# kenahm/se3-icp

Measured on AMD Instinct MI355X. Metric: ICP iterations/sec + pairs/sec, ~120k-pt KITTI clouds, 1/2/4/8 GPU, higher is better.
Workload: dtype f32 sweep + f64 certify/solve

## Files before the change

include/se3icp.h:

```cpp
#ifndef SE3ICP_H
#define SE3ICP_H

#include <stdint.h>

#ifdef __cplusplus
extern "C" {
#endif

#define SE3ICP_ABI_VERSION 4

typedef enum se3icp_status {
    SE3ICP_OK = 0,
    SE3ICP_ERR_INVALID_ARG = -1,
    SE3ICP_ERR_INVALID_METHOD = -2,
    SE3ICP_ERR_EMPTY_CLOUD = -3,
    SE3ICP_ERR_K_TOO_LARGE = -4,
    SE3ICP_ERR_NO_DEVICE = -5,
    SE3ICP_ERR_HIP = -6,
    SE3ICP_ERR_NONFINITE = -7,
    SE3ICP_ERR_OUT_OF_MEMORY = -8,
    SE3ICP_ERR_INTERNAL = -9
} se3icp_status;

typedef enum se3icp_method {
    SE3ICP_PT2PT = 0,
    SE3ICP_PT2PL = 1,
    SE3ICP_GICP = 2,
    SE3ICP_SE3_PT2PT = 3,
    SE3ICP_SE3_PT2PL = 4,
    SE3ICP_SE3_GICP = 5,
    SE3ICP_SE3_GICP_WITH_CF = 6,
    SE3ICP_SE3_PURE_PT2PT = 7,
    SE3ICP_SE3_PURE_PT2PL = 8,
    SE3ICP_SE3_PURE_GICP = 9,
    SE3ICP_NUM_METHODS = 10
} se3icp_method;

typedef struct se3icp_params {
    int32_t max_num_iterations;
    int32_t max_num_se3_iterations;
    int32_t number_of_nn_for_LRF;
    int32_t _reserved;
    double mse;
    double mse_switch_error;
    double estimated_overlap;
    double alpha_rot;
    double beta_transl;
    double scale_preprocessing;
} se3icp_params;

typedef struct se3icp_result {
    double T[16];
    int32_t num_iterations;
    int32_t num_pure_se3_iterations;
    int32_t status;
    int32_t num_rechecked;
    double scaling_factor;
    double time_setup_ms;
    double time_loop_ms;
    double time_se3_correspondence_search_ms;
    double time_before_pure_icp_ms;
} se3icp_result;

int se3icp_abi_version(void);
const char* se3icp_status_string(int status);
int se3icp_method_from_name(const char* name);
const char* se3icp_method_name(int method);
void se3icp_default_params(se3icp_params* p);
int se3icp_device_count(void);

typedef struct se3icp_registration se3icp_registration;

se3icp_registration* se3icp_registration_new(void);
void se3icp_registration_free(se3icp_registration* r);
int se3icp_set_source_cloud(se3icp_registration* r, const double* xyz, int64_t n);
int se3icp_set_target_cloud(se3icp_registration* r, const double* xyz, int64_t n);
se3icp_params* se3icp_params_of(se3icp_registration* r);
int se3icp_run_icp(se3icp_registration* r, const char* variant);
int se3icp_run_se3_icp(se3icp_registration* r, const char* variant);
int se3icp_run_se3_icp_with_cf(se3icp_registration* r);
int se3icp_run_se3_pure(se3icp_registration* r, const char* variant);
int se3icp_get_result(const se3icp_registration* r, se3icp_result* out);

int se3icp_register_batch(int device, int32_t n_pairs, const double* const* src_xyz, const int64_t* n_src,
                          const double* const* tgt_xyz, const int64_t* n_tgt, int method,
                          const se3icp_params* params, se3icp_result* results);

int se3icp_register_batch_device(int device, int32_t n_pairs, const double* d_src_xyz, const int64_t* src_off,
                                 const double* d_tgt_xyz, const int64_t* tgt_off, int method,
                                 const se3icp_params* params, se3icp_result* results, void* hip_stream);

int se3icp_register_sweep(int device, int32_t n_pairs, const double* const* src_xyz, const int64_t* n_src,
                          const double* const* tgt_xyz, const int64_t* n_tgt, int method, int32_t n_variants,
                          const se3icp_params* variants, int32_t max_group, se3icp_result* results);
int se3icp_register_sweep_device(int device, int32_t n_pairs, const double* d_src_xyz, const int64_t* src_off,
                                 const double* d_tgt_xyz, const int64_t* tgt_off, int method, int32_t n_variants,
                                 const se3icp_params* variants, int32_t max_group, se3icp_result* results,
                                 void* hip_stream);

int se3icp_register_graph(int device, int32_t n_clouds, const double* const* xyz, const int64_t* n_pts,
                          int32_t n_pairs, const int32_t* src_cloud, const int32_t* tgt_cloud, int method,
                          const se3icp_params* params, int32_t sharing, se3icp_result* results);
int se3icp_register_graph_device(int device, int32_t n_clouds, const double* d_xyz, const int64_t* off,
                                 int32_t n_pairs, const int32_t* src_cloud, const int32_t* tgt_cloud, int method,
                                 const se3icp_params* params, int32_t sharing, se3icp_result* results,
                                 void* hip_stream);
struct se3icp_report_options;
struct se3icp_report;
int se3icp_register_graph_report(int device, int32_t n_clouds, const double* const* xyz, const int64_t* n_pts,
                                 int32_t n_pairs, const int32_t* src_cloud, const int32_t* tgt_cloud, int method,
                                 const se3icp_params* params, int32_t sharing, se3icp_result* results,
                                 const struct se3icp_report_options* opts, struct se3icp_report* reports);
int se3icp_register_graph_report_device(int device, int32_t n_clouds, const double* d_xyz, const int64_t* off,
                                        int32_t n_pairs, const int32_t* src_cloud, const int32_t* tgt_cloud,
                                        int method, const se3icp_params* params, int32_t sharing,
                                        se3icp_result* results, void* hip_stream,
                                        const struct se3icp_report_options* opts, struct se3icp_report* reports);
#define SE3ICP_GRAPH_STATS_N 9
int se3icp_last_graph_stats(int device, int64_t* out, int n);

int se3icp_set_batch_sharing(int device, int level);

typedef enum se3icp_stop_reason {
    SE3ICP_STOP_CONVERGED = 0,
    SE3ICP_STOP_MAX_ITERATIONS = 1,
    SE3ICP_STOP_MAX_SE3_ITERATIONS = 2,
    SE3ICP_STOP_RUNAWAY = 3
} se3icp_stop_reason;

typedef struct se3icp_report_options {
    double max_correspondence_distance;
    int32_t* corr_idx;
    double* corr_dist;
    int32_t outputs_on_device;
    int32_t _reserved;
} se3icp_report_options;

typedef struct se3icp_report {
    double fitness;
    double inlier_rmse;
    double information[36];
    double final_mse;
    double final_mse_change;
    int64_t n_inliers;
    int32_t switched;
    int32_t stop_reason;
} se3icp_report;

int se3icp_report_version(void);

int se3icp_register_batch_report(int device, int32_t n_pairs, const double* const* src_xyz, const int64_t* n_src,
                                 const double* const* tgt_xyz, const int64_t* n_tgt, int method,
                                 const se3icp_params* params, se3icp_result* results,
                                 const se3icp_report_options* opts, se3icp_report* reports);
int se3icp_register_batch_report_device(int device, int32_t n_pairs, const double* d_src_xyz, const int64_t* src_off,
                                        const double* d_tgt_xyz, const int64_t* tgt_off, int method,
                                        const se3icp_params* params, se3icp_result* results, void* hip_stream,
                                        const se3icp_report_options* opts, se3icp_report* reports);
int se3icp_register_sweep_report(int device, int32_t n_pairs, const double* const* src_xyz, const int64_t* n_src,
                                 const double* const* tgt_xyz, const int64_t* n_tgt, int method, int32_t n_variants,
                                 const se3icp_params* variants, int32_t max_group, se3icp_result* results,
                                 const se3icp_report_options* opts, se3icp_report* reports);
int se3icp_register_sweep_report_device(int device, int32_t n_pairs, const double* d_src_xyz, const int64_t* src_off,
                                        const double* d_tgt_xyz, const int64_t* tgt_off, int method,
                                        int32_t n_variants, const se3icp_params* variants, int32_t max_group,
                                        se3icp_result* results, void* hip_stream,
                                        const se3icp_report_options* opts, se3icp_report* reports);
int se3icp_request_report(se3icp_registration* r, const se3icp_report_options* opts);
int se3icp_get_report(const se3icp_registration* r, se3icp_report* out);

int se3icp_register(int device, const double* src_xyz, int64_t n_src, const double* tgt_xyz, int64_t n_tgt,
                    int method, const se3icp_params* params, se3icp_result* result);


int se3icp_toldi_frames(int device, const double* xyz, int64_t n, int k, double* frames);
int se3icp_knn_self(int device, const double* xyz, int64_t n, int k, int32_t* idx);
int se3icp_estimate_normals(int device, const double* xyz, int64_t n, int k, double* normals);
int se3icp_nn(int device, const double* query, int64_t nq, const double* data, int64_t nd, int dim,
              int32_t* idx, double* d2, int32_t* num_rechecked);

int64_t se3icp_synthetic_pairs(int device, const double* base, int64_t n, int32_t n_cases, const double* T,
                               double ratio, double noise_var, uint64_t seed, double* src_out, double* tgt_out,
                               int outputs_on_device);

#define SE3ICP_GEN_ARGS_LTR 1
int64_t se3icp_synthetic_reference(const double* cloud, int64_t n, int32_t n_cases, double ratio, double noise_var,
                                   double t_range, double r_range, int32_t flags, double* src_out, double* tgt_out,
                                   double* T_out);
int64_t se3icp_synthetic_reference_device(int device, const double* cloud, int64_t n, int32_t n_cases, double ratio,
                                          double noise_var, double t_range, double r_range, int32_t flags,
                                          double* src_out, double* tgt_out, double* T_out, int outputs_on_device);
int64_t se3icp_random_downsample(const double* xyz, int64_t n, double ratio, uint32_t seed, double* out);

int se3icp_set_profiling(int device, int on);
int se3icp_last_kernel_times(int device, double* out);
#define SE3ICP_KERNEL_TIMES_N 26
int se3icp_last_kernel_times_n(int device, double* out, int n);

typedef struct se3icp_trace {
    int32_t pair;
    int32_t max_iters;
    int32_t* corr_idx;
    float* corr_dist;
    uint64_t* trim_key;
    double* T;
    double* mse;
    int32_t* phase;
    int32_t iters_recorded;
    int32_t _reserved;
} se3icp_trace;
int se3icp_set_trace(int device, se3icp_trace* trace);

int se3icp_set_lrf_exact(int device, int exact_only);

int se3icp_set_nn_events(int device, int on);

#ifdef __cplusplus
}
#endif
#endif
```

se3-icp_amd/csrc/capi.cpp:

```cpp
#include <hip/hip_runtime.h>

#include <cmath>
#include <cstdio>
#include <cstring>
#include <iostream>
#include <mutex>
#include <string>
#include <vector>

#include "engine.hpp"
#include "graph.hpp"
#include "se3icp.h"

using se3icp::Engine;
using se3icp::engine_for;
using se3icp::graph_check;
using se3icp::GS_COUNT;

namespace {

const char* kMethodNames[SE3ICP_NUM_METHODS] = {"pt2pt",     "pt2pl",     "gicp",
                                                "se3_pt2pt", "se3_pt2pl", "se3_gicp",
                                                "se3_gicp_with_cf", "se3_pure_pt2pt", "se3_pure_pt2pl",
                                                "se3_pure_gicp"};
// ... 27 lines not shown
    se3icp_result res;
    bool want_report = false, have_report = false;
    se3icp_report_options ropts{};
    se3icp_report rep{};
};

extern "C" {

int se3icp_abi_version(void) { return SE3ICP_ABI_VERSION; }

const char* se3icp_status_string(int status) {
    switch (status) {
        case SE3ICP_OK: return "ok";
        case SE3ICP_ERR_INVALID_ARG: return "invalid argument";
        case SE3ICP_ERR_INVALID_METHOD: return "invalid method name";
        case SE3ICP_ERR_EMPTY_CLOUD: return "empty point cloud";
        case SE3ICP_ERR_K_TOO_LARGE: return "number_of_nn_for_LRF too large (unused since ABI 3: any k is taken)";
        case SE3ICP_ERR_NO_DEVICE: return "no usable HIP device (the engine has no CPU fallback)";
        case SE3ICP_ERR_HIP: return "HIP runtime error";
        case SE3ICP_ERR_NONFINITE: return "non-finite pose";
        case SE3ICP_ERR_OUT_OF_MEMORY: return "out of device memory";
        case SE3ICP_ERR_INTERNAL: return "internal error: a result left unset or out of range";
        default: return "unknown status";
    }
}

int se3icp_method_from_name(const char* name) {
    if (!name) return SE3ICP_ERR_INVALID_METHOD;
    for (int m = 0; m < SE3ICP_NUM_METHODS; ++m)
        if (!std::strcmp(name, kMethodNames[m])) return m;
    return SE3ICP_ERR_INVALID_METHOD;
}

const char* se3icp_method_name(int method) {
    return (method >= 0 && method < SE3ICP_NUM_METHODS) ? kMethodNames[method] : nullptr;
}

void se3icp_default_params(se3icp_params* p) {
    if (!p) return;
    std::memset(p, 0, sizeof(*p));
    p->max_num_iterations = 150;
    p->max_num_se3_iterations = 20;
    p->number_of_nn_for_LRF = 30;
    p->mse = 0.00001;
    p->mse_switch_error = 0.001;
    p->estimated_overlap = 1.0;
    p->alpha_rot = 3.0;
    p->beta_transl = 1.0;
    p->scale_preprocessing = 3.0;
}

int se3icp_device_count(void) {
    int n = 0;
    if (hipGetDeviceCount(&n) != hipSuccess) return 0;
    return n;
}

static se3icp_params params_or_defaults(const se3icp_params* params) {
    se3icp_params p;
    if (params) p = *params; else se3icp_default_params(&p);
    return p;
}

struct PairRanges {
    std::vector<const double*> s, t;
    std::vector<int64_t> ns, nt;
};
static int pair_ranges(int32_t n_pairs, const double* d_src_xyz, const int64_t* src_off, const double* d_tgt_xyz,
                       const int64_t* tgt_off, PairRanges* r) {
    if (n_pairs <= 0 || !d_src_xyz || !d_tgt_xyz || !src_off || !tgt_off) return SE3ICP_ERR_INVALID_ARG;
    r->s.resize(n_pairs); r->t.resize(n_pairs); r->ns.resize(n_pairs); r->nt.resize(n_pairs);
    for (int i = 0; i < n_pairs; ++i) {
        r->s[i] = d_src_xyz + 3 * src_off[i];
        r->t[i] = d_tgt_xyz + 3 * tgt_off[i];
        r->ns[i] = src_off[i + 1] - src_off[i];
        r->nt[i] = tgt_off[i + 1] - tgt_off[i];
    }
    return SE3ICP_OK;
}

static int report_check(const se3icp_report_options* opts, const se3icp_report* reports, bool per_point_allowed) {
    if (!opts || !reports) return SE3ICP_ERR_INVALID_ARG;
    if (std::isnan(opts->max_correspondence_distance)) return SE3ICP_ERR_INVALID_ARG;
    if (!per_point_allowed && (opts->corr_idx || opts->corr_dist)) return SE3ICP_ERR_INVALID_ARG;
    return SE3ICP_OK;
}

static int pairs_check(int32_t n_pairs, const double* const* src, const int64_t* n_src, const double* const* tgt,
                       const int64_t* n_tgt, int method, const se3icp_params* prm, const se3icp_result* results) {
    if (n_pairs <= 0 || !n_src || !n_tgt || !results) return SE3ICP_ERR_INVALID_ARG;
    if (method < 0 || method >= SE3ICP_NUM_METHODS) return SE3ICP_ERR_INVALID_METHOD;
    for (int32_t p = 0; p < n_pairs; ++p)
        if (n_src[p] <= 0 || n_tgt[p] <= 0) return SE3ICP_ERR_EMPTY_CLOUD;
    if (method >= SE3ICP_SE3_PT2PT && prm && prm->number_of_nn_for_LRF <= 0) return SE3ICP_ERR_INVALID_ARG;
    for (int32_t p = 0; p < n_pairs; ++p)
        if (!src[p] || !tgt[p]) return SE3ICP_ERR_INVALID_ARG;
    return SE3ICP_OK;
}

static int batch_run(int device, int args, int32_t n_pairs, const double* const* src, const int64_t* n_src,
                     const double* const* tgt, const int64_t* n_tgt, bool on_device, int method,
                     const se3icp_params* params, se3icp_result* results, void* hip_stream,
                     const se3icp_report_options* opts, se3icp_report* reports, bool with_report) {
    if (with_report) {
        int rc = args ? args : report_check(opts, reports, true);
        if (!rc) rc = pairs_check(n_pairs, src, n_src, tgt, n_tgt, method, params, results);
        if (rc) return rc;
    }
    Engine* e = usable_engine(device);
    if (!e) return SE3ICP_ERR_NO_DEVICE;
    if (args) return args;
    const se3icp_params p = params_or_defaults(params);
    std::lock_guard<std::mutex> lk(e->mutex());
    return e->register_batch(n_pairs, src, n_src, tgt, n_tgt, on_device, method, p, results, (hipStream_t)hip_stream,
                             with_report ? opts : nullptr, with_report ? reports : nullptr);
}

static int sweep_run(int device, int args, int32_t n_pairs, const double* const* src, const int64_t* n_src,
                     const double* const* tgt, const int64_t* n_tgt, bool on_device, int method, int32_t n_variants,
                     const se3icp_params* variants, int32_t max_group, se3icp_result* results, void* hip_stream,
                     const se3icp_report_options* opts, se3icp_report* reports, bool with_report) {
    int rc = args;
    if (!rc && with_report) rc = report_check(opts, reports, false);
    if (!rc && (n_variants <= 0 || !variants || max_group < 0)) rc = SE3ICP_ERR_INVALID_ARG;
    if (!rc) rc = pairs_check(n_pairs, src, n_src, tgt, n_tgt, method, variants, results);
    for (int32_t v = 1; !rc && v < n_variants; ++v)
        if (variants[v].number_of_nn_for_LRF != variants[0].number_of_nn_for_LRF ||
            variants[v].scale_preprocessing != variants[0].scale_preprocessing)
            rc = SE3ICP_ERR_INVALID_ARG;
    if (rc) return rc;
    Engine* e = usable_engine(device);
    if (!e) return SE3ICP_ERR_NO_DEVICE;
    std::lock_guard<std::mutex> lk(e->mutex());
    return e->register_sweep(n_pairs, src, n_src, tgt, n_tgt, on_device, method, n_variants, variants, max_group,
                             results, (hipStream_t)hip_stream, with_report ? opts : nullptr,
                             with_report ? reports : nullptr);
}

int se3icp_register_batch(int device, int32_t n_pairs, const double* const* src_xyz, const int64_t* n_src,
                          const double* const* tgt_xyz, const int64_t* n_tgt, int method,
                          const se3icp_params* params, se3icp_result* results) {
    return batch_run(device, SE3ICP_OK, n_pairs, src_xyz, n_src, tgt_xyz, n_tgt, false, method, params, results,
                     nullptr, nullptr, nullptr, false);
}

int se3icp_register_batch_device(int device, int32_t n_pairs, const double* d_src_xyz, const int64_t* src_off,
                                 const double* d_tgt_xyz, const int64_t* tgt_off, int method,
                                 const se3icp_params* params, se3icp_result* results, void* hip_stream) {
    PairRanges r;
    const int args = pair_ranges(n_pairs, d_src_xyz, src_off, d_tgt_xyz, tgt_off, &r);
    return batch_run(device, args, n_pairs, r.s.data(), r.ns.data(), r.t.data(), r.nt.data(), true, method, params,
                     results, hip_stream, nullptr, nullptr, false);
}

int se3icp_register_batch_report(int device, int32_t n_pairs, const double* const* src_xyz, const int64_t* n_src,
                                 const double* const* tgt_xyz, const int64_t* n_tgt, int method,
                                 const se3icp_params* params, se3icp_result* results,
                                 const se3icp_report_options* opts, se3icp_report* reports) {
    const int args = (!src_xyz || !tgt_xyz) ? SE3ICP_ERR_INVALID_ARG : SE3ICP_OK;
    return batch_run(device, args, n_pairs, src_xyz, n_src, tgt_xyz, n_tgt, false, method, params, results, nullptr,
                     opts, reports, true);
}

int se3icp_register_batch_report_device(int device, int32_t n_pairs, const double* d_src_xyz, const int64_t* src_off,
                                        const double* d_tgt_xyz, const int64_t* tgt_off, int method,
                                        const se3icp_params* params, se3icp_result* results, void* hip_stream,
                                        const se3icp_report_options* opts, se3icp_report* reports) {
    PairRanges r;
    const int args = pair_ranges(n_pairs, d_src_xyz, src_off, d_tgt_xyz, tgt_off, &r);
    return batch_run(device, args, n_pairs, r.s.data(), r.ns.data(), r.t.data(), r.nt.data(), true, method, params,
                     results, hip_stream, opts, reports, true);
}

int se3icp_register_sweep(int device, int32_t n_pairs, const double* const* src_xyz, const int64_t* n_src,
                          const double* const* tgt_xyz, const int64_t* n_tgt, int method, int32_t n_variants,
                          const se3icp_params* variants, int32_t max_group, se3icp_result* results) {
    const int args = (!src_xyz || !tgt_xyz) ? SE3ICP_ERR_INVALID_ARG : SE3ICP_OK;
    return sweep_run(device, args, n_pairs, src_xyz, n_src, tgt_xyz, n_tgt, false, method, n_variants, variants,
                     max_group, results, nullptr, nullptr, nullptr, false);
}

int se3icp_register_sweep_device(int device, int32_t n_pairs, const double* d_src_xyz, const int64_t* src_off,
                                 const double* d_tgt_xyz, const int64_t* tgt_off, int method, int32_t n_variants,
                                 const se3icp_params* variants, int32_t max_group, se3icp_result* results,
                                 void* hip_stream) {
    PairRanges r;
    const int args = pair_ranges(n_pairs, d_src_xyz, src_off, d_tgt_xyz, tgt_off, &r);
    return sweep_run(device, args, n_pairs, r.s.data(), r.ns.data(), r.t.data(), r.nt.data(), true, method, n_variants,
                     variants, max_group, results, hip_stream, nullptr, nullptr, false);
}

int se3icp_report_version(void) { return 1; }

int se3icp_register_sweep_report(int device, int32_t n_pairs, const double* const* src_xyz, const int64_t* n_src,
                                 const double* const* tgt_xyz, const int64_t* n_tgt, int method, int32_t n_variants,
                                 const se3icp_params* variants, int32_t max_group, se3icp_result* results,
                                 const se3icp_report_options* opts, se3icp_report* reports) {
    const int args = (!src_xyz || !tgt_xyz) ? SE3ICP_ERR_INVALID_ARG : SE3ICP_OK;
    return sweep_run(device, args, n_pairs, src_xyz, n_src, tgt_xyz, n_tgt, false, method, n_variants, variants,
                     max_group, results, nullptr, opts, reports, true);
}

int se3icp_register_sweep_report_device(int device, int32_t n_pairs, const double* d_src_xyz, const int64_t* src_off,
                                        const double* d_tgt_xyz, const int64_t* tgt_off, int method,
                                        int32_t n_variants, const se3icp_params* variants, int32_t max_group,
                                        se3icp_result* results, void* hip_stream,
                                        const se3icp_report_options* opts, se3icp_report* reports) {
    PairRanges r;
    const int args = pair_ranges(n_pairs, d_src_xyz, src_off, d_tgt_xyz, tgt_off, &r);
    return sweep_run(device, args, n_pairs, r.s.data(), r.ns.data(), r.t.data(), r.nt.data(), true, method, n_variants,
                     variants, max_group, results, hip_stream, opts, reports, true);
}

static int graph_run(int device, int32_t n_clouds, const double* const* xyz, const int64_t* n_pts, bool on_device,
                     int32_t n_pairs, const int32_t* src_cloud, const int32_t* tgt_cloud, int method,
                     const se3icp_params* params, int32_t sharing, se3icp_result* results, void* hip_stream,
                     bool with_report, const se3icp_report_options* opts, se3icp_report* reports) {
    if (with_report) {
        const int rc = report_check(opts, reports, true);
        if (rc) return rc;
    }
    int rc = graph_check(n_clouds, n_pts, nullptr, n_pairs, src_cloud, tgt_cloud, method, SE3ICP_NUM_METHODS, sharing,
                         results);
    if (rc) return rc;
    if (method >= SE3ICP_SE3_PT2PT && params && params->number_of_nn_for_LRF <= 0) return SE3ICP_ERR_INVALID_ARG;
    for (int32_t p = 0; p < n_pairs; ++p)
        if (!xyz[src_cloud[p]] || !xyz[tgt_cloud[p]]) return SE3ICP_ERR_INVALID_ARG;
    Engine* e = usable_engine(device);
    if (!e) return SE3ICP_ERR_NO_DEVICE;
    const se3icp_params p = params_or_defaults(params);
    std::lock_guard<std::mutex> lk(e->mutex());
    return e->register_graph(n_clouds, xyz, n_pts, n_pairs, src_cloud, tgt_cloud, on_device, method, p, sharing, results,
                             (hipStream_t)hip_stream, with_report ? opts : nullptr, with_report ? reports : nullptr);
}

static int cloud_ranges(int32_t n_clouds, const double* d_xyz, const int64_t* off, std::vector<const double*>& x,
                        std::vector<int64_t>& n) {
    if (n_clouds <= 0 || !d_xyz || !off) return SE3ICP_ERR_INVALID_ARG;
    x.resize(n_clouds);
    n.resize(n_clouds);
    for (int32_t c = 0; c < n_clouds; ++c) {
        x[c] = d_xyz + 3 * off[c];
        n[c] = off[c + 1] - off[c];
    }
    return SE3ICP_OK;
}

int se3icp_register_graph(int device, int32_t n_clouds, const double* const* xyz, const int64_t* n_pts,
                          int32_t n_pairs, const int32_t* src_cloud, const int32_t* tgt_cloud, int method,
                          const se3icp_params* params, int32_t sharing, se3icp_result* results) {
    if (!xyz) return SE3ICP_ERR_INVALID_ARG;
    return graph_run(device, n_clouds, xyz, n_pts, false, n_pairs, src_cloud, tgt_cloud, method, params, sharing, results,
                     nullptr, false, nullptr, nullptr);
}

int se3icp_register_graph_device(int device, int32_t n_clouds, const double* d_xyz, const int64_t* off,
                                 int32_t n_pairs, const int32_t* src_cloud, const int32_t* tgt_cloud, int method,
                                 const se3icp_params* params, int32_t sharing, se3icp_result* results,
                                 void* hip_stream) {
    std::vector<const double*> x;
    std::vector<int64_t> n;
    const int rc = cloud_ranges(n_clouds, d_xyz, off, x, n);
    if (rc) return rc;
    return graph_run(device, n_clouds, x.data(), n.data(), true, n_pairs, src_cloud, tgt_cloud, method, params, sharing,
                     results, hip_stream, false, nullptr, nullptr);
}

int se3icp_register_graph_report(int device, int32_t n_clouds, const double* const* xyz, const int64_t* n_pts,
                                 int32_t n_pairs, const int32_t* src_cloud, const int32_t* tgt_cloud, int method,
                                 const se3icp_params* params, int32_t sharing, se3icp_result* results,
                                 const se3icp_report_options* opts, se3icp_report* reports) {
    if (!xyz) return SE3ICP_ERR_INVALID_ARG;
    return graph_run(device, n_clouds, xyz, n_pts, false, n_pairs, src_cloud, tgt_cloud, method, params, sharing, results,
                     nullptr, true, opts, reports);
}

int se3icp_register_graph_report_device(int device, int32_t n_clouds, const double* d_xyz, const int64_t* off,
                                        int32_t n_pairs, const int32_t* src_cloud, const int32_t* tgt_cloud, int method,
                                        const se3icp_params* params, int32_t sharing, se3icp_result* results,
                                        void* hip_stream, const se3icp_report_options* opts, se3icp_report* reports) {
    std::vector<const double*> x;
    std::vector<int64_t> n;
    const int rc = cloud_ranges(n_clouds, d_xyz, off, x, n);
    if (rc) return rc;
    return graph_run(device, n_clouds, x.data(), n.data(), true, n_pairs, src_cloud, tgt_cloud, method, params, sharing,
                     results, hip_stream, true, opts, reports);
}

int se3icp_last_graph_stats(int device, int64_t* out, int n) {
    if (!out || n < GS_COUNT) return SE3ICP_ERR_INVALID_ARG;
    Engine* e = usable_engine(device);
    if (!e) return SE3ICP_ERR_NO_DEVICE;
    std::lock_guard<std::mutex> lk(e->mutex());
    for (int k = 0; k < GS_COUNT; ++k) out[k] = e->graph_stats()[k];
    return SE3ICP_OK;
}

int se3icp_set_batch_sharing(int device, int level) {
    if (level < se3icp::kBatchSharingMin || level > se3icp::kBatchSharingMax) return SE3ICP_ERR_INVALID_ARG;
    Engine* e = usable_engine(device);
    if (!e) return SE3ICP_ERR_NO_DEVICE;
    std::lock_guard<std::mutex> lk(e->mutex());
    e->set_batch_sharing(level);
    return SE3ICP_OK;
}

int se3icp_register(int device, const double* src_xyz, int64_t n_src, const double* tgt_xyz, int64_t n_tgt,
                    int method, const se3icp_params* params, se3icp_result* result) {
    return se3icp_register_batch(device, 1, &src_xyz, &n_src, &tgt_xyz, &n_tgt, method, params, result);
}

se3icp_registration* se3icp_registration_new(void) {
    auto* r = new (std::nothrow) se3icp_registration;
    if (!r) return nullptr;
    se3icp_default_params(&r->prm);
    std::memset(&r->res, 0, sizeof(r->res));
    for (int i = 0; i < 4; ++i) r->res.T[i * 4 + i] = 1.0;
    r->res.num_pure_se3_iterations = -1;
    return r;
}

void se3icp_registration_free(se3icp_registration* r) { delete r; }

int se3icp_set_source_cloud(se3icp_registration* r, const double* xyz, int64_t n) {
    if (!r || (n > 0 && !xyz) || n < 0) return SE3ICP_ERR_INVALID_ARG;
    r->src.insert(r->src.end(), xyz, xyz + 3 * n);
    return 0;
}

int se3icp_set_target_cloud(se3icp_registration* r, const double* xyz, int64_t n) {
    if (!r || (n > 0 && !xyz) || n < 0) return SE3ICP_ERR_INVALID_ARG;
    r->tgt.insert(r->tgt.end(), xyz, xyz + 3 * n);
    return 0;
}

se3icp_params* se3icp_params_of(se3icp_registration* r) { return r ? &r->prm : nullptr; }

static int run_object(se3icp_registration* r, int method) {
    const int64_t ns = (int64_t)r->src.size() / 3, nt = (int64_t)r->tgt.size() / 3;
    if (ns <= 0 || nt <= 0) return SE3ICP_ERR_EMPTY_CLOUD;
    const double* s = r->src.data();
    const double* t = r->tgt.data();
    se3icp_result res;
    se3icp_report rep;
    int rc = r->want_report ? se3icp_register_batch_report(current_device(), 1, &s, &ns, &t, &nt, method, &r->prm, &res,
                                                           &r->ropts, &rep)
                            : se3icp_register_batch(current_device(), 1, &s, &ns, &t, &nt, method, &r->prm, &res);
    if (rc == SE3ICP_OK || rc == SE3ICP_ERR_NONFINITE) {
        r->res = res;
        r->have_report = r->want_report;
        if (r->want_report) r->rep = rep;
    }
    return rc;
}

int se3icp_run_icp(se3icp_registration* r, const char* variant) {
    if (!r) return SE3ICP_ERR_INVALID_ARG;
    const int v = variant_index(variant);
    if (v < 0) {
        std::cerr << "Invalid ICP variant name. Valid names are pt2pt, pt2pl and gicp.\n";
        return SE3ICP_ERR_INVALID_METHOD;
    }
    return run_object(r, SE3ICP_PT2PT + v);
}

int se3icp_run_se3_icp(se3icp_registration* r, const char* variant) {
    if (!r) return SE3ICP_ERR_INVALID_ARG;
    const int v = variant_index(variant);
    if (v < 0) {
        std::cerr << "Invalid variant name. Choose one of: pt2pt, pt2pl, gicp \n";
        std::cout << "Unknown optimization strategy for SE(3) \n";
        const int64_t ns = (int64_t)r->src.size() / 3, nt = (int64_t)r->tgt.size() / 3;
        if (ns <= 0 || nt <= 0) return SE3ICP_ERR_EMPTY_CLOUD;
        double cs[3] = {0, 0, 0}, ct[3] = {0, 0, 0};
        for (int64_t i = 0; i < ns; ++i)
            for (int a = 0; a < 3; ++a) cs[a] += r->src[3 * i + a];
        for (int64_t i = 0; i < nt; ++i)
            for (int a = 0; a < 3; ++a) ct[a] += r->tgt[3 * i + a];
        std::memset(r->res.T, 0, sizeof(r->res.T));
        for (int a = 0; a < 4; ++a) r->res.T[a * 4 + a] = 1.0;
        for (int a = 0; a < 3; ++a) r->res.T[a * 4 + 3] = ct[a] / (double)nt - cs[a] / (double)ns;
        r->res.num_iterations = 1;
        r->res.num_pure_se3_iterations = 1;
        r->res.status = SE3ICP_ERR_INVALID_METHOD;
        return SE3ICP_ERR_INVALID_METHOD;
    }
    return run_object(r, SE3ICP_SE3_PT2PT + v);
}

int se3icp_run_se3_icp_with_cf(se3icp_registration* r) {
    if (!r) return SE3ICP_ERR_INVALID_ARG;
    const int rc = run_object(r, SE3ICP_SE3_GICP_WITH_CF);
    if (rc == SE3ICP_OK || rc == SE3ICP_ERR_NONFINITE)
        std::cout << "### scaling factor = " << r->res.scaling_factor << std::endl;
    return rc;
}

int se3icp_run_se3_pure(se3icp_registration* r, const char* variant) {
    if (!r) return SE3ICP_ERR_INVALID_ARG;
    const int v = variant_index(variant);
    if (v < 0) {
        std::cerr << "Invalid variant name. Choose one of: pt2pt, pt2pl, gicp \n";
        return SE3ICP_ERR_INVALID_METHOD;
    }
    const int rc = run_object(r, SE3ICP_SE3_PURE_PT2PT + v);
    if (rc == SE3ICP_OK || rc == SE3ICP_ERR_NONFINITE) std::cout << "pure se3 finished" << std::endl;
    return rc;
}

int se3icp_get_result(const se3icp_registration* r, se3icp_result* out) {
    if (!r || !out) return SE3ICP_ERR_INVALID_ARG;
    *out = r->res;
    return 0;
}

int se3icp_request_report(se3icp_registration* r, const se3icp_report_options* opts) {
    if (!r) return SE3ICP_ERR_INVALID_ARG;
    if (!opts) {
        r->want_report = false;
        return 0;
    }
    if (std::isnan(opts->max_correspondence_distance) || opts->outputs_on_device) return SE3ICP_ERR_INVALID_ARG;
    r->ropts = *opts;
    r->want_report = true;
    return 0;
}

int se3icp_get_report(const se3icp_registration* r, se3icp_report* out) {
    if (!r || !out || !r->have_report) return SE3ICP_ERR_INVALID_ARG;
    *out = r->rep;
    return 0;
}

int se3icp_toldi_frames(int device, const double* xyz, int64_t n, int k, double* frames) {
    Engine* e = usable_engine(device);
    if (!e) return SE3ICP_ERR_NO_DEVICE;
    std::lock_guard<std::mutex> lk(e->mutex());
    return e->toldi_frames(xyz, n, k, frames);
}

int se3icp_knn_self(int device, const double* xyz, int64_t n, int k, int32_t* idx) {
    Engine* e = usable_engine(device);
    if (!e) return SE3ICP_ERR_NO_DEVICE;
    std::lock_guard<std::mutex> lk(e->mutex());
    return e->knn_self(xyz, n, k, idx);
}

int se3icp_estimate_normals(int device, const double* xyz, int64_t n, int k, double* normals) {
    Engine* e = usable_engine(device);
    if (!e) return SE3ICP_ERR_NO_DEVICE;
    std::lock_guard<std::mutex> lk(e->mutex());
    return e->estimate_normals(xyz, n, k, normals);
}

int se3icp_nn(int device, const double* query, int64_t nq, const double* data, int64_t nd, int dim, int32_t* idx,
              double* d2, int32_t* num_rechecked) {
    Engine* e = usable_engine(device);
    if (!e) return SE3ICP_ERR_NO_DEVICE;
    std::lock_guard<std::mutex> lk(e->mutex());
    return e->nn(query, nq, data, nd, dim, idx, d2, num_rechecked);
}

int se3icp_set_profiling(int device, int on) {
    Engine* e = usable_engine(device);
    if (!e) return SE3ICP_ERR_NO_DEVICE;
    e->set_profiling(on != 0);
    return 0;
}

int se3icp_set_trace(int device, se3icp_trace* trace) {
    Engine* e = usable_engine(device);
    if (!e) return SE3ICP_ERR_NO_DEVICE;
    if (trace && (trace->max_iters < 0 || trace->pair < 0)) return SE3ICP_ERR_INVALID_ARG;
    std::lock_guard<std::mutex> lk(e->mutex());
    e->set_trace(trace);
    return 0;
}

int se3icp_set_lrf_exact(int device, int exact_only) {
    Engine* e = usable_engine(device);
    if (!e) return SE3ICP_ERR_NO_DEVICE;
    std::lock_guard<std::mutex> lk(e->mutex());
    if (exact_only < 0 || exact_only > 2) return SE3ICP_ERR_INVALID_ARG;
    e->set_lrf_exact(exact_only);
    return 0;
}

int se3icp_set_nn_events(int device, int on) {
    Engine* e = usable_engine(device);
    if (!e) return SE3ICP_ERR_NO_DEVICE;
    std::lock_guard<std::mutex> lk(e->mutex());
    e->set_nn_events(on != 0);
    return 0;
}

int se3icp_last_kernel_times(int device, double* out ) {
    double x[SE3ICP_KERNEL_TIMES_N];
    const int rc = se3icp_last_kernel_times_n(device, x, SE3ICP_KERNEL_TIMES_N);
    if (rc == 0)
        for (int i = 0; i < 24; ++i) out[i] = x[i];
    return rc;
}

int se3icp_last_kernel_times_n(int device, double* out, int n) {
    Engine* e = usable_engine(device);
    if (!e || !out) return SE3ICP_ERR_NO_DEVICE;
    if (n < SE3ICP_KERNEL_TIMES_N) return SE3ICP_ERR_INVALID_ARG;
    const auto& k = e->kernel_times();
    out[0] = k.nn_se3_ms;
    out[1] = k.nn_r3_ms;
    out[2] = k.recheck_ms;
    out[3] = k.trim_ms;
    out[4] = k.reduce_ms;
    out[5] = k.setup_ms;
    out[6] = (double)k.nn_se3_launches;
    out[7] = (double)k.nn_r3_launches;
    out[8] = k.se3_dist_evals;
    out[9] = k.se3_box_tests;
    out[10] = k.r3_dist_evals;
    out[11] = k.r3_box_tests;
    out[12] = k.lrf_ms;
    out[13] = k.lrf_queries;
    out[14] = k.lrf_leaves;
    out[15] = k.lrf_merges;
    out[16] = k.lrf_box_tests;
    out[17] = k.lrf_candidates;
    out[18] = k.nn_prep_ms;
    out[19] = k.se3_queries;
    out[20] = k.se3_searched;
    out[21] = k.r3_queries;
    out[22] = k.r3_searched;
    out[23] = k.lrf_fallback;
    out[24] = k.se3_useful_evals;
    out[25] = k.r3_useful_evals;
    return 0;
}

}
```

se3-icp_amd/csrc/common.hpp:

```cpp
#pragma once
#include <stdint.h>

namespace se3icp {

constexpr int kSmallK = 128;
constexpr int kBlock = 256;
constexpr int kRedVals = 28;
constexpr int kStatCols = 17;
constexpr int kStatUseSe3 = 15, kStatUseR3 = 16;
constexpr int kHist = 256;
constexpr int kTrimList = 4096;
constexpr int kTrimBlocks = 32;
constexpr int kChunkQ = 1024;

enum Phase : int32_t { PHASE_IDLE = 0, PHASE_SE3 = 1, PHASE_R3 = 2 };
enum Estimator : int32_t { EST_PT2PT = 0, EST_PT2PL = 1, EST_GICP = 2 };

struct CloudDev {
    int32_t off;
    int32_t n;
};

struct PairDev {
    double T[12];
    double f32_center[3];
    int32_t src, tgt;
    int32_t phase;
    int32_t est;
    int32_t cf;
    int32_t trim;
    int32_t nkeep;
    int32_t iter;
    float tgt_norm12;
    float tgt_norm3;
    int32_t phase_start;
    int32_t _pad;
};

constexpr int kRedThreads = 256;
constexpr int kRedPer = 1;
constexpr int kRedQ = kRedThreads * kRedPer;

struct BlockWork {
    int32_t pair;
    int32_t q0, q1;
    int32_t s_off, t_off;
    int32_t _pad[3];
};

}
```

se3-icp_amd/csrc/engine.cpp:

```cpp
#include "engine.hpp"

#include <algorithm>
#include <chrono>
#include <cmath>
#include <cstdio>
#include <cstdlib>
#include <cstring>
#include <map>
#include <memory>

#include "graph.hpp"
#include "report.hpp"
#include "sweep.hpp"
#include "tree.hpp"

namespace se3icp {

namespace {

#define HIPCHK(x)                                                                                   \
    do {                                                                                            \
        hipError_t e_ = (x);                                                                        \
        if (e_ != hipSuccess) {                                                                     \
            std::fprintf(stderr, "se3icp: HIP error %s at %s:%d (%s)\n", hipGetErrorString(e_), __FILE__, \
// ... 124 lines not shown

int Engine::init() {
    int n = 0;
    if (hipGetDeviceCount(&n) != hipSuccess || dev_ < 0 || dev_ >= n) return SE3ICP_ERR_NO_DEVICE;
    HIPCHK(hipSetDevice(dev_));
    HIPCHK(hipStreamCreateWithFlags(&stream_, hipStreamNonBlocking));
    for (auto& e : ev_) HIPCHK(hipEventCreate(&e));
    for (auto& e : loop_ev_) HIPCHK(hipEventCreate(&e));
    if (const char* e = std::getenv("SE3ICP_NN_TRACE")) nn_trace_ = std::atoi(e) != 0;
    return 0;
}

Engine::~Engine() {
    if (!ok_) return;
    (void)hipSetDevice(dev_);
    for (DevBuf* b : bufs_)
        if (b->p) (void)hipFree(b->p);
    for (PinnedMem* m : pins_)
        if (m->mem) (void)hipHostFree(m->mem);
    for (auto& e : ev_)
        if (e) (void)hipEventDestroy(e);
    for (auto& e : loop_ev_)
        if (e) (void)hipEventDestroy(e);
    if (h_phase_) (void)hipHostFree(h_phase_);
    if (stream_) (void)hipStreamDestroy(stream_);
}

template <class T>
T* Engine::ensure(DevBuf& b, size_t count) {
    const size_t want = std::max<size_t>(count, 1) * sizeof(T);
    if (b.bytes >= want) return static_cast<T*>(b.p);
    if (b.p) (void)hipFree(b.p);
    b.p = nullptr;
    b.bytes = 0;
    const size_t alloc = want + want / 4;
    if (hipMalloc(&b.p, alloc) != hipSuccess) {
        b.p = nullptr;
        return nullptr;
    }
    b.bytes = alloc;
    return static_cast<T*>(b.p);
}

int Engine::alloc_points(int64_t ntot, int kmax, bool knn_list) {
    if (ntot >= (int64_t)1 << 30) return SE3ICP_ERR_INVALID_ARG;
    ntot_ = ntot;
    ld_ = (int)((std::max<int64_t>(ntot, 1) + 63) / 64 * 64);
    kmax_ = std::max(kmax, 1);
    knn_list_ = knn_list;
    const size_t L = (size_t)ld_;
    bool ok = ensure<int32_t>(d_cloud_of_, L) && ensure<double>(d_in_, 3 * L) && ensure<double>(d_xyz64_, 3 * L) &&
              ensure<float>(d_xyz32_, 3 * L) && ensure<double>(d_fr64_, 12 * L) && ensure<float>(d_fr32_, 12 * L) &&
              ensure<double>(d_nrm64_, 3 * L) && ensure<double>(d_conf64_, L) && ensure<double>(d_tgeo_, 8 * L) &&
              (!knn_list || ensure<int32_t>(d_knn_, L * kmax_)) && ensure<int32_t>(d_corr_idx_, L) && ensure<float>(d_corr_dist_, L) &&
              ensure<int32_t>(d_flag_count_, 4) &&
              ensure<uint32_t>(d_keys0_, L) &&
              ensure<int32_t>(d_vals1_, L) && ensure<unsigned long long>(d_stats_, kStatCols * kStatSlots) &&
              ensure<NNCert>(d_cert_, L) &&
              ensure<int32_t>(d_sqlist_, L);
    for (TreeBufs* t : {&t3_, &t12_})
        ok = ok && ensure<int32_t>(t->perm, L) && ensure<int32_t>(t->pos, L);
    ok = ok && ensure<float>(t3_.vec, 3 * L) && ensure<float>(t12_.vec, 12 * L);
    return ok ? 0 : SE3ICP_ERR_OUT_OF_MEMORY;
}

View Engine::view() const {
    View v{};
    v.ld = ld_;
    v.npts = (int32_t)ntot_;
    v.nclouds = nclouds_;
    v.npairs = npairs_;
    v.kmax = kmax_;
    v.clouds = (CloudDev*)d_clouds_.p;
    v.setup = (CloudSetup*)d_setup_.p;
    v.pairs = (PairDev*)d_pairs_.p;
    v.cloud_of = (int32_t*)d_cloud_of_.p;
    v.in_ptr = (const double* const*)d_inptr_.p;
    v.xyz64 = (double*)d_xyz64_.p;
    v.xyz32 = (float*)d_xyz32_.p;
    v.fr64 = (double*)d_fr64_.p;
    v.fr32 = (float*)d_fr32_.p;
    v.nrm64 = (double*)d_nrm64_.p;
    v.conf64 = (double*)d_conf64_.p;
    v.tgeo = (double*)d_tgeo_.p;
    v.knn = knn_list_ ? (int32_t*)d_knn_.p : nullptr;
    v.corr_idx = (int32_t*)d_corr_idx_.p;
    v.corr_dist = (float*)d_corr_dist_.p;
    v.stats = (unsigned long long*)d_stats_.p;
    v.flag_count = (int32_t*)d_flag_count_.p;
    v.gcost = (uint32_t*)d_gcost_.p;
    v.cls = (int32_t*)d_cls_.p;
    v.trim_key = (uint64_t*)d_trim_key_.p;
    v.trim_cand = (unsigned long long*)d_trim_cand_.p;
    v.trim_ctr = (unsigned*)d_trim_ctr_.p;
    v.trim_hist = (unsigned*)d_trim_hist_.p;
    v.red_partial = (double*)d_red_partial_.p;
    v.red_out = (double*)d_red_out_.p;
    v.work = (const BlockWork*)d_work_.p;
    v.nwork = nwork_;
    v.pair_rechecked = (int32_t*)d_rechecked_.p;
    auto ref = [&](const TreeBufs& t) {
        TreeRef r{};
        r.L = t.L;
        r.GL = tree_L_;
        r.nnodes = 2 << t.L;
        r.perm = (const int32_t*)t.perm.p;
        r.pos = (const int32_t*)t.pos.p;
        r.tvec = (const float*)t.vec.p;
        r.tvec64 = (const double*)t.vec64.p;
        r.tpt64 = (const double4*)t.vec64a.p;
        r.lo = (const float*)t.lo.p;
        r.hi = (const float*)t.hi.p;
        return r;
    };
    v.t3 = ref(t3_);
    v.t12 = ref(t12_);
    v.chunk_level = chunk_level_;
    v.nchunks = nchunks_;
    v.qlist = (int32_t*)d_qlist_.p;
    v.qcount = (int32_t*)d_qcount_.p;
    v.sq_list = (int32_t*)d_sqlist_.p;
    v.hist = (const double*)d_hist_.p;
    v.cert = (NNCert*)d_cert_.p;
    return v;
}

int Engine::build_tree(int D, const float* vec, hipStream_t s, const double* vec64) {
    TreeBufs& tb = (D == 12) ? t12_ : t3_;
    tb.L = tree_L_;
    const int nnodes = 2 << tb.L;
    const size_t nb = (size_t)nclouds_ * nnodes * D;
    if (!ensure<uint32_t>(tb.blo, nb) || !ensure<uint32_t>(tb.bhi, nb) || !ensure<float>(tb.lo, nb) ||
        !ensure<float>(tb.hi, nb) || !ensure<float>(tb.scr, (size_t)D * ld_) ||
        (D == 12 && !ensure<float>(tb.vecT, (size_t)12 * ld_)) ||
        (vec64 && !ensure<double>(tb.vec64, (size_t)3 * ld_)) ||
        (vec64 && D == 3 && !ensure<double4>(tb.vec64a, (size_t)ld_)))
        return SE3ICP_ERR_OUT_OF_MEMORY;
    std::vector<int32_t> host_n(nclouds_);
    int max_n = 0;
    for (int c = 0; c < nclouds_; ++c) max_n = std::max(max_n, host_n[c] = h_clouds_[c].n);
    const size_t need = tree_build_temp_bytes((int)ntot_, nclouds_, max_n, tb.L);
    if (!ensure<char>(d_sort_tmp_, std::max<size_t>(need, 256))) return SE3ICP_ERR_OUT_OF_MEMORY;
    TreeView t{};
    t.host_n = host_n.data();
    t.D = D;
    t.L = tb.L;
    t.nnodes = nnodes;
    t.nclouds = nclouds_;
    t.npts = (int32_t)ntot_;
    t.ld = ld_;
    t.clouds = (const CloudDev*)d_clouds_.p;
    t.cloud_of = (const int32_t*)d_cloud_of_.p;
    t.vec = vec;
    t.vecT = (D == 12) ? (float*)tb.vecT.p : const_cast<float*>(vec);
    t.perm = (int32_t*)tb.perm.p;
    t.pos = (int32_t*)tb.pos.p;
    t.tvec = (float*)tb.vec.p;
    t.vec64 = vec64;
    t.tvec64 = vec64 ? (double*)tb.vec64.p : nullptr;
    t.tpt64 = (vec64 && D == 3) ? (double4*)tb.vec64a.p : nullptr;
    t.vec64_sources_only = D == 12;
    t.blo = (uint32_t*)tb.blo.p;
    t.bhi = (uint32_t*)tb.bhi.p;
    t.scr = (float*)tb.scr.p;
    t.lo = (float*)tb.lo.p;
    t.hi = (float*)tb.hi.p;
    if (build_trees(t, d_sort_tmp_.p, d_sort_tmp_.bytes, (uint32_t*)d_keys0_.p, (int32_t*)d_vals1_.p, s) != 0)
        return SE3ICP_ERR_HIP;
    return 0;
}

int Engine::upload_clouds(const std::vector<CloudReq>& clouds, bool on_device, hipStream_t s) {
    nclouds_ = (int)clouds.size();
    h_clouds_.assign(nclouds_, CloudDev{});
    h_setup_.resize(nclouds_);
    h_chunks_.clear();
    h_inptr_.assign(nclouds_, nullptr);
    int64_t off = 0;
    int max_n = 1;
    for (int c = 0; c < nclouds_; ++c) {
        h_clouds_[c].off = (int32_t)off;
        h_clouds_[c].n = (int32_t)clouds[c].n;
        h_setup_[c] = clouds[c].st;
        max_n = std::max<int>(max_n, (int)clouds[c].n);
        for (int64_t p0 = 0; p0 < clouds[c].n; p0 += kChunk) h_chunks_.push_back(ChunkWork{c, (int32_t)p0});
        off += clouds[c].n;
    }
    tree_L_ = tree_depth_for(max_n);
    double* d_in = (double*)d_in_.p;
    for (int c = 0; c < nclouds_; ++c) {
        if (on_device) {
            h_inptr_[c] = clouds[c].in;
        } else {
            double* dst = d_in + 3 * (size_t)h_clouds_[c].off;
            HIPCHK(hipMemcpyAsync(dst, clouds[c].in, sizeof(double) * 3 * clouds[c].n, hipMemcpyHostToDevice, s));
            h_inptr_[c] = dst;
        }
    }
    const int nch = (int)h_chunks_.size();
    if (!ensure<CloudDev>(d_clouds_, nclouds_) || !ensure<CloudSetup>(d_setup_, nclouds_) ||
        !ensure<ChunkWork>(d_chunks_, nch) || !ensure<const double*>(d_inptr_, nclouds_) ||
        !ensure<double>(d_partial_, (size_t)nch * 9) || !ensure<double>(d_centers_, 3 * (size_t)nclouds_))
        return SE3ICP_ERR_OUT_OF_MEMORY;
    if (h_partial_.reserve((size_t)nch * 9 + 8)) return SE3ICP_ERR_OUT_OF_MEMORY;
    HIPCHK(hipMemcpyAsync(d_clouds_.p, h_clouds_.data(), sizeof(CloudDev) * nclouds_, hipMemcpyHostToDevice, s));
    HIPCHK(hipMemcpyAsync(d_setup_.p, h_setup_.data(), sizeof(CloudSetup) * nclouds_, hipMemcpyHostToDevice, s));
    HIPCHK(hipMemcpyAsync(d_chunks_.p, h_chunks_.data(), sizeof(ChunkWork) * nch, hipMemcpyHostToDevice, s));
    HIPCHK(hipMemcpyAsync(d_inptr_.p, h_inptr_.data(), sizeof(double*) * nclouds_, hipMemcpyHostToDevice, s));
    return 0;
}

int Engine::host_centroids(hipStream_t s, std::vector<double>* cen) {
    const int nch = (int)h_chunks_.size();
    HIPCHK(hipMemcpyAsync(h_partial_, d_partial_.p, sizeof(double) * 9 * nch, hipMemcpyDeviceToHost, s));
    SYNC_STREAM(s);
    std::vector<double> sum(3 * (size_t)nclouds_, 0.0);
    for (int k = 0; k < nch; ++k)
        for (int a = 0; a < 3; ++a) sum[3 * (size_t)h_chunks_[k].cloud + a] += h_partial_[9 * (size_t)k + a];
    cen->assign(3 * (size_t)nclouds_, 0.0);
    for (int c = 0; c < nclouds_; ++c)
        for (int a = 0; a < 3; ++a)
            (*cen)[3 * (size_t)c + a] = h_clouds_[c].n > 0 ? sum[3 * (size_t)c + a] / (double)h_clouds_[c].n : 0.0;
    return 0;
}

int Engine::setup_clouds(const std::vector<CloudReq>& clouds, bool on_device, bool pairs, bool normalize,
                         double scale_pre, hipStream_t s) {
    int rc = upload_clouds(clouds, on_device, s);
    if (rc) return rc;
    const int nch = (int)h_chunks_.size();
    View v = view();

    launch_ingest(v, (const ChunkWork*)d_chunks_.p, nch, (double*)d_partial_.p, s);
    HIPCHK(hipGetLastError());
    if (normalize) {
        if (!ensure<double>(d_scales_, std::max(1, nclouds_ / 2))) return SE3ICP_ERR_OUT_OF_MEMORY;
        launch_pair_centers(v, (const ChunkWork*)d_chunks_.p, nch, (const double*)d_partial_.p, (double*)d_centers_.p,
                            s);
        launch_radius(v, (const ChunkWork*)d_chunks_.p, nch, (const double*)d_centers_.p, (double*)d_partial_.p, s);
        launch_pair_scales(v, (const ChunkWork*)d_chunks_.p, nch, (const double*)d_partial_.p,
                           (const double*)d_centers_.p, scale_pre, (double*)d_scales_.p, s);
        HIPCHK(hipGetLastError());
        for (int c = 0; c < nclouds_; ++c)
            for (int a = 0; a < 3; ++a) h_setup_[c].f32_center[a] = 0.0;
    } else {
        std::vector<double> cen;
        rc = host_centroids(s, &cen);
        if (rc) return rc;
        for (int c = 0; c < nclouds_; ++c) {
            const int cc = pairs ? (c | 1) : c;
            for (int a = 0; a < 3; ++a) {
                h_setup_[c].norm_center[a] = 0.0;
                h_setup_[c].f32_center[a] = cen[3 * cc + a];
            }
            h_setup_[c].norm_scale = 1.0;
        }
        HIPCHK(hipMemcpyAsync(d_setup_.p, h_setup_.data(), sizeof(CloudSetup) * nclouds_, hipMemcpyHostToDevice, s));
    }

    launch_normalize(v, (const ChunkWork*)d_chunks_.p, nch, (double*)d_partial_.p, s);
    HIPCHK(hipGetLastError());

    rc = build_tree(3, (const float*)d_xyz32_.p, s, (const double*)d_xyz64_.p);
    if (rc) return rc;
    rc = setup_knn(s);
    if (rc) return rc;
    HIPCHK(hipGetLastError());
    return 0;
}

int Engine::setup_knn(hipStream_t s) {
    const View v = view();
    bool any_knn = false;
    for (int c = 0; c < nclouds_; ++c) any_knn |= h_setup_[c].k_knn > 0;
    if (any_knn) {
        HIPCHK(hipMemsetAsync(d_stats_.p, 0, sizeof(unsigned long long) * kStatCols * kStatSlots, s));
        HIPCHK(hipEventRecord(ev_[6], s));
        int kw_big = 0, n_big = 0;
        for (int c = 0; c < nclouds_; ++c) {
            const int kw = std::min<int>(h_setup_[c].k_knn, h_clouds_[c].n);
            if (kw > kSmallK || lrf_exact_only_ == 2) {
                kw_big = std::max(kw_big, kw);
                n_big += h_clouds_[c].n;
            }
        }
        int big_cap = 0, big_blocks = 0;
        if (n_big > 0) {
            big_cap = knn_big_cap(kw_big);
            big_blocks = knn_big_blocks(big_cap, n_big);
            if (!ensure<double>(d_big_d_, (size_t)big_blocks * big_cap) || !ensure<int32_t>(d_big_i_, (size_t)big_blocks * big_cap))
                return SE3ICP_ERR_OUT_OF_MEMORY;
        }
        auto big = [&](const int32_t* qlist, const int32_t* qcount, int k_min) {
            if (n_big > 0)
                launch_knn_big(v, knn_list_ ? 1 : 0, k_min, qlist, qcount, big_blocks, (double*)d_big_d_.p,
                               (int32_t*)d_big_i_.p, big_cap, s);
        };
        if (lrf_exact_only_ == 2) {
            big(nullptr, nullptr, 0);
        } else if (knn_list_ || lrf_exact_only_ == 1) {
            launch_lrf(v, knn_list_ ? 1 : 0, s);
            big(nullptr, nullptr, kSmallK);
        } else {
            std::vector<int32_t> wb(nclouds_ + 1, 0);
            for (int c = 0; c < nclouds_; ++c) wb[c + 1] = wb[c] + (h_setup_[c].k_knn > 0 ? (h_clouds_[c].n + 7) / 8 : 0);
            const int nw = wb[nclouds_];
            if (!ensure<int32_t>(d_lrf_fb_, (size_t)8 * nw + 64) || !ensure<int32_t>(d_lrf_fbn_, 2 + nclouds_ + 1))
                return SE3ICP_ERR_OUT_OF_MEMORY;
            int32_t* d_wb = (int32_t*)d_lrf_fbn_.p + 2;
            int32_t* fb = (int32_t*)d_lrf_fb_.p;
            int32_t* fbn = (int32_t*)d_lrf_fbn_.p;
            HIPCHK(hipMemsetAsync(fbn, 0, 2 * sizeof(int32_t), s));
            HIPCHK(hipMemcpyAsync(d_wb, wb.data(), sizeof(int32_t) * (nclouds_ + 1), hipMemcpyHostToDevice, s));
            launch_lrf8(v, d_wb, 0, nw, fb, fbn, s);
            launch_lrf_list(v, fb, fbn, s);
            big(fb, fbn, kSmallK);
        }
        HIPCHK(hipEventRecord(ev_[7], s));
        HIPCHK(hipGetLastError());
        if (h_lrf_stats_.reserve((size_t)kStatCols * kStatSlots)) return SE3ICP_ERR_OUT_OF_MEMORY;
        HIPCHK(hipMemcpyAsync(h_lrf_stats_, d_stats_.p, sizeof(unsigned long long) * kStatCols * kStatSlots,
                              hipMemcpyDeviceToHost, s));
        lrf_stats_pending_ = true;
    }
    return 0;
}

int Engine::read_lrf_stats() {
    if (!lrf_stats_pending_) return 0;
    lrf_stats_pending_ = false;
    double sum[kStatCols] = {};
    for (int i = 0; i < kStatSlots; ++i)
        for (int k = 0; k < kStatCols; ++k) sum[k] += (double)h_lrf_stats_[kStatCols * i + k];
    float ms = 0;
    HIPCHK(hipEventElapsedTime(&ms, ev_[6], ev_[7]));
    ktimes_.lrf_ms = ms;
    ktimes_.lrf_queries = sum[0];
    ktimes_.lrf_leaves = sum[1];
    ktimes_.lrf_merges = sum[2];
    ktimes_.lrf_box_tests = sum[3];
    ktimes_.lrf_candidates = sum[4];
    ktimes_.lrf_fallback = sum[6];
#ifdef SE3ICP_PROF
    tree_prof_report();
    std::fprintf(stderr, "[prof] k_lrf cycles/query: knn|scan %.0f sort|tighten %.0f sums|final+sums %.0f finish %.0f "
                 "(queries %.0f, wave cycles summed over the kernel's waves)\n",
                 sum[8] / sum[0], sum[9] / sum[0], sum[10] / sum[0], sum[11] / sum[0], sum[0]);
    std::fprintf(stderr, "[prof] k_lrf8 per query: tightenings %.3f (overflow %.3f, final %.3f), leaf scans %.3f\n",
                 sum[2] / sum[0], sum[3] / sum[0], sum[7] / sum[0], sum[1] / sum[0]);
    {
        unsigned long long f = 0;
        for (int i = 0; i < kStatSlots; ++i) f += h_lrf_stats_[kStatCols * i + 5];
        std::fprintf(stderr, "[prof] k_lrf8 hand-overs: waves with the leaf table full %llu, no room %llu, > 128 at the end %llu; "
                     "queries with f32-equal f64-distinct ranks %llu\n",
                     f & 0xffff, (f >> 16) & 0xffff, (f >> 32) & 0xffff, f >> 48);
    }
#endif
    return 0;
}

int Engine::sync_stream(hipStream_t s) {
    HIPCHK(hipEventRecord(ev_[15], s));
    HIPCHK(spin_wait(ev_[15]));
    return read_lrf_stats();
}

int Engine::setup_chunks(int npairs, hipStream_t s) {
    chunk_level_ = std::max(0, tree_L_ - 4);
    nchunks_ = npairs << chunk_level_;
    if (!ensure<int32_t>(d_qlist_, (size_t)nchunks_ * kChunkQ) || !ensure<int32_t>(d_qcount_, (size_t)nchunks_ * (kChunkQ / 64)) ||
        !ensure<double>(d_hist_, (size_t)kHist * npairs * 12) || !ensure<uint32_t>(d_gcost_, (size_t)nchunks_ * 16) ||
        !ensure<int32_t>(d_cls_, nn_cls_words(nchunks_)))
        return SE3ICP_ERR_OUT_OF_MEMORY;
    if (h_hist_.reserve((size_t)npairs * 12)) return SE3ICP_ERR_OUT_OF_MEMORY;
    HIPCHK(hipMemsetAsync(d_cert_.p, 0xff, sizeof(NNCert) * ld_, s));
    HIPCHK(hipMemsetAsync(d_gcost_.p, 0, sizeof(uint32_t) * nchunks_ * 16, s));
    HIPCHK(hipMemsetAsync(d_cls_.p, 0, sizeof(int32_t) * 2 * 8 * 16, s));
    return 0;
}

int Engine::open_call(int args, int64_t nslots, int rest, hipStream_t user_stream, Call* c) {
    if (!ok_) return SE3ICP_ERR_NO_DEVICE;
    se3icp_trace* tr = c->tr = trace_;
    trace_ = nullptr;
    if (args) return args;
    if (tr && (tr->pair < 0 || (int64_t)tr->pair >= nslots || tr->max_iters < 0)) return SE3ICP_ERR_INVALID_ARG;
    if (tr) tr->iters_recorded = 0;
    if (rest) return rest;
    HIPCHK(hipSetDevice(dev_));
    c->s = user_stream ? user_stream : stream_;
    ktimes_ = KernelTimes{};
    HIPCHK(hipEventRecord(ev_[12], c->s));
    return 0;
}

int Engine::run_pairs(const MethodPlan& mp, int npairs, const int64_t* ns, const int64_t* nt,
                      const se3icp_params* vprm, int pairs_per_variant, bool sweep, const Call& c, se3icp_result* out,
                      const se3icp_report_options* ropts, se3icp_report* reports) {
    hipStream_t s = c.s;
    int rc = 0;
    if (mp.se3) rc = build_tree(12, (const float*)d_fr32_.p, s, (const double*)d_fr64_.p);
    if (rc) return rc;
    rc = prepare_pairs(npairs, ns, nt, s);
    if (rc) return rc;
    rc = setup_chunks(npairs, s);
    if (rc) return rc;
    HIPCHK(hipMemsetAsync(d_corr_idx_.p, 0xff, sizeof(int32_t) * ld_, s));
    HIPCHK(hipMemsetAsync(d_stats_.p, 0, sizeof(unsigned long long) * kStatCols * kStatSlots, s));
    for (double& t : trace_prev_) t = 0;
    HIPCHK(hipEventRecord(ev_[13], s));
    const ReportReq rq{ropts, reports};
    return run_loop(npairs, ns, mp.kind, mp.est, vprm, pairs_per_variant, sweep, c.tr, out, s,
                    (ropts && reports) ? &rq : nullptr);
}

int Engine::register_batch(int npairs, const double* const* src, const int64_t* ns, const double* const* tgt,
                           const int64_t* nt, bool on_device, int method, const se3icp_params& prm,
                           se3icp_result* out, hipStream_t user_stream, const se3icp_report_options* ropts,
                           se3icp_report* reports) {
    const int args = (npairs <= 0 || !src || !tgt || !ns || !nt || !out) ? SE3ICP_ERR_INVALID_ARG : 0;
    MethodPlan mp{};
    const int rest = args ? 0 : plan_pairs(method, prm.number_of_nn_for_LRF, npairs, src, ns, tgt, nt, &mp);
    Call call;
    int rc = open_call(args, npairs, rest, user_stream, &call);
    if (rc) return rc;

    npairs_ = npairs;
    int64_t ntot = 0;
    for (int p = 0; p < npairs; ++p) ntot += ns[p] + nt[p];
    rc = alloc_points(ntot, mp.kmax);
    if (rc) return rc;
    std::vector<CloudReq> clouds(2 * npairs);
    for (int p = 0; p < npairs; ++p)
        for (int side = 0; side < 2; ++side)
            clouds[2 * p + side] = CloudReq{side == 0 ? src[p] : tgt[p], side == 0 ? ns[p] : nt[p],
                                            cloud_setup(mp, side, prm.alpha_rot, prm.beta_transl, true)};
    bool look = false;
    if (on_device && batch_sharing_ != 1) {
        std::vector<int64_t> n(clouds.size());
        for (size_t u = 0; u < clouds.size(); ++u) n[u] = clouds[u].n;
        look = clouds.size() <= kShareMaxSlots && share_any_equal_n((int32_t)n.size(), n.data());
        for (int64_t& g : graph_stats_) g = 0;
        graph_stats_[GS_CLOUDS] = graph_stats_[GS_USES] = graph_stats_[GS_CLASSES] = (int64_t)clouds.size();
        for (const CloudReq& c : clouds) graph_stats_[GS_FULL] += c.st.k_knn > 0;
    }
    rc = look ? setup_pairs_shared(clouds, mp, prm.scale_preprocessing, call.s)
              : setup_clouds(clouds, on_device, true, mp.se3, prm.scale_preprocessing, call.s);
    if (rc) return rc;
    return run_pairs(mp, npairs, ns, nt, &prm, npairs, false, call, out, ropts, reports);
}

int Engine::setup_pairs_shared(const std::vector<CloudReq>& clouds, const MethodPlan& mp, double scale_pre,
                               hipStream_t s) {
    const int U = (int)clouds.size();
    const bool se3 = mp.se3;
    int rc = upload_clouds(clouds, true, s);
    if (rc) return rc;
    const int nch = (int)h_chunks_.size();
    if (!ensure<uint64_t>(d_share_hash_, U) || !ensure<SharePair>(d_share_pairs_, U) ||
        !ensure<int32_t>(d_share_same_, U) || h_share_hash_.reserve(U) || h_share_same_.reserve(U) ||
        h_share_setup_.reserve(U))
        return SE3ICP_ERR_OUT_OF_MEMORY;
    View v = view();
    HIPCHK(hipMemsetAsync(d_share_hash_.p, 0, sizeof(uint64_t) * U, s));
    launch_share_hash(v, (unsigned long long*)d_share_hash_.p, s);
    HIPCHK(hipMemcpyAsync(h_share_hash_, d_share_hash_.p, sizeof(uint64_t) * U, hipMemcpyDeviceToHost, s));
    launch_ingest(v, (const ChunkWork*)d_chunks_.p, nch, (double*)d_partial_.p, s);
    HIPCHK(hipGetLastError());
    if (se3) {
        if (!ensure<double>(d_scales_, std::max(1, nclouds_ / 2))) return SE3ICP_ERR_OUT_OF_MEMORY;
        launch_pair_centers(v, (const ChunkWork*)d_chunks_.p, nch, (const double*)d_partial_.p, (double*)d_centers_.p,
                            s);
        launch_radius(v, (const ChunkWork*)d_chunks_.p, nch, (const double*)d_centers_.p, (double*)d_partial_.p, s);
        launch_pair_scales(v, (const ChunkWork*)d_chunks_.p, nch, (const double*)d_partial_.p,
                           (const double*)d_centers_.p, scale_pre, (double*)d_scales_.p, s);
        HIPCHK(hipGetLastError());
        HIPCHK(hipMemcpyAsync(h_share_setup_, d_setup_.p, sizeof(CloudSetup) * U, hipMemcpyDeviceToHost, s));
        HIPCHK(hipEventRecord(ev_[10], s));
        for (int c = 0; c < nclouds_; ++c)
            for (int a = 0; a < 3; ++a) h_setup_[c].f32_center[a] = 0.0;
    } else {
        std::vector<double> cen;
        rc = host_centroids(s, &cen);
        if (rc) return rc;
        for (int c = 0; c < nclouds_; ++c) {
            for (int a = 0; a < 3; ++a) {
                h_setup_[c].norm_center[a] = 0.0;
                h_setup_[c].f32_center[a] = cen[3 * (c | 1) + a];
            }
            h_setup_[c].norm_scale = 1.0;
        }
        HIPCHK(hipMemcpyAsync(d_setup_.p, h_setup_.data(), sizeof(CloudSetup) * nclouds_, hipMemcpyHostToDevice, s));
    }
    launch_normalize(v, (const ChunkWork*)d_chunks_.p, nch, (double*)d_partial_.p, s);
    HIPCHK(hipGetLastError());
    rc = build_tree(3, (const float*)d_xyz32_.p, s, (const double*)d_xyz64_.p);
    if (rc) return rc;
    if (se3) HIPCHK(spin_wait(ev_[10]));

    std::vector<int64_t> n(U);
    for (int u = 0; u < U; ++u) n[u] = clouds[u].n;
    std::vector<int32_t> first, cloud;
    const int ncand = share_candidates(U, n.data(), h_share_hash_, &first);
    int nc = U;
    if (ncand > 0) {
        share_pairs_.clear();
        for (int u = 0; u < U; ++u)
            if (first[u] != u) share_pairs_.push_back(SharePair{u, first[u]});
        HIPCHK(hipMemcpyAsync(d_share_pairs_.p, share_pairs_.data(), sizeof(SharePair) * ncand, hipMemcpyHostToDevice, s));
        HIPCHK(hipMemsetAsync(d_share_same_.p, 1, sizeof(int32_t) * U, s));
        launch_share_compare(v, (const SharePair*)d_share_pairs_.p, ncand, (int32_t*)d_share_same_.p, s);
        HIPCHK(hipGetLastError());
        HIPCHK(hipMemcpyAsync(h_share_same_, d_share_same_.p, sizeof(int32_t) * U, hipMemcpyDeviceToHost, s));
        HIPCHK(hipEventRecord(ev_[11], s));
        HIPCHK(spin_wait(ev_[11]));
        nc = share_clouds(U, first.data(), h_share_same_, &cloud);
    }
    if (nc == U) return setup_knn(s);

    const CloudSetup* dev_table = se3 ? (const CloudSetup*)h_share_setup_ : h_setup_.data();
    share_setup_.assign(dev_table, dev_table + U);
    std::vector<GraphUse> use(U);
    for (int u = 0; u < U; ++u) {
        const CloudSetup& st = share_setup_[u];
        use[u].cloud = cloud[u];
        use[u].k_nrm = st.k_nrm;
        use[u].norm_scale = st.norm_scale;
        for (int a = 0; a < 3; ++a) {
            use[u].norm_center[a] = st.norm_center[a];
            use[u].f32_center[a] = st.f32_center[a];
        }
    }
    GraphPlan plan;
    graph_plan_uses(U, use.data(), se3, true, &plan);
    graph_stats_[GS_CLOUDS] = nc;
    graph_stats_[GS_CLASSES] = (int64_t)plan.classes.size();
    return select_by_class(plan, share_setup_, mp, s);
}

int Engine::select_by_class(const GraphPlan& plan, const std::vector<CloudSetup>& batch, const MethodPlan& mp,
                            hipStream_t s) {
    const int U = (int)batch.size(), K = (int)plan.classes.size();
    const bool se3 = mp.se3;
    std::vector<int32_t> home(K, -1);
    for (int u = 0; u < U; ++u)
        if (home[plan.use_class[u]] < 0) home[plan.use_class[u]] = u;
    sel_batch_ = batch;
    sel_run_ = sel_batch_;
    sel_chunks_.clear();
    sel_seg_.assign(U, GraphSeg{});
    graph_stats_[GS_FULL] = 0;
    for (int u = 0; u < U; ++u) {
        const int k = plan.use_class[u];
        const GraphClass& gc = plan.classes[k];
        CloudSetup& st = sel_run_[u];
        const bool is_home = home[k] == u;
        st.k_lrf = is_home ? mp.k_lrf : 0;
        st.k_nrm = (is_home && gc.nrm_from == k) ? gc.k_nrm : 0;
        st.k_knn = std::max(st.k_lrf, st.k_nrm);
        graph_stats_[GS_FULL] += st.k_knn > 0;
        const int hf = home[k], hn = home[gc.nrm_from];
        sel_seg_[u] = GraphSeg{h_clouds_[hf].off, hf, h_clouds_[hn].off, (hf != u && se3) ? 1 : 0};
        if ((hf != u && se3) || hn != u)
            for (int64_t p0 = 0; p0 < h_clouds_[u].n; p0 += kChunk) sel_chunks_.push_back(ChunkWork{u, (int32_t)p0});
    }
    const int nchS = (int)sel_chunks_.size();
    if (!ensure<ChunkWork>(g_chunks_, nchS) || !ensure<GraphSeg>(g_seg_, U)) return SE3ICP_ERR_OUT_OF_MEMORY;
    h_setup_ = sel_run_;
    HIPCHK(hipMemcpyAsync(d_setup_.p, sel_run_.data(), sizeof(CloudSetup) * U, hipMemcpyHostToDevice, s));
    const int rc = setup_knn(s);
    if (rc) return rc;
    HIPCHK(hipGetLastError());
    h_setup_ = sel_batch_;
    HIPCHK(hipMemcpyAsync(d_setup_.p, sel_batch_.data(), sizeof(CloudSetup) * U, hipMemcpyHostToDevice, s));
    if (nchS > 0) {
        HIPCHK(hipMemcpyAsync(g_chunks_.p, sel_chunks_.data(), sizeof(ChunkWork) * nchS, hipMemcpyHostToDevice, s));
        HIPCHK(hipMemcpyAsync(g_seg_.p, sel_seg_.data(), sizeof(GraphSeg) * U, hipMemcpyHostToDevice, s));
        launch_graph_share(view(), (const ChunkWork*)g_chunks_.p, nchS, (const GraphSeg*)g_seg_.p, s);
        HIPCHK(hipGetLastError());
    }
    return 0;
}

int Engine::prepare_pairs(int npairs, const int64_t* ns, const int64_t* nt, hipStream_t s) {
    int64_t soff = 0;
    h_work_.clear();
    h_wb_.assign(npairs, 0);
    h_wn_.assign(npairs, 0);
    for (int p = 0; p < npairs; ++p) {
        h_wb_[p] = (int32_t)h_work_.size();
        for (int64_t q0 = 0; q0 < ns[p]; q0 += kRedQ)
            h_work_.push_back(BlockWork{p, (int32_t)q0, (int32_t)std::min<int64_t>(q0 + kRedQ, ns[p]), (int32_t)soff,
                                        (int32_t)(soff + ns[p]), {0, 0, 0}});
        soff += ns[p] + nt[p];
        h_wn_[p] = (int32_t)h_work_.size() - h_wb_[p];
    }
    nwork_ = (int)h_work_.size();
    if (!ensure<PairDev>(d_pairs_, npairs) || !ensure<BlockWork>(d_work_, nwork_) || !ensure<int32_t>(d_wb_, npairs) ||
        !ensure<int32_t>(d_wn_, npairs) || !ensure<uint64_t>(d_trim_key_, 2 * (size_t)npairs) ||
        !ensure<unsigned long long>(d_trim_cand_, (size_t)npairs * kTrimList) || !ensure<unsigned>(d_trim_ctr_, 4 * (size_t)npairs) ||
        !ensure<unsigned>(d_trim_hist_, 4096 * (size_t)npairs) ||
        !ensure<double>(d_red_partial_, (size_t)nwork_ * kRedVals) || !ensure<double>(d_red_out_, (size_t)npairs * kRedVals) ||
        !ensure<int32_t>(d_rechecked_, npairs))
        return SE3ICP_ERR_OUT_OF_MEMORY;
    if (h_pairs_.reserve(npairs) || h_red_.reserve((size_t)npairs * kRedVals) || h_rechecked_.reserve(npairs))
        return SE3ICP_ERR_OUT_OF_MEMORY;
    HIPCHK(hipMemcpyAsync(d_work_.p, h_work_.data(), sizeof(BlockWork) * nwork_, hipMemcpyHostToDevice, s));
    HIPCHK(hipMemcpyAsync(d_wb_.p, h_wb_.data(), sizeof(int32_t) * npairs, hipMemcpyHostToDevice, s));
    HIPCHK(hipMemcpyAsync(d_wn_.p, h_wn_.data(), sizeof(int32_t) * npairs, hipMemcpyHostToDevice, s));
    HIPCHK(hipMemsetAsync(d_rechecked_.p, 0, sizeof(int32_t) * npairs, s));
    return 0;
}

int Engine::run_loop(int npairs, const int64_t* ns, int kind, int est, const se3icp_params* vprm,
                     int pairs_per_variant, bool sweep, se3icp_trace* tr, se3icp_result* out, hipStream_t s,
                     const ReportReq* rq) {
    const MethodInfo mi{(Kind)kind, est};
    const bool se3 = mi.kind != KIND_ICP;
    int rc = 0;

    if (!ensure<PairState>(d_state_, npairs) || h_state_.reserve(npairs))
        return SE3ICP_ERR_OUT_OF_MEMORY;
    if (h_phase_cap_ < (size_t)npairs * kLoopRing) {
        if (h_phase_) (void)hipHostFree(h_phase_);
        h_phase_ = nullptr;
        h_phase_cap_ = 0;
        const size_t want = std::max<size_t>((size_t)npairs * kLoopRing, 64);
        if (hipHostMalloc((void**)&h_phase_, want * sizeof(int32_t), hipHostMallocMapped | hipHostMallocCoherent) !=
                hipSuccess ||
            hipHostGetDevicePointer((void**)&d_phase_, h_phase_, 0) != hipSuccess)
            return SE3ICP_ERR_OUT_OF_MEMORY;
        h_phase_cap_ = want;
    }
    int se3_limit = 0;
    for (int k = 0; k * pairs_per_variant < npairs; ++k) {
        const int m = vprm[k].max_num_se3_iterations;
        se3_limit = (m < 1 || se3_limit < 0) ? -1 : std::max(se3_limit, m);
    }
    int n_se3 = 0, n_r3 = 0;
    bool any_trim = false;
    for (int p = 0; p < npairs; ++p) {
        const se3icp_params& prm = vprm[p / pairs_per_variant];
        const float ratio = std::min(1.0f, std::max(0.0f, (float)prm.estimated_overlap));
        PairState& S = h_state_[p];
        std::memset(&S, 0, sizeof(S));
        S.T = M4::eye();
        S.mse_prev = S.mse_cur = S.rel = 1e7;
        S.sf = 1.0;
        S.mse = prm.mse;
        S.mse_switch = prm.mse_switch_error;
        S.kind = mi.kind;
        S.max_iter = prm.max_num_iterations;
        S.max_se3 = prm.max_num_se3_iterations;
        S.phase = PHASE_IDLE;
        S.phase_start = 1;
        const unsigned nv = (unsigned)std::floor(ratio * (float)ns[p]);
        const bool trim = (int64_t)nv < ns[p];
        S.K = trim ? (double)nv : (double)ns[p];
        PairDev& P = h_pairs_[p];
        std::memset(&P, 0, sizeof(P));
        P.src = 2 * p;
        P.tgt = 2 * p + 1;
        P.est = mi.est;
        P.cf = mi.kind == KIND_CF;
        P.trim = trim;
        P.nkeep = (int)nv;
        for (int a = 0; a < 3; ++a) P.f32_center[a] = h_setup_[2 * p].f32_center[a];
        pair_open_iteration(S, P);
        std::memcpy(h_hist_ + 12 * (size_t)p, P.T, sizeof(P.T));
        n_se3 += P.phase == PHASE_SE3;
        n_r3 += P.phase == PHASE_R3;
        any_trim |= trim;
    }
    HIPCHK(hipMemcpyAsync(d_pairs_.p, h_pairs_, sizeof(PairDev) * npairs, hipMemcpyHostToDevice, s));
    HIPCHK(hipMemcpyAsync(d_state_.p, h_state_, sizeof(PairState) * npairs, hipMemcpyHostToDevice, s));
    HIPCHK(hipMemcpyAsync((double*)d_hist_.p + (size_t)(1 % kHist) * npairs * 12, h_hist_, sizeof(double) * 12 * npairs,
                          hipMemcpyHostToDevice, s));
    HIPCHK(hipMemsetAsync(d_flag_count_.p, 0, 3 * sizeof(int32_t), s));
    launch_pair_norms(view(), 2 << t3_.L, se3 ? 2 << t12_.L : 0, se3 ? (const double*)d_scales_.p : nullptr,
                      (double*)((char*)d_state_.p + offsetof(PairState, sf)), (int)(sizeof(PairState) / sizeof(double)),
                      s);
    HIPCHK(hipGetLastError());
    HIPCHK(hipMemsetAsync((uint64_t*)d_trim_key_.p + npairs, 0, sizeof(uint64_t) * npairs, s));
    HIPCHK(hipMemsetAsync(d_trim_ctr_.p, 0, sizeof(unsigned) * 4 * npairs, s));
    launch_geo_rows(view(), s);
    HIPCHK(hipMemsetAsync(d_trim_hist_.p, 0, sizeof(unsigned) * 4096 * npairs, s));
    View v = view();
    double nn_ms = 0;
    const int lag = (nn_trace_ || tr) ? 0 : 1;
    int trace_phase = tr ? h_pairs_[tr->pair].phase : 0;
    auto enqueue = [&](int it) -> int {
        hipEvent_t* ev = &loop_ev_[(it % kLoopRing) * kLoopEv];
        for (int p = 0; p < npairs; ++p) h_phase_[(size_t)(it % kLoopRing) * npairs + p] = -1;
        const bool do_se3 =
            n_se3 > 0 && (se3_limit < 1 || it <= se3_limit);
        const bool do_r3 = n_r3 > 0 || (mi.kind != KIND_ICP && mi.kind != KIND_PURE && it >= 2);
        const bool detail = profile_ || nn_trace_;
        const bool t_se3 = detail || (do_se3 && nn_events_);
        if (detail) HIPCHK(hipEventRecord(ev[0], s));
        launch_nn_prep(v, (lag == 1 && it >= 2) ? d_phase_ + (size_t)((it - 1) % kLoopRing) * npairs : nullptr, s);
        if (t_se3) HIPCHK(hipEventRecord(ev[1], s));
        if (do_se3) launch_nn(v, 12, s);
        if (t_se3) HIPCHK(hipEventRecord(ev[2], s));
        if (do_r3) launch_nn(v, 3, s);
        if (detail) HIPCHK(hipEventRecord(ev[3], s));
        if (detail) HIPCHK(hipEventRecord(ev[4], s));
        if (any_trim) launch_trim(v, s);
        if (detail) HIPCHK(hipEventRecord(ev[5], s));
        launch_reduce(v, (const int32_t*)d_wb_.p, (const int32_t*)d_wn_.p, (PairState*)d_state_.p, (double*)d_hist_.p,
                      lag == 0 ? d_phase_ + (size_t)(it % kLoopRing) * npairs : nullptr, s);
        HIPCHK(hipGetLastError());
        if (detail) HIPCHK(hipEventRecord(ev[6], s));
        loop_detail_[it % kLoopRing] = detail;
        loop_flags_[it % kLoopRing] = (do_se3 ? 1 : 0) | (do_r3 ? 2 : 0) | (t_se3 ? 4 : 0);
        return 0;
    };
    auto finish = [&](int it, bool last) -> int {
        hipEvent_t* ev = &loop_ev_[(it % kLoopRing) * kLoopEv];
        if (loop_detail_[it % kLoopRing]) HIPCHK(spin_wait(ev[6]));
        if (last && lag == 1) {
            if (!loop_detail_[it % kLoopRing]) {
                HIPCHK(hipEventRecord(ev_[15], s));
                HIPCHK(spin_wait(ev_[15]));
            }
        } else {
            HIPCHK(spin_phases(h_phase_ + (size_t)(it % kLoopRing) * npairs, npairs, s));
        }
        float ms[6] = {};
        if (loop_detail_[it % kLoopRing]) {
            for (int k = 0; k < 6; ++k) HIPCHK(hipEventElapsedTime(&ms[k], ev[k], ev[k + 1]));
        } else if (loop_flags_[it % kLoopRing] & 4) {
            HIPCHK(hipEventElapsedTime(&ms[1], ev[1], ev[2]));
        }
        ktimes_.nn_prep_ms += ms[0];
        ktimes_.nn_se3_ms += ms[1];
        ktimes_.nn_r3_ms += ms[2];
        ktimes_.recheck_ms += ms[3];
        ktimes_.trim_ms += ms[4];
        ktimes_.reduce_ms += ms[5];
        nn_ms += ms[0] + ms[1] + ms[2] + ms[3];
        const int flags = loop_flags_[it % kLoopRing];
        if (flags & 1) ktimes_.nn_se3_launches++;
        if (flags & 2) ktimes_.nn_r3_launches++;
        if (nn_trace_) {
            unsigned long long stats[kStatCols * kStatSlots];
            HIPCHK(hipMemcpy(stats, d_stats_.p, sizeof(stats), hipMemcpyDeviceToHost));
            double sum[kStatCols] = {};
            for (int i = 0; i < kStatSlots; ++i)
                for (int k = 0; k < kStatCols; ++k) sum[k] += (double)stats[kStatCols * i + k];
            std::fprintf(stderr,
                         "[nn] iter %d: se3 %.0f/%.0f searched, evals %.3g boxes %.3g | r3 %.0f/%.0f, evals %.3g "
                         "boxes %.3g | prep %.3f nn12 %.3f nn3 %.3f recheck %.3f ms\n",
                         it, sum[5] - trace_prev_[5], sum[4] - trace_prev_[4], sum[0] - trace_prev_[0],
                         sum[1] - trace_prev_[1], sum[7] - trace_prev_[7], sum[6] - trace_prev_[6],
                         sum[2] - trace_prev_[2], sum[3] - trace_prev_[3], ms[0], ms[1], ms[2], ms[3]);
#ifdef SE3ICP_PROF
            {
                double d[kStatCols];
                for (int k = 0; k < kStatCols; ++k) d[k] = sum[k] - trace_prev_[k];
                const double nw = std::floor(d[11] / 17592186044416.0), dt = d[11] - nw * 17592186044416.0;
                std::fprintf(stderr, "[nn] iter %d: %.0f SE(3) group waves, mean %.1f us, summed %.1f ms (100 MHz clock)\n",
                             it, nw, nw > 0 ? dt / nw / 100.0 : 0.0, dt / 1e5);
                std::fprintf(stderr, "[nn] iter %d: k_nn_prep span %.1f us\n", it, nn_prep_span());
                nn_wave_report(it);
                std::fprintf(stderr, "[nn] iter %d: wave cycles in leaf visits %.1f %% (target loads %.1f %%), "
                             "%.0f cycles per leaf visit, %.0f per box-test step\n", it, 100.0 * d[12] / std::max(1.0, d[13]),
                             100.0 * d[14] / std::max(1.0, d[13]), d[12] / std::max(1.0, d[9]),
                             (d[13] - d[12]) / std::max(1.0, d[1] / 128.0));
            }
#endif
            for (int k = 0; k < kStatCols; ++k) trace_prev_[k] = sum[k];
#ifdef SE3ICP_PROF
            std::fprintf(stderr, "[nn] iter %d: longest SE(3) group wave %.1f us (%llu box-test steps, %llu leaf visits, "
                         "%llu queries)\n", it, (double)(stats[10] >> 40) / 100.0, (stats[10] >> 20) & 0xfffffull,
                         (stats[10] >> 6) & 0x3fffull, stats[10] & 63ull);
            HIPCHK(hipMemset((unsigned long long*)d_stats_.p + 10, 0, sizeof(unsigned long long)));
#endif
        }
        if (last && lag == 1) return 0;
        const volatile int32_t* ph = h_phase_ + (size_t)(it % kLoopRing) * npairs;
        n_se3 = n_r3 = 0;
        for (int p = 0; p < npairs; ++p) {
            const int32_t f = ph[p];
            n_se3 += f == PHASE_SE3;
            n_r3 += f == PHASE_R3;
        }
        return n_se3 + n_r3;
    };
    static_assert(kLoopRing >= 2, "one iteration in flight while the previous one is read");
    int it = 1;
    if (enqueue(it)) return SE3ICP_ERR_HIP;
    for (;;) {
        if (lag == 0) {
            const int left = finish(it, false);
            if (tr) {
                rc = record_trace(tr, it, trace_phase, s);
                if (rc) return rc;
            }
            if (left == 0) break;
            ++it;
            if (enqueue(it)) return SE3ICP_ERR_HIP;
            continue;
        }
        ++it;
        if (enqueue(it)) return SE3ICP_ERR_HIP;
        if (finish(it - 1, false) == 0) {
            (void)finish(it, true);
            break;
        }
    }
    HIPCHK(hipEventRecord(ev_[14], s));
    HIPCHK(hipMemcpyAsync(h_state_, d_state_.p, sizeof(PairState) * npairs, hipMemcpyDeviceToHost, s));
    const int nbase = 2 * pairs_per_variant;
    if (se3) HIPCHK(hipMemcpyAsync(h_partial_, d_centers_.p, sizeof(double) * 3 * nbase, hipMemcpyDeviceToHost, s));
    HIPCHK(hipMemcpyAsync(h_rechecked_, d_rechecked_.p, sizeof(int32_t) * npairs, hipMemcpyDeviceToHost, s));
    {
        if (h_loop_stats_.reserve((size_t)kStatCols * kStatSlots)) return SE3ICP_ERR_OUT_OF_MEMORY;
        const unsigned long long* stats = h_loop_stats_;
        HIPCHK(hipMemcpyAsync(h_loop_stats_, d_stats_.p, sizeof(unsigned long long) * kStatCols * kStatSlots,
                              hipMemcpyDeviceToHost, s));
        if (rq) {
            rc = queue_report(npairs, ns, *rq, s);
            if (rc) return rc;
        }
        SYNC_STREAM(s);
        double sum[kStatCols] = {};
        for (int i = 0; i < kStatSlots; ++i)
            for (int k = 0; k < kStatCols; ++k) sum[k] += (double)stats[kStatCols * i + k];
        ktimes_.se3_dist_evals += sum[0];
        ktimes_.se3_box_tests += sum[1];
        ktimes_.r3_dist_evals += sum[2];
        ktimes_.r3_box_tests += sum[3];
        ktimes_.se3_queries += sum[4];
        ktimes_.se3_searched += sum[5];
        ktimes_.r3_queries += sum[6];
        ktimes_.r3_searched += sum[7];
        ktimes_.se3_useful_evals += sum[kStatUseSe3];
        ktimes_.r3_useful_evals += sum[kStatUseR3];
#ifdef SE3ICP_PROF
        {
            const double nw = std::max(1.0, std::floor(sum[11] / 17592186044416.0));
            const double mean = std::fmod(sum[11], 17592186044416.0) / nw;
            const double sq = (double)stats[kStatCols + 10] / nw;
            nn_prof_report();
            trim_prof_report();
            std::fprintf(stderr, "[prof] nn12: leaf visits %.0f; %.0f group waves, %.1f us each on average (sd %.1f, "
                         "longest %.1f us; 100 MHz clock)\n",
                         sum[9], nw, mean / 100.0, std::sqrt(std::max(0.0, sq - mean * mean)) / 100.0,
                         (double)(stats[10] >> 40) / 100.0);
            std::fprintf(stderr, "[prof] nn12 longest wave: %llu box-test steps, %llu leaf visits, %llu queries\n",
                         (stats[10] >> 20) & 0xfffffull, (stats[10] >> 6) & 0x3fffull, stats[10] & 63ull);
        }
#endif
    }
    float setup_ms = 0, loop_ms = 0;
    if (sweep) {
        float shared_ms = 0, group_ms = 0;
        HIPCHK(hipEventElapsedTime(&shared_ms, ev_[12], ev_[8]));
        HIPCHK(hipEventElapsedTime(&group_ms, ev_[9], ev_[13]));
        setup_ms = shared_ms + group_ms;
        ktimes_.setup_ms = shared_ms;
    } else {
        HIPCHK(hipEventElapsedTime(&setup_ms, ev_[12], ev_[13]));
        ktimes_.setup_ms = setup_ms;
    }
    HIPCHK(hipEventElapsedTime(&loop_ms, ev_[13], ev_[14]));

    int worst = 0;
    for (int p = 0; p < npairs; ++p) {
        const PairState& S = h_state_[p];
        M4 T = S.T;
        const int bp = p % pairs_per_variant;
        if (rq) {
// ... 590 lines not shown
```

se3-icp_amd/csrc/engine.hpp:

```cpp
#pragma once
#include <hip/hip_runtime.h>

#include <mutex>
#include <stdint.h>
#include <vector>

#include "graph.hpp"
#include "pairmath.hpp"
#include "se3icp.h"
#include "view.hpp"

namespace se3icp {

struct DevBuf {
    void* p = nullptr;
    size_t bytes = 0;
    explicit DevBuf(std::vector<DevBuf*>& owner) { owner.push_back(this); }
};
struct PinnedMem {
    void* mem = nullptr;
    size_t cap = 0;
};
template <class T>
struct Pinned : PinnedMem {
    explicit Pinned(std::vector<PinnedMem*>& owner) { owner.push_back(this); }
    operator T*() const { return static_cast<T*>(mem); }
    int reserve(size_t count) {
        if (cap >= count && mem) return 0;
        if (mem) (void)hipHostFree(mem);
        mem = nullptr;
        cap = 0;
        const size_t want = count > 16 ? count : 16;
        if (hipHostMalloc(&mem, want * sizeof(T), hipHostMallocDefault) != hipSuccess) return SE3ICP_ERR_OUT_OF_MEMORY;
        cap = want;
        return 0;
    }
};

struct KernelTimes {
    double nn_se3_ms = 0, nn_r3_ms = 0, recheck_ms = 0, trim_ms = 0, reduce_ms = 0;
    double setup_ms = 0;
    int64_t nn_se3_launches = 0, nn_r3_launches = 0;
    double se3_dist_evals = 0, se3_box_tests = 0, r3_dist_evals = 0, r3_box_tests = 0;
    double se3_useful_evals = 0, r3_useful_evals = 0;
    double lrf_ms = 0, lrf_queries = 0, lrf_leaves = 0, lrf_merges = 0, lrf_box_tests = 0, lrf_candidates = 0;
    double lrf_fallback = 0;
    double nn_prep_ms = 0, se3_queries = 0, se3_searched = 0, r3_queries = 0, r3_searched = 0;
};

struct MethodPlan {
    Kind kind;
    int est;
    bool se3;
    int k_lrf, k_nrm_s, k_nrm_t, kmax;
};

class Engine {
  public:
    explicit Engine(int device);
    ~Engine();
    Engine(const Engine&) = delete;
    Engine& operator=(const Engine&) = delete;

    int device() const { return dev_; }
    std::mutex& mutex() { return mu_; }
    void set_profiling(bool on) { profile_ = on; }
    void set_trace(se3icp_trace* t) { trace_ = t; }
    void set_lrf_exact(int mode) { lrf_exact_only_ = mode; }
    void set_nn_events(bool on) { nn_events_ = on; }
    void set_batch_sharing(int level) { batch_sharing_ = level; }
    const KernelTimes& kernel_times() const { return ktimes_; }

    int register_batch(int npairs, const double* const* src, const int64_t* ns, const double* const* tgt,
                       const int64_t* nt, bool on_device, int method, const se3icp_params& prm,
                       se3icp_result* out, hipStream_t user_stream, const se3icp_report_options* ropts = nullptr,
                       se3icp_report* reports = nullptr);
    int register_sweep(int npairs, const double* const* src, const int64_t* ns, const double* const* tgt,
                       const int64_t* nt, bool on_device, int method, int nvariants, const se3icp_params* variants,
                       int max_group, se3icp_result* out, hipStream_t user_stream,
                       const se3icp_report_options* ropts = nullptr, se3icp_report* reports = nullptr);

    int register_graph(int nclouds, const double* const* xyz, const int64_t* npts, int npairs, const int32_t* src,
                       const int32_t* tgt, bool on_device, int method, const se3icp_params& prm, int sharing,
                       se3icp_result* out, hipStream_t user_stream, const se3icp_report_options* ropts = nullptr,
                       se3icp_report* reports = nullptr);
    const int64_t* graph_stats() const { return graph_stats_; }

    int knn_self(const double* xyz, int64_t n, int k, int32_t* idx);
    int toldi_frames(const double* xyz, int64_t n, int k, double* frames);
    int estimate_normals(const double* xyz, int64_t n, int k, double* normals);
    int nn(const double* query, int64_t nq, const double* data, int64_t nd, int dim, int32_t* idx, double* d2,
           int32_t* num_rechecked);

  private:
    struct CloudReq {
        const double* in = nullptr;
        int64_t n = 0;
        CloudSetup st{};
    };
    struct TreeBufs {
        DevBuf perm, pos, vec, vec64, vec64a, blo, bhi, lo, hi, scr, vecT;
        int L = 0;
        explicit TreeBufs(std::vector<DevBuf*>& o)
            : perm(o), pos(o), vec(o), vec64(o), vec64a(o), blo(o), bhi(o), lo(o), hi(o), scr(o), vecT(o) {}
    };
    int init();
    template <class T>
    T* ensure(DevBuf& b, size_t count);
    int alloc_points(int64_t ntot, int kmax, bool knn_list = false);
    int build_tree(int D, const float* vec, hipStream_t s, const double* vec64 = nullptr);
    struct Call {
        se3icp_trace* tr = nullptr;
        hipStream_t s = nullptr;
    };
    int open_call(int args, int64_t nslots, int rest, hipStream_t user_stream, Call* c);
    int upload_clouds(const std::vector<CloudReq>& clouds, bool on_device, hipStream_t s);
    int host_centroids(hipStream_t s, std::vector<double>* cen);
    int setup_clouds(const std::vector<CloudReq>& clouds, bool on_device, bool pairs, bool normalize, double scale_pre,
                     hipStream_t s);
    int setup_knn(hipStream_t s);
    int setup_pairs_shared(const std::vector<CloudReq>& clouds, const MethodPlan& mp, double scale_pre, hipStream_t s);
    int select_by_class(const GraphPlan& plan, const std::vector<CloudSetup>& batch, const MethodPlan& mp,
                        hipStream_t s);
    int setup_chunks(int npairs, hipStream_t s);
    int run_pairs(const MethodPlan& mp, int npairs, const int64_t* ns, const int64_t* nt,
                  const se3icp_params* vprm, int pairs_per_variant, bool sweep, const Call& c, se3icp_result* out,
                  const se3icp_report_options* ropts, se3icp_report* reports);
    int prepare_pairs(int npairs, const int64_t* ns, const int64_t* nt, hipStream_t s);
    struct ReportReq {
        const se3icp_report_options* opts;
        se3icp_report* out;
    };
    int run_loop(int npairs, const int64_t* ns, int kind, int est, const se3icp_params* vprm, int pairs_per_variant,
                 bool sweep, se3icp_trace* tr, se3icp_result* out, hipStream_t s, const ReportReq* rq = nullptr);
    int queue_report(int npairs, const int64_t* ns, const ReportReq& rq, hipStream_t s);
    int read_lrf_stats();
    int sync_stream(hipStream_t s);
    View view() const;

    int dev_;
    bool ok_ = false;
    bool profile_ = false;
    std::mutex mu_;
    hipStream_t stream_ = nullptr;
    KernelTimes ktimes_;

    int nclouds_ = 0, npairs_ = 0;
    int64_t ntot_ = 0;
    int ld_ = 0, kmax_ = 1, nwork_ = 0, tree_L_ = 0;
    int chunk_level_ = 0, nchunks_ = 0;
    bool knn_list_ = false;
    bool nn_trace_ = false;
    int lrf_exact_only_ = 0;
    bool nn_events_ = true;
    int batch_sharing_ = 0;
    se3icp_trace* trace_ = nullptr;
    int record_trace(se3icp_trace* tr, int it, int& phase_of_it, hipStream_t s);
    double trace_prev_[kStatCols] = {};
    std::vector<CloudDev> h_clouds_;
    std::vector<CloudSetup> h_setup_;
    std::vector<BlockWork> h_work_;
    std::vector<int32_t> h_wb_, h_wn_;
    std::vector<ChunkWork> h_chunks_;
    std::vector<const double*> h_inptr_;

    std::vector<DevBuf*> bufs_;
    std::vector<PinnedMem*> pins_;
    DevBuf d_clouds_{bufs_}, d_setup_{bufs_}, d_pairs_{bufs_}, d_cloud_of_{bufs_}, d_inptr_{bufs_}, d_in_{bufs_},
        d_xyz64_{bufs_}, d_xyz32_{bufs_}, d_fr64_{bufs_}, d_fr32_{bufs_}, d_nrm64_{bufs_}, d_tgeo_{bufs_},
        d_conf64_{bufs_}, d_knn_{bufs_}, d_corr_idx_{bufs_}, d_corr_dist_{bufs_}, d_flag_count_{bufs_},
        d_gcost_{bufs_}, d_cls_{bufs_}, d_trim_key_{bufs_}, d_red_partial_{bufs_}, d_red_out_{bufs_}, d_work_{bufs_},
        d_wb_{bufs_}, d_wn_{bufs_}, d_chunks_{bufs_}, d_partial_{bufs_}, d_centers_{bufs_}, d_rechecked_{bufs_},
        d_keys0_{bufs_}, d_vals1_{bufs_}, d_sort_tmp_{bufs_}, d_stats_{bufs_}, d_qlist_{bufs_}, d_qcount_{bufs_},
        d_hist_{bufs_}, d_cert_{bufs_}, d_sqlist_{bufs_}, d_state_{bufs_}, d_trim_cand_{bufs_}, d_trim_ctr_{bufs_},
        d_scales_{bufs_}, d_trim_hist_{bufs_},
        d_lrf_fb_{bufs_}, d_lrf_fbn_{bufs_},
        d_big_d_{bufs_}, d_big_i_{bufs_},
        d_raw_{bufs_}, d_sweep_w_{bufs_},
        d_rep_partial_{bufs_}, d_rep_out_{bufs_}, d_rep_off_{bufs_}, d_rep_idx_{bufs_}, d_rep_dist_{bufs_};
    TreeBufs t3_{bufs_}, t12_{bufs_};
    DevBuf g_raw_xyz_{bufs_}, g_raw_conf_{bufs_}, g_seg_{bufs_}, g_chunks_{bufs_};
    DevBuf d_share_hash_{bufs_}, d_share_pairs_{bufs_}, d_share_same_{bufs_};
    Pinned<uint64_t> h_share_hash_{pins_};
    Pinned<int32_t> h_share_same_{pins_};
    Pinned<CloudSetup> h_share_setup_{pins_};
    std::vector<SharePair> share_pairs_;
    std::vector<CloudSetup> share_setup_;
    std::vector<CloudSetup> sel_batch_, sel_run_;
    std::vector<ChunkWork> sel_chunks_;
    std::vector<GraphSeg> sel_seg_;
    int64_t graph_stats_[9] = {};
    Pinned<PairDev> h_pairs_{pins_};
    Pinned<double> h_red_{pins_}, h_partial_{pins_};
    Pinned<int32_t> h_rechecked_{pins_};
    Pinned<double> h_hist_{pins_};
    Pinned<double> h_rep_{pins_};
    std::vector<int64_t> h_rep_off_;
    Pinned<PairState> h_state_{pins_};
    int32_t* h_phase_ = nullptr;
    int32_t* d_phase_ = nullptr;
    size_t h_phase_cap_ = 0;
    Pinned<unsigned long long> h_lrf_stats_{pins_};
    Pinned<unsigned long long> h_loop_stats_{pins_};
    bool lrf_stats_pending_ = false;
    hipEvent_t ev_[16];
    static constexpr int kLoopRing = 4, kLoopEv = 7;
    hipEvent_t loop_ev_[kLoopRing * kLoopEv];
    int loop_flags_[kLoopRing] = {};
    bool loop_detail_[kLoopRing] = {};
};

Engine* engine_for(int device);

}
```

se3-icp_amd/csrc/graph.hpp:

```cpp
#pragma once
#include <hip/hip_runtime.h>
#include <stdint.h>

#include <cmath>
#include <cstring>
#include <map>
#include <utility>
#include <vector>

namespace se3icp {

constexpr int kGraphSharingMin = 0, kGraphSharingMax = 3;
enum GraphStat : int {
    GS_CLOUDS = 0,
    GS_USES,
    GS_CLASSES,
    GS_FULL,
    GS_ADOPTED,
    GS_REJ_ORDER,
    GS_REJ_GAP,
    GS_NO_LIST,
    GS_BYTES_UPLOADED,
    GS_COUNT
};

inline double graph_pair_scale(double scale_pre, double r_src, double r_tgt) {
    const double rmax = std::fmax(r_src, r_tgt);
    return scale_pre * (1.0 / rmax);
}

struct GraphClass {
    int32_t cloud;
    int32_t k_nrm;
    int32_t n_uses;
    int32_t nrm_from;
    double norm_center[3];
    double norm_scale;
    double f32_center[3];
};

struct GraphPlan {
    std::vector<int32_t> use_class;
    std::vector<GraphClass> classes;
};

struct GraphUse {
    int32_t cloud;
    int32_t k_nrm;
    double norm_center[3];
    double norm_scale;
    double f32_center[3];
};

inline void graph_plan_uses(int32_t n_uses, const GraphUse* use, bool normalize, bool dedupe, GraphPlan* plan) {
    struct Key {
        int32_t cloud;
        uint64_t b[7];
        bool operator<(const Key& o) const {
            if (cloud != o.cloud) return cloud < o.cloud;
            return std::memcmp(b, o.b, sizeof(b)) < 0;
        }
    };
    std::map<Key, int32_t> seen;
    plan->use_class.assign((size_t)n_uses, -1);
    plan->classes.clear();
    for (int32_t u = 0; u < n_uses; ++u) {
        GraphClass g{};
        g.cloud = use[u].cloud;
        g.k_nrm = use[u].k_nrm;
        g.n_uses = 1;
        g.norm_scale = use[u].norm_scale;
        for (int a = 0; a < 3; ++a) {
            g.norm_center[a] = use[u].norm_center[a];
            g.f32_center[a] = use[u].f32_center[a];
        }
        Key k{};
        k.cloud = g.cloud;
        std::memcpy(&k.b[0], &g.norm_scale, 8);
        std::memcpy(&k.b[1], g.f32_center, 24);
        std::memcpy(&k.b[4], g.norm_center, 24);
        int32_t id = -1;
        if (dedupe) {
            auto it = seen.find(k);
            if (it != seen.end()) id = it->second;
        }
        if (id < 0) {
            id = (int32_t)plan->classes.size();
            plan->classes.push_back(g);
            if (dedupe) seen[k] = id;
        } else {
            GraphClass& h = plan->classes[id];
            h.k_nrm = h.k_nrm > g.k_nrm ? h.k_nrm : g.k_nrm;
            h.n_uses++;
        }
        plan->use_class[u] = id;
    }
    std::map<int32_t, int32_t> owner;
    for (int32_t k = 0; k < (int32_t)plan->classes.size(); ++k) {
        GraphClass& g = plan->classes[k];
        g.nrm_from = k;
        if (normalize || !dedupe || g.k_nrm <= 0) continue;
        auto it = owner.find(g.cloud);
        if (it == owner.end()) owner[g.cloud] = k;
        else if (plan->classes[it->second].k_nrm == g.k_nrm) g.nrm_from = it->second;
    }
}

inline void graph_plan(int32_t n_pairs, const int32_t* src, const int32_t* tgt, bool normalize, double scale_pre,
                       const double* center, const double* radius, int k_nrm_src, int k_nrm_tgt, bool dedupe,
                       GraphPlan* plan) {
    std::vector<GraphUse> use(2 * (size_t)n_pairs);
    for (int32_t p = 0; p < n_pairs; ++p) {
        const double scale = normalize ? graph_pair_scale(scale_pre, radius[src[p]], radius[tgt[p]]) : 1.0;
        for (int side = 0; side < 2; ++side) {
            const int32_t c = side == 0 ? src[p] : tgt[p];
            GraphUse& g = use[2 * (size_t)p + side];
            g.cloud = c;
            g.k_nrm = side == 0 ? k_nrm_src : k_nrm_tgt;
            g.norm_scale = scale;
            for (int a = 0; a < 3; ++a) {
                g.norm_center[a] = normalize ? center[3 * c + a] : 0.0;
                g.f32_center[a] = normalize ? 0.0 : center[3 * tgt[p] + a];
            }
        }
    }
    graph_plan_uses(2 * n_pairs, use.data(), normalize, dedupe, plan);
}

constexpr int kBatchSharingMin = 0, kBatchSharingMax = 2;

inline bool share_any_equal_n(int32_t n_slots, const int64_t* n) {
    std::map<int64_t, int32_t> seen;
    for (int32_t u = 0; u < n_slots; ++u)
        if (++seen[n[u]] > 1) return true;
    return false;
}

inline int32_t share_candidates(int32_t n_slots, const int64_t* n, const uint64_t* hash, std::vector<int32_t>* first) {
    std::map<std::pair<int64_t, uint64_t>, int32_t> seen;
    first->assign((size_t)n_slots, -1);
    int32_t cand = 0;
    for (int32_t u = 0; u < n_slots; ++u) {
        auto it = seen.find({n[u], hash[u]});
        if (it == seen.end()) {
            seen[{n[u], hash[u]}] = u;
            (*first)[u] = u;
        } else {
            (*first)[u] = it->second;
            ++cand;
        }
    }
    return cand;
}

inline int32_t share_clouds(int32_t n_slots, const int32_t* first, const int32_t* same, std::vector<int32_t>* cloud) {
    cloud->assign((size_t)n_slots, -1);
    int32_t nc = 0;
    for (int32_t u = 0; u < n_slots; ++u)
        (*cloud)[u] = (first[u] != u && same[u]) ? (*cloud)[first[u]] : nc++;
    return nc;
}

inline int graph_check(int32_t n_clouds, const int64_t* n_pts, const int64_t* off, int32_t n_pairs,
                       const int32_t* src, const int32_t* tgt, int method, int n_methods, int32_t sharing,
                       const void* results) {
    if (n_clouds <= 0 || n_pairs <= 0 || (!n_pts && !off) || !src || !tgt || !results) return -1;
    if (sharing < kGraphSharingMin || sharing > kGraphSharingMax) return -1;
    if (method < 0 || method >= n_methods) return -2;
    for (int32_t p = 0; p < n_pairs; ++p)
        if (src[p] < 0 || src[p] >= n_clouds || tgt[p] < 0 || tgt[p] >= n_clouds) return -1;
    for (int32_t p = 0; p < n_pairs; ++p)
        for (int side = 0; side < 2; ++side) {
            const int32_t c = side == 0 ? src[p] : tgt[p];
            const int64_t n = n_pts ? n_pts[c] : off[c + 1] - off[c];
            if (n <= 0) return -3;
        }
    return 0;
}

struct View;
struct ChunkWork;
struct GraphSeg { int32_t src_off; int32_t src_cloud; int32_t nrm_off; int32_t frames; };
struct SharePair { int32_t slot; int32_t first; };
void launch_share_hash(const View& v, unsigned long long* hash, hipStream_t s);
void launch_share_compare(const View& v, const SharePair* pairs, int npairs, int32_t* same, hipStream_t s);
void launch_graph_normalize(const View& v, const ChunkWork* chunks, int nchunks, const GraphSeg* seg,
                            const double* raw_xyz64, const double* raw_conf64, hipStream_t s);
void launch_graph_share(const View& v, const ChunkWork* chunks, int nchunks, const GraphSeg* seg, hipStream_t s);

}
```

se3-icp_amd/csrc/k_lrf8.hip:

```cpp
#include <hip/hip_runtime.h>

#include <cfloat>
#include <climits>

#include "devmath.hpp"
#include "knn_util.hpp"
#include "tree.hpp"
#include "view.hpp"
#include "wave.hpp"

namespace se3icp {

namespace {

using namespace knn;

#ifndef SE3ICP_LRF8_WAVES
#define SE3ICP_LRF8_WAVES 4
#endif
constexpr int kW = SE3ICP_LRF8_WAVES;
constexpr int kQ = 8;
#ifndef SE3ICP_LRF8_CAP
#define SE3ICP_LRF8_CAP 192
#endif
constexpr int kCap = SE3ICP_LRF8_CAP;
#ifndef SE3ICP_LRF8_FILL
#define SE3ICP_LRF8_FILL SE3ICP_LRF8_CAP
#endif
constexpr int kFill = SE3ICP_LRF8_FILL;
constexpr int kStride = kCap + 4;
static_assert(((kStride / 4) & 1) == 1, "an odd number of 16-B slots per list");
constexpr int kLeaves = 64;
constexpr unsigned kIdBits = 0xfffu;
constexpr unsigned kAll = 0x7f7fffffu;
constexpr unsigned kPad = 0xffffffffu;

enum Park8 {
    P8_SUM = 0,
    P8_R = 21, P8_KK = 22, P8_GP = 23, P8_FLAGS = 24, P8_K = 25, P8_NTOP = 26, P8_ZN = 27,
    P8_W = 30,
    P8_N = 31
};
constexpr int kParkAt = 128;
static_assert(kCap >= kParkAt + 2 * P8_N && kStride >= kCap, "the park overlays the list tail");

__device__ __forceinline__ unsigned gx(unsigned x, int m) {
    switch (m) {
    case 1: return (unsigned)__builtin_amdgcn_mov_dpp((int)x, 0xB1, 0xF, 0xF, true);
    case 2: return (unsigned)__builtin_amdgcn_mov_dpp((int)x, 0x4E, 0xF, 0xF, true);
    case 3: return (unsigned)__builtin_amdgcn_mov_dpp((int)x, 0x1B, 0xF, 0xF, true);
    case 4: return (unsigned)__builtin_amdgcn_ds_swizzle((int)x, 0x101F);
    case 7: return (unsigned)__builtin_amdgcn_mov_dpp((int)x, 0x141, 0xF, 0xF, true);
    default: return (unsigned)__shfl_xor((int)x, m, 64);
    }
}
__device__ __forceinline__ double gxd(double x, int m) {
    const unsigned long long u = (unsigned long long)__double_as_longlong(x);
    const unsigned lo = gx((unsigned)u, m), hi = gx((unsigned)(u >> 32), m);
    return __longlong_as_double((long long)(((unsigned long long)hi << 32) | lo));
}

__device__ __forceinline__ unsigned med3u(unsigned a, unsigned b, unsigned x) {
    unsigned r;
    asm("v_med3_u32 %0, %1, %2, %3" : "=v"(r) : "v"(a), "v"(b), "v"(x));
    return r;
}

template <int PER, int KK, int JD>
__device__ __forceinline__ void stage8(unsigned (&k)[PER], int l) {
    if constexpr (JD == 0) {
        if constexpr (KK <= PER) {
#pragma unroll
            for (int s = 0; s < PER; ++s) {
                const int t = s ^ (KK - 1);
                if (s < t) {
                    const unsigned a = k[s], b = k[t];
                    k[s] = min(a, b);
                    k[t] = max(a, b);
                }
            }
        } else {
            constexpr int lm = KK / PER - 1;
            const unsigned x = (l & (KK / PER / 2)) == 0 ? 0u : ~0u;
#pragma unroll
            for (int s = 0; s < PER / 2; ++s) {
                const int t = PER - 1 - s;
                const unsigned a = gx(k[t], lm), b = gx(k[s], lm);
                k[s] = med3u(k[s], a, x);
                k[t] = med3u(k[t], b, x);
            }
        }
    } else if constexpr (JD < PER) {
#pragma unroll
        for (int s = 0; s < PER; ++s) {
            if ((s & JD) == 0) {
                const int t = s | JD;
                const unsigned a = k[s], b = k[t];
                k[s] = min(a, b);
                k[t] = max(a, b);
            }
        }
    } else {
        constexpr int lm = JD / PER;
        const unsigned x = (l & lm) == 0 ? 0u : ~0u;
#pragma unroll
        for (int s = 0; s < PER; ++s) k[s] = med3u(k[s], gx(k[s], lm), x);
    }
}
template <int PER, int N, int KK = 2, int JD = 0>
__device__ __forceinline__ void net8(unsigned (&k)[PER], int l) {
    stage8<PER, KK, JD>(k, l);
    constexpr int next_jd = JD == 0 ? KK / 4 : JD / 2;
    if constexpr (next_jd > 0) net8<PER, N, KK, next_jd>(k, l);
    else if constexpr (KK < N) net8<PER, N, KK * 2, 0>(k, l);
}
template <int PER>
__device__ __forceinline__ void sort8(unsigned (&k)[PER], int l) {
    net8<PER, 8 * PER>(k, l);
}

template <int PER>
__device__ __forceinline__ void load_head(const unsigned* list, int len, int l, unsigned (&k)[PER]) {
#pragma unroll
    for (int q = 0; q < PER / 4; ++q) {
        const int e0 = l * PER + 4 * q;
        uint4 x = make_uint4(kPad, kPad, kPad, kPad);
        if (e0 < len) x = *reinterpret_cast<const uint4*>(list + e0);
        k[4 * q] = x.x;
        k[4 * q + 1] = e0 + 1 < len ? x.y : kPad;
        k[4 * q + 2] = e0 + 2 < len ? x.z : kPad;
        k[4 * q + 3] = e0 + 3 < len ? x.w : kPad;
    }
}
template <int PER>
__device__ __forceinline__ void store_head(unsigned* list, int len, int l, const unsigned (&k)[PER], unsigned add = 0u) {
#pragma unroll
    for (int q = 0; q < PER / 4; ++q) {
        const int e0 = l * PER + 4 * q;
        if (e0 < len)
            *reinterpret_cast<uint4*>(list + e0) =
                make_uint4(k[4 * q] + add, k[4 * q + 1] + add, k[4 * q + 2] + add, k[4 * q + 3] + add);
    }
}
template <int PER = 16>
__device__ __forceinline__ void sort_head(unsigned* list, int len, int l) {
    unsigned k[PER];
    load_head<PER>(list, len, l, k);
    sort8<PER>(k, l);
    __builtin_amdgcn_wave_barrier();
    store_head<PER>(list, len, l, k);
    __builtin_amdgcn_wave_barrier();
}
template <int PER = 16>
__device__ __forceinline__ void sort_run(unsigned* list, int len, int l) {
    unsigned k[PER];
#pragma unroll
    for (int s = 0; s < PER; ++s) {
        const int e = l * PER + s;
        k[s] = e < len ? list[e] : kPad;
    }
    sort8<PER>(k, l);
    __builtin_amdgcn_wave_barrier();
#pragma unroll
    for (int s = 0; s < PER; ++s) {
        const int e = l * PER + s;
        if (e < len) list[e] = k[s];
    }
    __builtin_amdgcn_wave_barrier();
}
__device__ __forceinline__ float f32_err3(float d, float S) {
    const float u = 5.9604645e-08f;
    return 1.25f * (2.f * u * S * sqrtf(fmaxf(d, 0.f)) + 6.f * u * d + 4.f * u * u * S * S) + 1e-30f;
}
__device__ __forceinline__ unsigned widen_bound(unsigned t, float S) {
    if (t >= 0x7f800000u) return kAll;
    const float b = __uint_as_float(t);
    return min((__float_as_uint(fmaf(2.02f, f32_err3(b, S), b)) + 2u) | kIdBits, kAll);
}
__device__ __forceinline__ int upper_count(const unsigned* A, int n, unsigned t) {
    int lo = 0, hi = n;
    while (lo < hi) {
        const int m = (lo + hi) >> 1;
        if (A[m] <= t) lo = m + 1; else hi = m;
    }
    return lo;
}
__device__ __forceinline__ unsigned kth_of_two(const unsigned* A, int na, const unsigned* B, int nb, int r) {
    int lo = max(0, r + 1 - nb), hi = min(r + 1, na);
    while (lo < hi) {
        const int i = (lo + hi) >> 1;
        if (A[i] < B[r - i]) lo = i + 1; else hi = i;
    }
    const int j = r + 1 - lo;
    return max(lo > 0 ? A[lo - 1] : 0u, j > 0 ? B[j - 1] : 0u);
}
__device__ __forceinline__ uint3 tighten_group_sorted(unsigned* lists, int g, int l, int nbg, int mv, int nmax, int Kw,
                                                      bool presort, int tail_per, float S) {
    unsigned* list = lists + g * kStride;
    if (presort) {
        mv = min(nbg, 128);
        sort_head<16>(list, mv, l);
    }
    const int nb = nbg - mv;
    unsigned* B = list + mv;
    if (tail_per == 8) sort_run<8>(B, nb, l);
    else if (tail_per == 16) sort_run<16>(B, nb, l);
    const unsigned tg = nbg >= Kw ? widen_bound(kth_of_two(list, mv, B, nb, Kw - 1) | kIdBits, S) : kAll;
    const int ka = upper_count(list, mv, tg), kb = upper_count(B, nb, tg);
    const int kept = ka + kb;
    if (__ballot(kept > 128) == 0ull) {
        unsigned k[16];
        load_head<16>(list, ka, l, k);
#pragma unroll
        for (int s = 0; s < 16; ++s) {
            const int e = l * 16 + s;
            if (e >= 128 - kb) k[s] = B[127 - e];
        }
        __builtin_amdgcn_wave_barrier();
        stage8<16, 128, 64>(k, l);
        stage8<16, 128, 32>(k, l);
        stage8<16, 128, 16>(k, l);
        stage8<16, 128, 8>(k, l);
        stage8<16, 128, 4>(k, l);
        stage8<16, 128, 2>(k, l);
        stage8<16, 128, 1>(k, l);
        store_head<16>(list, kept, l, k);
        __builtin_amdgcn_wave_barrier();
        return make_uint3(tg, (unsigned)kept, (unsigned)kept);
    }
    unsigned keep_n = 0;
    for (int r0 = 0; r0 < nmax; r0 += 8) {
        const int e = r0 + l;
        const unsigned ent = e < nbg ? list[e] : kPad;
        const bool keep = ent <= tg;
        const unsigned long long m = __ballot(keep);
        const unsigned gm = (unsigned)(m >> (8 * g)) & 0xffu;
        __builtin_amdgcn_wave_barrier();
        if (keep) list[(int)keep_n + __popc(gm & ((1u << l) - 1u))] = ent;
        keep_n += (unsigned)__popc(gm);
        __builtin_amdgcn_wave_barrier();
    }
    return make_uint3(tg, keep_n, 0u);
}

struct p3 { double x, y, z; };
__device__ __forceinline__ p3 ld3(const double4* __restrict__ P4, int i) {
    const double2 xy = *reinterpret_cast<const double2*>(P4 + i);
    const double z = reinterpret_cast<const double*>(P4 + i)[2];
    return p3{xy.x, xy.y, z};
}

__device__ __forceinline__ bool final_group(unsigned* lists, const int* leaf_slot, const double4* __restrict__ P4,
                                            const int32_t* __restrict__ perm, double qx, double qy, double qz, int off,
                                            int g, int l, int nbg, int mv, int fmode, int lim) {
    unsigned* list = lists + g * kStride;
    unsigned long long k[16];
    bool unsorted = false;
    {
        unsigned k32[16];
        if (fmode == 0) {
            load_head<16>(list, nbg, l, k32);
            sort8<16>(k32, l);
        } else {
            const int nb = nbg - mv;
            unsigned* B = list + mv;
            if (fmode == 1) sort_run<8>(B, nb, l);
            load_head<16>(list, mv, l, k32);
            if (fmode == 1) {
#pragma unroll
                for (int s = 0; s < 16; ++s) {
                    const int e = l * 16 + s;
                    if (e >= 128 - nb) k32[s] = B[127 - e];
                }
                __builtin_amdgcn_wave_barrier();
                stage8<16, 128, 64>(k32, l);
                stage8<16, 128, 32>(k32, l);
                stage8<16, 128, 16>(k32, l);
                stage8<16, 128, 8>(k32, l);
                stage8<16, 128, 4>(k32, l);
                stage8<16, 128, 2>(k32, l);
                stage8<16, 128, 1>(k32, l);
            }
        }
#pragma unroll
        for (int s = 0; s < 16; ++s) {
            const int e = l * 16 + s;
            unsigned long long x = ~0ull;
            if (e < nbg) {
                const unsigned id = k32[s] & kIdBits;
                const int slot = leaf_slot[id >> 6] + (int)(id & 63u);
                const p3 p = ld3(P4, slot);
                const unsigned key = __float_as_uint((float)l2_3(qx, qy, qz, p.x, p.y, p.z));
                x = ((unsigned long long)key << 32) | (unsigned)(slot - off);
            }
            k[s] = x;
        }
    }
    auto ce = [](unsigned long long& a, unsigned long long& b) __attribute__((always_inline)) {
        const bool sw = b < a;
        const unsigned long long lo = sw ? b : a, hi = sw ? a : b;
        a = lo;
        b = hi;
    };
    const int me = (int)(threadIdx.x & 63);
    auto next_first = [&]() __attribute__((always_inline)) {
        return ((unsigned long long)(unsigned)__shfl((int)(unsigned)(k[0] >> 32), me + 1, 64) << 32) |
               (unsigned)__shfl((int)(unsigned)k[0], me + 1, 64);
    };
#pragma unroll
    for (int s = 0; s < 16; s += 2) ce(k[s], k[s + 1]);
    {
#pragma unroll
        for (int s = 1; s + 1 < 16; s += 2) ce(k[s], k[s + 1]);
        const unsigned long long nx = next_first();
        const unsigned long long pv = ((unsigned long long)(unsigned)__shfl((int)(unsigned)(k[15] >> 32), me - 1, 64) << 32) |
                                      (unsigned)__shfl((int)(unsigned)k[15], me - 1, 64);
        if (l < 7 && nx < k[15]) k[15] = nx;
        if (l > 0 && k[0] < pv) k[0] = pv;
    }
#pragma unroll
    for (int s = 0; s < 16; s += 2) ce(k[s], k[s + 1]);
    const unsigned long long nx = next_first();
#pragma unroll
    for (int s = 0; s + 1 < 16; ++s) unsorted |= k[s + 1] < k[s];
    unsorted |= (l < 7) && nx < k[15];
    unsigned tall = 0u;
#pragma unroll
    for (int s = 0; s + 1 < 16; ++s) {
        const int e = l * 16 + s;
        if ((int)(e + 1 < nbg) & (int)((unsigned)(k[s] >> 32) == (unsigned)(k[s + 1] >> 32))) tall |= 1u << s;
    }
    {
        const int e = l * 16 + 15;
        if ((int)(l < 7) & (int)(e + 1 < nbg) & (int)((unsigned)(k[15] >> 32) == (unsigned)(nx >> 32))) tall |= 1u << 15;
    }
    const int nlim = lim - 1 - l * 16;
    unsigned tied = tall & (nlim >= 16 ? 0xffffu : nlim > 0 ? (1u << nlim) - 1u : 0u);
    const unsigned tprev = (unsigned)__shfl((int)tall, me - 1, 64), tnext = (unsigned)__shfl((int)tall, me + 1, 64);
    const unsigned tall_lo = (tall << 1) | (l > 0 ? (tprev >> 15) & 1u : 0u);
    const unsigned tall_hi = (tall >> 1) | (l < 7 ? (tnext & 1u) << 15 : 0u);
    const unsigned isolated = ~(tall_lo | tall_hi);
    __builtin_amdgcn_wave_barrier();
    {
        unsigned sl[16];
#pragma unroll
        for (int s = 0; s < 16; ++s) sl[s] = (unsigned)k[s];
        store_head<16>(list, nbg, l, sl, (unsigned)off);
    }
    __builtin_amdgcn_wave_barrier();
    bool bad = unsorted;
    while (tied) {
        const int sb = __builtin_ctz(tied);
        const int e = l * 16 + sb;
        tied &= tied - 1u;
        const int a = (int)list[e], b = (int)list[e + 1];
        const p3 pa = ld3(P4, a), pb = ld3(P4, b);
        const double da = l2_3(qx, qy, qz, pa.x, pa.y, pa.z), db = l2_3(qx, qy, qz, pb.x, pb.y, pb.z);
        const bool wrong = (bool)((int)(da > db) | ((int)(da == db) & (int)(perm[a] > perm[b])));
        bad |= (bool)((int)(e + 2 >= lim) & (int)((tall_hi >> sb) & 1u));
        if (wrong) {
            if ((isolated >> sb) & 1u) {
                list[e] = (unsigned)b;
                list[e + 1] = (unsigned)a;
            } else {
                bad = true;
            }
        } else if (!((isolated >> sb) & 1u)) {
            bad |= da != db;
        }
    }
    const bool ok = !(bool)(unsigned)((__ballot(bad) >> (8 * g)) & 0xffull);
    return ok;
}

#ifdef SE3ICP_PROF
#define PROF8_NOW(t) const unsigned long long t = __builtin_readcyclecounter()
#define PROF8_ADD(acc, a, b) acc += (b) - (a)
#else
#define PROF8_NOW(t) do {} while (0)
#define PROF8_ADD(acc, a, b) do {} while (0)
#endif

static_assert(kW >= 2 && kW * kQ <= 64, "the per-block epilogue: waves 0 and 1, a lane per query");

__global__ __launch_bounds__(64 * kW) __attribute__((amdgpu_waves_per_eu(kCap <= 192 ? 6 : (kCap <= 224 ? 5 : 4)))) void k_lrf8(
    View v, const int32_t* __restrict__ cloud_of, const CloudSetup* __restrict__ setup,
    const CloudDev* __restrict__ clouds, const float* __restrict__ tlo, const float* __restrict__ thi,
    const double4* __restrict__ P4, const int32_t* __restrict__ wave_base, int w_lo, int nwaves,
    int32_t* __restrict__ fb_list, int32_t* __restrict__ fb_count) {
    __shared__ __attribute__((aligned(16))) unsigned s_list[kW][kQ][kStride];
    auto park_of = [&](int w, int j) __attribute__((always_inline)) {
        return reinterpret_cast<double*>(&s_list[w][j][kParkAt]);
    };
    __shared__ int s_leaf[kW][kLeaves];
    __shared__ __attribute__((aligned(16))) float s_q[kW][3 * kQ];
    const int lane = threadIdx.x & 63, wid = __builtin_amdgcn_readfirstlane(threadIdx.x >> 6);
    const int g = lane >> 3, l = lane & 7;
    const int bid = xcd_block(blockIdx.x, gridDim.x);
    const TreeRef T = v.t3;
    const int first_leaf = (1 << T.L) - 1;
    unsigned* lists = &s_list[wid][0][0];
    int* leaves = s_leaf[wid];
    unsigned n_leaves = 0, n_sel = 0, n_cand = 0, n_q = 0;
#ifdef SE3ICP_PROF
    unsigned long long c_scan = 0, c_tight = 0, c_sums = 0, c_epi = 0;
    unsigned n_tover = 0, n_tend = 0;
    unsigned long long fb_cause = 0;
#define PROF8_FB(field) fb_cause += 1ull << (16 * (field))
#else
#define PROF8_FB(field) do {} while (0)
#endif
    PROF8_NOW(t_a0);

    const int wv = __builtin_amdgcn_readfirstlane(w_lo + bid * kW + wid);
    int mode = 0, c = 0, w0 = 0, qn = 0;
    CloudSetup st{};
    CloudDev cl{0, 0};
    int K = 0, Kw = 0;
    if (wv < nwaves) {
        int lo = 0, hi = v.nclouds - 1;
        while (lo < hi) {
            const int mid = (lo + hi + 1) >> 1;
            if (wave_base[mid] <= wv) lo = mid; else hi = mid - 1;
        }
        c = lo;
        cl = clouds[c];
        st = setup[c];
        K = st.k_knn;
        w0 = cl.off + kQ * (wv - wave_base[c]);
        qn = min(kQ, cl.off + cl.n - w0);
        if (K > 0 && qn > 0) {
            Kw = min(K, cl.n);
            mode = (qn == kQ && Kw <= 128) ? 1 : 2;
        }
    }
    bool fb_wave = mode == 2;
    unsigned Tq[kQ], nbq[kQ];
#pragma unroll
    for (int j = 0; j < kQ; ++j) { Tq[j] = kAll; nbq[j] = 0u; }
    auto group_len = [&]() __attribute__((always_inline)) {
        int x = 0;
#pragma unroll
        for (int j = 0; j < kQ; ++j) asm volatile("v_writelane_b32 %0, %1, %2" : "+v"(x) : "s"(nbq[j]), "n"(8 * j));
        return (unsigned)__shfl(x, lane & ~7, 64);
    };
    int mvv = 0;
    float* qv = s_q[wid];
    float fqlo[3] = {0.f, 0.f, 0.f}, fqhi[3] = {0.f, 0.f, 0.f};
    int nlist = 0;
    const int n = cl.n;
    float s_norm = 0.f;
    if (mode == 1) {
        const float fx = lane < kQ ? T.tvec[w0 + lane] : 0.f;
        const float fy = lane < kQ ? T.tvec[v.ld + w0 + lane] : 0.f;
        const float fz = lane < kQ ? T.tvec[2 * (size_t)v.ld + w0 + lane] : 0.f;
        if (lane < kQ) {
            qv[lane] = fx;
            qv[kQ + lane] = fy;
            qv[2 * kQ + lane] = fz;
        }
        {
            const float* rlo = tlo + (size_t)c * T.nnodes * 3;
            const float* rhi = thi + (size_t)c * T.nnodes * 3;
            float r2 = 0.f;
#pragma unroll
            for (int a = 0; a < 3; ++a) r2 += fmaxf(rlo[a] * rlo[a], rhi[a] * rhi[a]);
            s_norm = 2.f * sqrtf(r2) * 1.0001f;
        }
        __builtin_amdgcn_wave_barrier();
        fqlo[0] = fqhi[0] = __shfl(fx, 0, 64);
        fqlo[1] = fqhi[1] = __shfl(fy, 0, 64);
        fqlo[2] = fqhi[2] = __shfl(fz, 0, 64);
#pragma unroll
        for (int j = 1; j < kQ; ++j) {
            const float a = __shfl(fx, j, 64), b = __shfl(fy, j, 64), d = __shfl(fz, j, 64);
            fqlo[0] = fminf(fqlo[0], a); fqhi[0] = fmaxf(fqhi[0], a);
            fqlo[1] = fminf(fqlo[1], b); fqhi[1] = fmaxf(fqhi[1], b);
            fqlo[2] = fminf(fqlo[2], d); fqhi[2] = fmaxf(fqhi[2], d);
        }
        n_q = kQ;
    }

    auto tighten = [&]() __attribute__((always_inline)) {
        ++n_sel;
        unsigned nmax = 0;
#pragma unroll
        for (int j = 0; j < kQ; ++j) nmax = max(nmax, nbq[j]);
        __builtin_amdgcn_wave_barrier();
        int dmax = 0;
        bool anyz = false;
#pragma unroll
        for (int j = 0; j < kQ; ++j) {
            const int mj = __builtin_amdgcn_readlane(mvv, 8 * j);
            dmax = max(dmax, (int)nbq[j] - mj);
            anyz |= mj == 0;
        }
        const bool presort = anyz || dmax > 128;
        const int tail_per = presort ? (nmax <= 128 ? 0 : (nmax <= 192 ? 8 : 16)) : (dmax == 0 ? 0 : dmax <= 64 ? 8 : 16);
        const uint3 r3 = tighten_group_sorted(lists, g, l, (int)group_len(), mvv, (int)nmax, Kw, presort, tail_per, s_norm);
        mvv = (int)r3.z;
        __builtin_amdgcn_wave_barrier();
#pragma unroll
        for (int j = 0; j < kQ; ++j) {
            Tq[j] = (unsigned)__builtin_amdgcn_readlane((int)r3.x, 8 * j);
            nbq[j] = (unsigned)__builtin_amdgcn_readlane((int)r3.y, 8 * j);
        }
    };

    auto scan_leaf = [&](int i, int part) __attribute__((always_inline)) -> bool {
        if (nlist >= kLeaves) { fb_wave = true; PROF8_FB(0); return true; }
        const int li = nlist++;
        ++n_leaves;
        const int a = __builtin_amdgcn_readfirstlane(tree_first(n, T.L, i));
        const int b = __builtin_amdgcn_readfirstlane(tree_first(n, T.L, i + 1));
        if (lane == 0) leaves[li] = cl.off + a;
        const bool valid = (bool)((int)(lane < b - a) & (int)(part == 0 || (part == 1) == (lane < 32)));
        const int slot = cl.off + a + (valid ? lane : 0);
        const unsigned id = (unsigned)((li << 6) | lane);
        unsigned ent[kQ];
        unsigned long long m[kQ];
        bool over = false;
        float dq[kQ];
        {
            typedef float f2 __attribute__((ext_vector_type(2)));
            const float px = valid ? T.tvec[slot] : INFINITY;
            const float py = valid ? T.tvec[v.ld + slot] : INFINITY;
            const float pz = valid ? T.tvec[2 * (size_t)v.ld + slot] : INFINITY;
            const f2* qf2 = reinterpret_cast<const f2*>(qv);
            const f2 pxx = f2{px, px}, pyy = f2{py, py}, pzz = f2{pz, pz};
            auto pk_sub = [](f2 a, f2 b) __attribute__((always_inline)) {
                f2 r;
                asm("v_pk_add_f32 %0, %1, %2 neg_lo:[0,1] neg_hi:[0,1]" : "=v"(r) : "v"(a), "v"(b));
                return r;
            };
#pragma unroll
            for (int jp = 0; jp < kQ / 2; ++jp) {
                const f2 ex = pk_sub(qf2[jp], pxx), ey = pk_sub(qf2[kQ / 2 + jp], pyy), ez = pk_sub(qf2[kQ + jp], pzz);
                f2 s2 = ex * ex;
                s2 = __builtin_elementwise_fma(ey, ey, s2);
                s2 = __builtin_elementwise_fma(ez, ez, s2);
                dq[2 * jp] = s2.x;
                dq[2 * jp + 1] = s2.y;
            }
        }
#pragma unroll
        for (int j = 0; j < kQ; ++j) {
            ent[j] = (__float_as_uint(dq[j]) & ~kIdBits) | id;
            m[j] = __ballot(ent[j] <= Tq[j]);
            over |= nbq[j] + (unsigned)__popcll(m[j]) > (unsigned)kCap;
        }
        if (over) {
            --nlist;
            --n_leaves;
            return false;
        }
#pragma unroll
        for (int j = 0; j < kQ; ++j) {
            if (ent[j] <= Tq[j]) {
                const int at = (int)nbq[j] + __builtin_amdgcn_mbcnt_hi((unsigned)(m[j] >> 32), __builtin_amdgcn_mbcnt_lo((unsigned)m[j], 0u));
                lists[j * kStride + at] = ent[j];
            }
            nbq[j] += (unsigned)__popcll(m[j]);
        }
        __builtin_amdgcn_wave_barrier();
        return true;
    };

    if (mode == 1) {
        const int lf0 = tree_node_of(w0 - cl.off, n, T.L), lf1 = tree_node_of(w0 + kQ - 1 - cl.off, n, T.L);
        const int nleaf = 1 << T.L;
        int s_lo = lf0, s_hi = lf1;
        auto thr_f = [&]() __attribute__((always_inline)) {
            unsigned tm = 0u;
#pragma unroll
            for (int j = 0; j < kQ; ++j) tm = max(tm, Tq[j]);
            return __uint_as_float(f32_up_bits((double)__uint_as_float(tm) * (1.0 + 2e-6)));
        };
        auto box_lb = [&](int h) __attribute__((always_inline)) {
            const float* lo = tlo + ((size_t)c * T.nnodes + h) * 3;
            const float* hi = thi + ((size_t)c * T.nnodes + h) * 3;
            float s = 0.f;
#pragma unroll
            for (int a = 0; a < 3; ++a) {
                const float e = fmaxf(fmaxf(lo[a] - fqhi[a], fqlo[a] - hi[a]), 0.f);
                s += e * e;
            }
            return s;
        };
        const int sh = T.L > 6 ? 6 : T.L;
        const int nA = 1 << (T.L - sh), firstA = nA - 1;
        int stage = 0, nxt = lf0, c0 = 0, l0 = 0;
        bool up = true, haveA = false;
        float lbA = INFINITY, lbL = INFINITY;
        OutwardBits itA(0ull, 0), itL(0ull, 0);
        int cur = -1, part = 0;
        bool do_tighten = false, retried = false;
        float tf = INFINITY;
        while (!fb_wave) {
            if (do_tighten) {
                PROF8_NOW(t_t0);
                tighten();
                PROF8_NOW(t_t1);
                PROF8_ADD(c_tight, t_t0, t_t1);
                do_tighten = false;
                tf = thr_f();
#if defined(SE3ICP_LRF8_CUT) && SE3ICP_LRF8_CUT == 4
                if (stage == 2) break;
#endif
            }
            if (cur >= 0) {
#if defined(SE3ICP_LRF8_CUT) && SE3ICP_LRF8_CUT == 5
                if (stage >= 2) { cur = -1; part = 0; ++n_leaves; continue; }
#endif
                if (scan_leaf(cur, part)) {
                    if (part == 1) part = 2;
                    else { cur = -1; part = 0; }
                    retried = false;
                } else if (!retried && (int)nbq[0] >= Kw) {
                    do_tighten = true;
                    retried = true;
#ifdef SE3ICP_PROF
                    ++n_tover;
#endif
                } else if (part == 0) {
                    part = 1;
                    retried = false;
                } else {
                    fb_wave = true;
                    PROF8_FB(1);
                }
                continue;
            }
            int leaf = -1;
            if (stage == 0) {
                leaf = nxt++;
                if (nxt > lf1) stage = 1;
            } else if (stage == 1) {
                const bool more_hi = s_hi < nleaf - 1, more_lo = s_lo > 0;
                const int cand = (more_hi && (up || !more_lo)) ? s_hi + 1 : s_lo - 1;
                const int csz = (more_hi || more_lo) ? tree_first(n, T.L, cand + 1) - tree_first(n, T.L, cand) : 0;
                if ((more_hi || more_lo) && ((int)nbq[0] < Kw || (int)nbq[0] + csz <= kFill)) {
                    leaf = cand;
                    if (cand > s_hi) s_hi = cand; else s_lo = cand;
                    up = !up;
                } else {
                    do_tighten = true;
                    stage = 2;
                    continue;
                }
            } else if (stage == 2) {
                if (!haveA) {
                    if (c0 >= nA) {
                        unsigned nmax = 0;
#pragma unroll
                        for (int j = 0; j < kQ; ++j) nmax = max(nmax, nbq[j]);
                        if (nmax > 128 && !retried) {
#ifdef SE3ICP_PROF
                            ++n_tend;
#endif
                            do_tighten = true;
                            retried = true;
                            continue;
                        }
                        if (nmax > 128) { fb_wave = true; PROF8_FB(2); }
                        break;
                    }
                    const int ai = c0 + lane;
                    lbA = ai < nA ? box_lb(firstA + ai) : INFINITY;
                    itA = OutwardBits(__ballot(lbA <= tf), (lf0 >> sh) - c0);
                    haveA = true;
                }
                const int j = itA.next();
                if (j < 0) { haveA = false; c0 += 64; continue; }
                if (!(__int_as_float(__builtin_amdgcn_readlane(__float_as_int(lbA), j)) <= tf)) continue;
                l0 = (c0 + j) << sh;
                const int li = l0 + lane;
                lbL = INFINITY;
                if ((int)(lane < (1 << sh)) & ((int)(li < s_lo) | (int)(li > s_hi))) lbL = box_lb(first_leaf + li);
                itL = OutwardBits(__ballot(lbL <= tf), lf0 - l0);
                stage = 3;
                continue;
            } else {
                const int t = itL.next();
                if (t < 0) { stage = 2; continue; }
                if (!(__int_as_float(__builtin_amdgcn_readlane(__float_as_int(lbL), t)) <= tf)) continue;
                leaf = l0 + t;
            }
            cur = leaf;
        }
    }
    __builtin_amdgcn_wave_barrier();

    PROF8_NOW(t_a1);
#if defined(SE3ICP_LRF8_CUT) && (SE3ICP_LRF8_CUT == 1 || SE3ICP_LRF8_CUT == 4 || SE3ICP_LRF8_CUT == 5)
    if (lane == 0 && n_leaves == 12345u) v.stats[0] = nlist;
    return;
#endif
    PROF8_ADD(c_scan, t_a0, t_a1);
    const int kl = st.k_lrf, kn_want = st.k_nrm;
    const bool want_t = kl > 0, want_n = kn_want > 0;
    bool fb_q = fb_wave;
    const int nbg = (int)group_len();
    const int nTop = min(Kw, nbg);
    const int kk = min(kl, nTop), kn = min(kn_want, nTop);
    const int wq = w0 + g;
    p3 qg{0.0, 0.0, 0.0};
    if (mode == 1) qg = ld3(P4, wq);
    if (mode == 1 && !fb_wave) {
        __builtin_amdgcn_wave_barrier();
        int fmode = 0;
        {
            int dmax = 0;
            bool anyz = false;
#pragma unroll
            for (int j = 0; j < kQ; ++j) {
                const int mj = __builtin_amdgcn_readlane(mvv, 8 * j);
                dmax = max(dmax, (int)nbq[j] - mj);
                anyz |= mj == 0;
            }
            fmode = anyz || dmax > 64 ? 0 : dmax == 0 ? 2 : 1;
        }
        const bool exact = final_group(lists, leaves, P4, T.perm, qg.x, qg.y, qg.z, cl.off, g, l, nbg, mvv, fmode,
                                       min(nbg, max(kk, kn) + 1));
        fb_q = (bool)((int)!exact | (int)(nTop < Kw));
        n_cand += (unsigned)nbg;
#ifdef SE3ICP_PROF
        fb_cause += (unsigned long long)__popcll(__ballot((int)fb_q & (int)(l == 0) & (int)(g < qn))) << 48;
#endif
    }
    if ((int)(mode != 0) & (int)fb_q & (int)(l == 0) & (int)(g < qn)) {
        const int at = atomicAdd(fb_count, 1);
        fb_list[at] = wq;
        atomicAdd(v.stats + kStatCols * (wv & 63) + 6, 1ull);
    }
    const bool mine = (bool)((int)(mode == 1) & (int)!fb_q);

#if defined(SE3ICP_LRF8_CUT) && SE3ICP_LRF8_CUT == 2
    if (lane == 0 && n_cand == 12345u) v.stats[0] = n_cand;
    return;
#endif
    const unsigned* rl = lists + g * kStride;
    double* pj = park_of(wid, g);
    {
        double x[12];
#pragma unroll
        for (int i = 0; i < 12; ++i) x[i] = 0.0;
        double Rf = 0.0;
        if ((int)mine & (int)want_t) {
            const int rz = kk / 3;
            const int hi = min(rz, kk - 1);
            p3 pn = ld3(P4, (int)rl[max(min(1 + l, hi), 0)]);
            for (int rk = 1 + l; rk <= hi; rk += 8) {
                const p3 p = pn;
                pn = ld3(P4, (int)rl[min(rk + 8, hi)]);
                const double vx = p.x - qg.x, vy = p.y - qg.y, vz = p.z - qg.z;
                if (rk < rz) { x[0] += vx; x[1] += vy; x[2] += vz; }
                x[3] += vx; x[4] += vy; x[5] += vz;
                x[6] += vx * vx; x[7] += vx * vy; x[8] += vx * vz;
                x[9] += vy * vy; x[10] += vy * vz; x[11] += vz * vz;
            }
            if (l == 0) {
                const p3 f = ld3(P4, (int)rl[kk - 1]);
                const double fdx = qg.x - f.x, fdy = qg.y - f.y, fdz = qg.z - f.z;
                Rf = sqrt(fdx * fdx + fdy * fdy + fdz * fdz);
            }
        }
#pragma unroll
        for (int i = 0; i < 12; ++i) {
            x[i] += gxd(x[i], 1);
            x[i] += gxd(x[i], 2);
            x[i] += gxd(x[i], 4);
        }
        __builtin_amdgcn_wave_barrier();
        if ((int)(l == 0) & (int)mine) {
#pragma unroll
            for (int i = 0; i < 12; ++i) pj[P8_SUM + i] = x[i];
            pj[P8_R] = Rf;
        }
    }
    {
        double x[9];
#pragma unroll
        for (int i = 0; i < 9; ++i) x[i] = 0.0;
        if ((int)mine & (int)want_n) {
            p3 pn = ld3(P4, (int)rl[max(min(l, kn - 1), 0)]);
            for (int r = l; r < kn; r += 8) {
                const p3 p = pn;
                pn = ld3(P4, (int)rl[min(r + 8, kn - 1)]);
                const double px = p.x, py = p.y, pz = p.z;
                x[0] += px; x[1] += py; x[2] += pz;
                x[3] += px * px; x[4] += px * py; x[5] += px * pz;
                x[6] += py * py; x[7] += py * pz; x[8] += pz * pz;
            }
        }
#pragma unroll
        for (int i = 0; i < 9; ++i) {
            x[i] += gxd(x[i], 1);
            x[i] += gxd(x[i], 2);
            x[i] += gxd(x[i], 4);
        }
        __builtin_amdgcn_wave_barrier();
        if (l == 0) {
            const int flags = mine ? ((want_t ? 1 : 0) | (want_n ? 2 : 0)) : 0;
            pj[P8_FLAGS] = (double)flags;
            if (mine) {
#pragma unroll
                for (int i = 0; i < 9; ++i) pj[P8_SUM + 12 + i] = x[i];
                pj[P8_KK] = (double)kk;
                pj[P8_GP] = (double)(cl.off + T.perm[wq]);
                pj[P8_K] = (double)K;
                pj[P8_NTOP] = (double)nTop;
                pj[P8_W] = (double)wq;
            }
        }
        __builtin_amdgcn_wave_barrier();
    }
    PROF8_NOW(t_a2);
    PROF8_ADD(c_sums, t_a1, t_a2);
    unsigned long long* ctr = v.stats + kStatCols * (wv & 63);
    if (lane == 0) {
        atomicAdd(ctr + 0, (unsigned long long)n_q);
        atomicAdd(ctr + 1, (unsigned long long)n_leaves);
        atomicAdd(ctr + 2, (unsigned long long)n_sel);
        atomicAdd(ctr + 4, (unsigned long long)n_cand);
    }

#if defined(SE3ICP_LRF8_CUT) && SE3ICP_LRF8_CUT == 3
    return;
#endif
    auto toldi_eig = [&](double* pb) __attribute__((always_inline)) {
        const p3 q = ld3(P4, (int)pb[P8_W]);
        const double rz = (double)((int)pb[P8_KK] / 3);
        const double q3[3] = {q.x, q.y, q.z};
        double cq[3], S[3];
#pragma unroll
        for (int a = 0; a < 3; ++a) {
            cq[a] = (pb[P8_SUM + a] - q3[a]) / rz;
            S[a] = pb[P8_SUM + 3 + a];
        }
        const double* M = pb + P8_SUM + 6;
        const int ia[6] = {0, 0, 0, 1, 1, 2}, ib[6] = {0, 1, 2, 1, 2, 2};
        double c6[6];
#pragma unroll
        for (int k = 0; k < 6; ++k)
            c6[k] = M[k] - S[ia[k]] * cq[ib[k]] - cq[ia[k]] * S[ib[k]] + rz * cq[ia[k]] * cq[ib[k]];
        const d3 zn = jacobi_smallest_evec(c6[0], c6[1], c6[2], c6[3], c6[4], c6[5]);
        pb[P8_ZN] = zn.x;
        pb[P8_ZN + 1] = zn.y;
        pb[P8_ZN + 2] = zn.z;
    };
    auto normal_eig = [&](const double* pb) __attribute__((always_inline)) {
        const int wb = (int)pb[P8_W];
        const int cc = cloud_of[wb];
        const int knb = min(setup[cc].k_nrm, (int)pb[P8_NTOP]);
        double n6[6] = {1, 0, 0, 1, 0, 1};
        if (knb >= 3) {
            double cu[9];
#pragma unroll
            for (int i = 0; i < 9; ++i) cu[i] = pb[P8_SUM + 12 + i] / (double)knb;
            n6[0] = cu[3] - cu[0] * cu[0];
            n6[1] = cu[4] - cu[0] * cu[1];
            n6[2] = cu[5] - cu[0] * cu[2];
            n6[3] = cu[6] - cu[1] * cu[1];
            n6[4] = cu[7] - cu[1] * cu[2];
            n6[5] = cu[8] - cu[2] * cu[2];
        }
        d3 nm = fast_eigen3x3(n6[0], n6[1], n6[2], n6[3], n6[4], n6[5]);
        if (sqrt(dot3(nm, nm)) == 0.0) nm = d3{0, 0, 1};
        const int gp = (int)pb[P8_GP];
        v.nrm64[gp] = nm.x;
        v.nrm64[v.ld + gp] = nm.y;
        v.nrm64[2 * (size_t)v.ld + gp] = nm.z;
    };
    __syncthreads();
    if (wid <= 1) {
        double* pb = park_of(lane < kW * kQ ? lane / kQ : 0, lane % kQ);
        const int b_flags = lane < kW * kQ ? (int)pb[P8_FLAGS] : 0;
        if ((b_flags & 1) && wid == 0) toldi_eig(pb);
        if ((b_flags & 2) && wid == 1) normal_eig(pb);
    }
    __syncthreads();

    {
        const int flags = (int)pj[P8_FLAGS];
        double x6[6] = {0.0, 0.0, 0.0, 0.0, 0.0, 0.0};
        if (flags & 1) {
            const double nx = pj[P8_ZN], ny = pj[P8_ZN + 1], nz = pj[P8_ZN + 2];
            const double R = pj[P8_R];
            const int kkq = (int)pj[P8_KK];
            p3 pn = ld3(P4, (int)rl[max(min(1 + l, kkq - 1), 0)]);
            for (int r = 1 + l; r < kkq; r += 8) {
                const p3 p = pn;
                pn = ld3(P4, (int)rl[min(r + 8, kkq - 1)]);
                const double vx = p.x - qg.x, vy = p.y - qg.y, vz = p.z - qg.z;
                x6[0] += vx; x6[1] += vy; x6[2] += vz;
                const double an = nx * vx + ny * vy + nz * vz;
                const double rr = R - sqrt(vx * vx + vy * vy + vz * vz);
                const double wgt = (rr * rr) * (an * an);
                x6[3] += wgt * vx; x6[4] += wgt * vy; x6[5] += wgt * vz;
            }
        }
#pragma unroll
        for (int i = 0; i < 6; ++i) {
            x6[i] += gxd(x6[i], 1);
            x6[i] += gxd(x6[i], 2);
            x6[i] += gxd(x6[i], 4);
        }
        __builtin_amdgcn_wave_barrier();
        if ((int)(l == 0) & (int)((flags & 1) != 0)) {
#pragma unroll
            for (int i = 0; i < 6; ++i) pj[P8_SUM + i] = x6[i];
        }
    }
    __syncthreads();
    if (wid == 0) {
        const double* pb = park_of(lane < kW * kQ ? lane / kQ : 0, lane % kQ);
        const int b_flags = lane < kW * kQ ? (int)pb[P8_FLAGS] : 0;
        if (b_flags & 1) {
            const int w = (int)pb[P8_W];
            const CloudSetup sw = setup[cloud_of[w]];
            const p3 q = ld3(P4, w);
            d3 nrm{pb[P8_ZN], pb[P8_ZN + 1], pb[P8_ZN + 2]};
            if (nrm.x * pb[P8_SUM] + nrm.y * pb[P8_SUM + 1] + nrm.z * pb[P8_SUM + 2] < 0.0)
                nrm = d3{-nrm.x, -nrm.y, -nrm.z};
            const d3 zax = nrm;
            const d3 accs{pb[P8_SUM + 3], pb[P8_SUM + 4], pb[P8_SUM + 5]};
            d3 xax = accs - dot3(accs, zax) * zax;
            xax = (1.0 / sqrt(dot3(xax, xax))) * xax;
            const d3 yax = cross3(zax, xax);
            const double al = sw.alpha, be = sw.beta;
            const double f12[12] = {al * xax.x, al * xax.y, al * xax.z, al * yax.x, al * yax.y, al * yax.z,
                                    al * zax.x, al * zax.y, al * zax.z, be * q.x, be * q.y, be * q.z};
            store_frame_rows(v.fr64, v.fr32, (int)pb[P8_GP], f12, sw.cf_target, q.x, q.y, q.z);
        }
    }
#ifdef SE3ICP_PROF
    PROF8_NOW(t_a3);
    PROF8_ADD(c_epi, t_a2, t_a3);
    if (lane == 0) {
        atomicAdd(ctr + 8, c_scan - c_tight);
        atomicAdd(ctr + 9, c_tight);
        atomicAdd(ctr + 10, c_sums);
        atomicAdd(ctr + 11, c_epi);
        atomicAdd(ctr + 3, (unsigned long long)n_tover);
        atomicAdd(ctr + 7, (unsigned long long)n_tend);
        atomicAdd(ctr + 5, fb_cause);
    }
#endif
}

}

void launch_lrf8(const View& v, const int32_t* wave_base, int w_lo, int w_hi, int32_t* fb_list, int32_t* fb_count,
                 hipStream_t s) {
    const int nb = (w_hi - w_lo + kW - 1) / kW;
    if (nb <= 0) return;
    hipLaunchKernelGGL(k_lrf8, dim3(nb), dim3(64 * kW), 0, s, v, v.cloud_of, v.setup, v.clouds, v.t3.lo, v.t3.hi,
                       v.t3.tpt64, wave_base, w_lo, w_hi, fb_list, fb_count);
}

}
```

se3-icp_amd/csrc/view.hpp:

```cpp
#pragma once
#include <hip/hip_runtime.h>
#include <stdint.h>

#include "common.hpp"

namespace se3icp {

struct CloudSetup {
    int32_t k_knn;
    int32_t k_lrf;
    int32_t k_nrm;
    int32_t want_cov;
    int32_t want_conf;
    int32_t is_target;
    int32_t cf_target;
    int32_t _pad;
    double alpha, beta;
    double norm_center[3];
    double norm_scale;
    double f32_center[3];
};

struct TreeRef {
    int32_t L;
    int32_t GL;
    int32_t nnodes;
    const int32_t* perm;
    const int32_t* pos;
    const float* tvec;
    const double* tvec64;
    const double4* tpt64;
    const float* lo;
    const float* hi;
};

struct alignas(16) NNCert {
    float d1, l2;
    int32_t iter, j;
    double t[3];
    float margin;
    int32_t _pad;
};
static_assert(sizeof(NNCert) == 48, "three 16-B words");

struct View {
    int32_t ld;
    int32_t npts;
    int32_t nclouds;
    int32_t npairs;
    int32_t kmax;
    CloudDev* clouds;
    CloudSetup* setup;
    PairDev* pairs;
    int32_t* cloud_of;
    const double* const* in_ptr;
    double* xyz64;
    float* xyz32;
    double* fr64;
    float* fr32;
    double* nrm64;
    double* conf64;
    double* tgeo;
    int32_t* knn;
    int32_t* corr_idx;
    float* corr_dist;
    unsigned long long* stats;
    int32_t* flag_count;
    uint64_t* trim_key;
    unsigned long long* trim_cand;
    unsigned* trim_ctr;
    unsigned* trim_hist;
    double* red_partial;
    double* red_out;
    const BlockWork* work;
    int32_t nwork;
    int32_t* pair_rechecked;
    TreeRef t3, t12;
    int32_t chunk_level;
    int32_t nchunks;
    int32_t* qlist;
    int32_t* qcount;
    int32_t* sq_list;
    const double* hist;
    NNCert* cert;
    uint32_t* gcost;
    int32_t* cls;
};

constexpr int kChunk = 2048;
struct ChunkWork { int32_t cloud; int32_t p0; };

void launch_ingest(const View& v, const ChunkWork* chunks, int nchunks, double* partial , hipStream_t s);
void launch_radius(const View& v, const ChunkWork* chunks, int nchunks, const double* centers ,
                   double* partial , hipStream_t s);
void launch_normalize(const View& v, const ChunkWork* chunks, int nchunks, double* partial ,
                      hipStream_t s);
void launch_pair_centers(const View& v, const ChunkWork* chunks, int nchunks, const double* partial, double* centers,
                         hipStream_t s);
void launch_pair_scales(const View& v, const ChunkWork* chunks, int nchunks, const double* partial,
                        const double* centers, double scale_pre, double* scales, hipStream_t s);
void launch_pair_norms(const View& v, int nnodes3, int nnodes12, const double* scales, double* state_sf,
                       int state_stride, hipStream_t s);
void launch_lrf(const View& v, int write_knn, hipStream_t s);
void launch_lrf_list(const View& v, const int32_t* qlist, const int32_t* qcount, hipStream_t s, int qpw = 0);
void launch_lrf8(const View& v, const int32_t* wave_base, int w_lo, int w_hi, int32_t* fb_list, int32_t* fb_count,
                 hipStream_t s);
int knn_big_cap(int kw_max);
int knn_big_blocks(int cap, int nq);
void launch_knn_big(const View& v, int write_knn, int k_min, const int32_t* qlist, const int32_t* qcount, int nblocks,
                    double* scratch_d, int32_t* scratch_i, int cap, hipStream_t s);

void launch_nn_prep(const View& v, int32_t* publish, hipStream_t s);
void nn_prof_report();
void trim_prof_report();
#ifdef SE3ICP_PROF
double nn_prep_span();
void nn_wave_report(int it);
#endif
void launch_nn(const View& v, int D, hipStream_t s);
size_t nn_cls_words(int nchunks);
void launch_trim(const View& v, hipStream_t s);
void launch_geo_rows(const View& v, hipStream_t s);
struct PairState;
void launch_reduce(const View& v, const int32_t* pair_wb, const int32_t* pair_wn, PairState* state, double* hist,
                   int32_t* next_phase, hipStream_t s);

}
```

se3-icp_amd/se3icp/__init__.py:

```python
from ._lib import (METHODS, Params, Result, Se3IcpError, default_params, device_count, load,
                   method_id, status_string)
from .io import read_ply_xyz, write_ply_xyz
from .registration import (DeviceBatchRunner, IterativeSE3Registration, PairResult, PipelinedBatchRunner,
                           cli_params,
                           estimate_normals,
                           kitti_params, knn_self, last_kernel_times, set_nn_events, set_profiling, lounge_params,
                           nearest_neighbors,
                           register_batch, register_batch_device, register_batch_traced, toldi_frames,
                           alpha_grid, register_sweep, register_sweep_device, register_sweep_traced, sweep_params,
                           PairReport, register_batch_report, register_batch_report_device, register_sweep_report,
                           register_sweep_report_device,
                           expand_edges, last_graph_stats, register_graph, register_graph_device,
                           register_graph_report, register_graph_traced, register_sequence, sequence_edges,
                           set_batch_sharing)
from ._lib import Report, ReportOptions

__all__ = [
    "IterativeSE3Registration", "register_batch", "register_batch_device", "DeviceBatchRunner", "PipelinedBatchRunner", "register_batch_traced", "toldi_frames", "knn_self",
    "estimate_normals", "nearest_neighbors", "default_params", "cli_params", "kitti_params", "lounge_params",
    "read_ply_xyz", "write_ply_xyz", "METHODS", "Se3IcpError",
    "register_sweep", "register_sweep_device", "register_sweep_traced", "alpha_grid", "sweep_params",
    "PairReport", "Report", "ReportOptions", "register_batch_report", "register_batch_report_device",
    "register_sweep_report", "register_sweep_report_device",
    "register_graph", "register_sequence", "sequence_edges", "expand_edges", "register_graph_device",
    "register_graph_report", "register_graph_traced", "last_graph_stats",
    "set_batch_sharing",
]
```

se3-icp_amd/se3icp/_lib.py:

```python
from __future__ import annotations

import ctypes as C
import os

_PKG = os.path.dirname(os.path.abspath(__file__))
_ROOT = os.path.dirname(_PKG)
LIB_PATH = os.environ.get("SE3ICP_LIB") or os.path.join(_ROOT, "lib", "libse3icp.so")

OK = 0
ERR_INVALID_ARG = -1
ERR_INVALID_METHOD = -2
ERR_EMPTY_CLOUD = -3
ERR_K_TOO_LARGE = -4
ERR_NO_DEVICE = -5
ERR_HIP = -6
ERR_NONFINITE = -7
ERR_OUT_OF_MEMORY = -8
ERR_INTERNAL = -9

METHODS = ["pt2pt", "pt2pl", "gicp", "se3_pt2pt", "se3_pt2pl", "se3_gicp", "se3_gicp_with_cf",
           "se3_pure_pt2pt", "se3_pure_pt2pl", "se3_pure_gicp"]

EXPORTED_SYMBOLS = [
    "se3icp_abi_version", "se3icp_status_string", "se3icp_method_from_name", "se3icp_method_name",
    "se3icp_default_params", "se3icp_device_count",
    "se3icp_registration_new", "se3icp_registration_free", "se3icp_set_source_cloud", "se3icp_set_target_cloud",
    "se3icp_params_of", "se3icp_run_icp", "se3icp_run_se3_icp", "se3icp_run_se3_icp_with_cf", "se3icp_run_se3_pure",
    "se3icp_get_result",
    "se3icp_register_batch", "se3icp_register_batch_device", "se3icp_register",
    "se3icp_register_sweep", "se3icp_register_sweep_device",
    "se3icp_register_graph", "se3icp_register_graph_device", "se3icp_register_graph_report",
    "se3icp_register_graph_report_device", "se3icp_last_graph_stats", "se3icp_set_batch_sharing",
    "se3icp_report_version", "se3icp_register_batch_report", "se3icp_register_batch_report_device",
    "se3icp_register_sweep_report", "se3icp_register_sweep_report_device",
    "se3icp_request_report", "se3icp_get_report",
    "se3icp_toldi_frames", "se3icp_knn_self", "se3icp_estimate_normals", "se3icp_nn",
    "se3icp_synthetic_pairs", "se3icp_synthetic_reference", "se3icp_synthetic_reference_device",
    "se3icp_random_downsample",
    "se3icp_set_profiling", "se3icp_last_kernel_times", "se3icp_last_kernel_times_n", "se3icp_set_trace", "se3icp_set_lrf_exact",
    "se3icp_set_nn_events",
    "se3icp_cc_rot_3d", "se3icp_cc_angular_error_so3", "se3icp_cc_angular_error_so3_alt",
    "se3icp_cc_error_filterreg", "se3icp_cc_rot2euler", "se3icp_cc_avg_eul_error",
    "se3icp_cc_evaluate_lrf_quality", "se3icp_cc_evaluate_trajectory",
    "se3icp_cc_read_trajectory", "se3icp_cc_read_kitti_poses", "se3icp_cc_read_redwood_log",
    "se3icp_cc_write_trajectory", "se3icp_cc_write_redwood_log",
]


class Params(C.Structure):
    _fields_ = [
        ("max_num_iterations", C.c_int32),
        ("max_num_se3_iterations", C.c_int32),
        ("number_of_nn_for_LRF", C.c_int32),
        ("_reserved", C.c_int32),
        ("mse", C.c_double),
        ("mse_switch_error", C.c_double),
        ("estimated_overlap", C.c_double),
        ("alpha_rot", C.c_double),
        ("beta_transl", C.c_double),
        ("scale_preprocessing", C.c_double),
    ]


class Result(C.Structure):
    _fields_ = [
        ("T", C.c_double * 16),
        ("num_iterations", C.c_int32),
        ("num_pure_se3_iterations", C.c_int32),
        ("status", C.c_int32),
        ("num_rechecked", C.c_int32),
        ("scaling_factor", C.c_double),
        ("time_setup_ms", C.c_double),
        ("time_loop_ms", C.c_double),
        ("time_se3_correspondence_search_ms", C.c_double),
        ("time_before_pure_icp_ms", C.c_double),
    ]


STOP_CONVERGED = 0
STOP_MAX_ITERATIONS = 1
STOP_MAX_SE3_ITERATIONS = 2
STOP_RUNAWAY = 3
STOP_REASONS = ["converged", "max_iterations", "max_se3_iterations", "runaway"]


class ReportOptions(C.Structure):
    _fields_ = [
        ("max_correspondence_distance", C.c_double),
        ("corr_idx", C.c_void_p),
        ("corr_dist", C.c_void_p),
        ("outputs_on_device", C.c_int32),
        ("_reserved", C.c_int32),
    ]


class Report(C.Structure):
    _fields_ = [
        ("fitness", C.c_double),
        ("inlier_rmse", C.c_double),
        ("information", C.c_double * 36),
        ("final_mse", C.c_double),
        ("final_mse_change", C.c_double),
        ("n_inliers", C.c_int64),
        ("switched", C.c_int32),
        ("stop_reason", C.c_int32),
    ]


class Trace(C.Structure):
    _fields_ = [
        ("pair", C.c_int32),
        ("max_iters", C.c_int32),
        ("corr_idx", C.POINTER(C.c_int32)),
        ("corr_dist", C.POINTER(C.c_float)),
        ("trim_key", C.POINTER(C.c_uint64)),
        ("T", C.POINTER(C.c_double)),
        ("mse", C.POINTER(C.c_double)),
        ("phase", C.POINTER(C.c_int32)),
        ("iters_recorded", C.c_int32),
        ("_reserved", C.c_int32),
    ]


GRAPH_STATS = ["clouds", "uses", "classes", "classes_full", "adopted", "rejected_order", "rejected_gap", "no_list",
               "bytes_uploaded"]


class Se3IcpError(RuntimeError):
    def __init__(self, code: int, what: str = ""):
        self.code = code
        msg = status_string(code) if _lib is not None else str(code)
        super().__init__(f"se3icp error {code} ({msg}){': ' + what if what else ''}")


_lib = None


def load():
    global _lib
    if _lib is not None:
        return _lib
    if not os.path.exists(LIB_PATH):
        raise ImportError(f"HIP engine library not built: {LIB_PATH} is missing "
                          "(run __graft_entry__.build() or `make -C se3-icp_amd`)")
    L = C.CDLL(LIB_PATH)
    dp, ip = C.POINTER(C.c_double), C.POINTER(C.c_int32)
    vp = C.c_void_p
    L.se3icp_abi_version.restype = C.c_int
    L.se3icp_status_string.restype = C.c_char_p
    L.se3icp_status_string.argtypes = [C.c_int]
    L.se3icp_method_from_name.argtypes = [C.c_char_p]
    L.se3icp_method_name.restype = C.c_char_p
    L.se3icp_method_name.argtypes = [C.c_int]
    L.se3icp_default_params.argtypes = [C.POINTER(Params)]
    L.se3icp_device_count.restype = C.c_int
    L.se3icp_registration_new.restype = vp
    L.se3icp_registration_free.argtypes = [vp]
    L.se3icp_set_source_cloud.argtypes = [vp, dp, C.c_int64]
    L.se3icp_set_target_cloud.argtypes = [vp, dp, C.c_int64]
    L.se3icp_params_of.restype = C.POINTER(Params)
    L.se3icp_params_of.argtypes = [vp]
    L.se3icp_run_icp.argtypes = [vp, C.c_char_p]
    L.se3icp_run_se3_icp.argtypes = [vp, C.c_char_p]
    L.se3icp_run_se3_icp_with_cf.argtypes = [vp]
    L.se3icp_run_se3_pure.argtypes = [vp, C.c_char_p]
    L.se3icp_get_result.argtypes = [vp, C.POINTER(Result)]
    L.se3icp_register_batch.argtypes = [C.c_int, C.c_int32, C.POINTER(dp), C.POINTER(C.c_int64), C.POINTER(dp),
                                        C.POINTER(C.c_int64), C.c_int, C.POINTER(Params), C.POINTER(Result)]
    L.se3icp_register_batch_device.argtypes = [C.c_int, C.c_int32, vp, C.POINTER(C.c_int64), vp,
                                               C.POINTER(C.c_int64), C.c_int, C.POINTER(Params), C.POINTER(Result), vp]
    L.se3icp_register_sweep.argtypes = [C.c_int, C.c_int32, C.POINTER(dp), C.POINTER(C.c_int64), C.POINTER(dp),
                                        C.POINTER(C.c_int64), C.c_int, C.c_int32, C.POINTER(Params), C.c_int32,
                                        C.POINTER(Result)]
    L.se3icp_register_sweep_device.argtypes = [C.c_int, C.c_int32, vp, C.POINTER(C.c_int64), vp,
                                               C.POINTER(C.c_int64), C.c_int, C.c_int32, C.POINTER(Params), C.c_int32,
                                               C.POINTER(Result), vp]
    rop, rep = C.POINTER(ReportOptions), C.POINTER(Report)
    L.se3icp_report_version.restype = C.c_int
    L.se3icp_register_batch_report.argtypes = L.se3icp_register_batch.argtypes + [rop, rep]
    L.se3icp_register_batch_report_device.argtypes = L.se3icp_register_batch_device.argtypes + [rop, rep]
    L.se3icp_register_sweep_report.argtypes = L.se3icp_register_sweep.argtypes + [rop, rep]
    L.se3icp_register_sweep_report_device.argtypes = L.se3icp_register_sweep_device.argtypes + [rop, rep]
    L.se3icp_register_graph.argtypes = [C.c_int, C.c_int32, C.POINTER(dp), C.POINTER(C.c_int64), C.c_int32, ip, ip,
                                        C.c_int, C.POINTER(Params), C.c_int32, C.POINTER(Result)]
    L.se3icp_register_graph_device.argtypes = [C.c_int, C.c_int32, vp, C.POINTER(C.c_int64), C.c_int32, ip, ip,
                                               C.c_int, C.POINTER(Params), C.c_int32, C.POINTER(Result), vp]
    L.se3icp_register_graph_report.argtypes = L.se3icp_register_graph.argtypes + [rop, rep]
    L.se3icp_register_graph_report_device.argtypes = L.se3icp_register_graph_device.argtypes + [rop, rep]
    L.se3icp_last_graph_stats.argtypes = [C.c_int, C.POINTER(C.c_int64), C.c_int]
    L.se3icp_request_report.argtypes = [vp, rop]
    L.se3icp_get_report.argtypes = [vp, rep]
    L.se3icp_register.argtypes = [C.c_int, dp, C.c_int64, dp, C.c_int64, C.c_int, C.POINTER(Params),
                                  C.POINTER(Result)]
    L.se3icp_toldi_frames.argtypes = [C.c_int, dp, C.c_int64, C.c_int, dp]
    L.se3icp_knn_self.argtypes = [C.c_int, dp, C.c_int64, C.c_int, ip]
    L.se3icp_estimate_normals.argtypes = [C.c_int, dp, C.c_int64, C.c_int, dp]
    L.se3icp_nn.argtypes = [C.c_int, dp, C.c_int64, dp, C.c_int64, C.c_int, ip, dp, ip]
    L.se3icp_synthetic_pairs.restype = C.c_int64
    L.se3icp_synthetic_pairs.argtypes = [C.c_int, dp, C.c_int64, C.c_int32, dp, C.c_double, C.c_double, C.c_uint64,
                                         vp, vp, C.c_int]
    L.se3icp_synthetic_reference.restype = C.c_int64
    L.se3icp_synthetic_reference.argtypes = [dp, C.c_int64, C.c_int32, C.c_double, C.c_double, C.c_double, C.c_double,
                                             C.c_int32, dp, dp, dp]
    L.se3icp_synthetic_reference_device.restype = C.c_int64
    L.se3icp_synthetic_reference_device.argtypes = [C.c_int, dp, C.c_int64, C.c_int32, C.c_double, C.c_double,
                                                    C.c_double, C.c_double, C.c_int32, vp, vp, dp, C.c_int]
    L.se3icp_random_downsample.restype = C.c_int64
    L.se3icp_random_downsample.argtypes = [dp, C.c_int64, C.c_double, C.c_uint32, dp]
    L.se3icp_set_profiling.argtypes = [C.c_int, C.c_int]
    L.se3icp_last_kernel_times.argtypes = [C.c_int, dp]
    L.se3icp_last_kernel_times_n.argtypes = [C.c_int, dp, C.c_int]
    L.se3icp_set_trace.argtypes = [C.c_int, C.POINTER(Trace)]
    L.se3icp_set_lrf_exact.argtypes = [C.c_int, C.c_int]
    L.se3icp_set_nn_events.argtypes = [C.c_int, C.c_int]
    _lib = L
    return L


def status_string(code: int) -> str:
    return load().se3icp_status_string(int(code)).decode()


def check(code: int, what: str = "") -> int:
    if code != OK:
        raise Se3IcpError(code, what)
    return code


def default_params(**overrides) -> Params:
    p = Params()
    load().se3icp_default_params(C.byref(p))
    for k, v in overrides.items():
        setattr(p, k, v)
    return p


def device_count() -> int:
    return load().se3icp_device_count()


def method_id(name: str) -> int:
    m = load().se3icp_method_from_name(name.encode())
    if m < 0:
        raise ValueError(f"unknown method {name!r}; valid: {', '.join(METHODS)}")
    return m
```

se3-icp_amd/se3icp/registration.py:

```python
from __future__ import annotations

import contextlib
import ctypes as C
import threading
import time
from dataclasses import dataclass

import numpy as np

from . import _lib
from .io import read_ply_xyz

_PARAM_FIELDS = {
    "max_num_iterations_": "max_num_iterations",
    "max_num_se3_iterations_": "max_num_se3_iterations",
    "number_of_nn_for_LRF_": "number_of_nn_for_LRF",
    "mse_": "mse",
    "mse_switch_error_": "mse_switch_error",
    "estimated_overlap_": "estimated_overlap",
    "alpha_rot": "alpha_rot",
    "beta_transl": "beta_transl",
    "scale_preprocessing": "scale_preprocessing",
}

# ... 319 lines not shown


@contextlib.contextmanager
def _armed_trace(device: int, slot: int, n_src: int, max_iters: int):
    L = _lib.load()
    tr = {"corr_idx": np.full((max_iters, n_src), -1, np.int32), "corr_dist": np.zeros((max_iters, n_src), np.float32),
          "trim_key": np.zeros(max_iters, np.uint64), "T": np.zeros((max_iters, 4, 4)), "mse": np.zeros(max_iters),
          "phase": np.zeros(max_iters, np.int32)}
    t = _lib.Trace(slot, max_iters, tr["corr_idx"].ctypes.data_as(C.POINTER(C.c_int32)),
                   tr["corr_dist"].ctypes.data_as(C.POINTER(C.c_float)),
                   tr["trim_key"].ctypes.data_as(C.POINTER(C.c_uint64)), tr["T"].ctypes.data_as(_DP),
                   tr["mse"].ctypes.data_as(_DP), tr["phase"].ctypes.data_as(C.POINTER(C.c_int32)), 0, 0)
    _lib.check(L.se3icp_set_trace(device, C.byref(t)), "set_trace")
    trace = {}
    try:
        yield trace
    finally:
        L.se3icp_set_trace(device, None)
    n = int(t.iters_recorded)
    trace.update({k: v[:n] for k, v in tr.items()})


def register_batch_traced(pairs, method: str, params: _lib.Params | None = None, pair: int = 0,
                          max_iters: int = 160, device: int = 0):
    with _armed_trace(device, pair, _as_xyz(pairs[pair][0]).shape[0], max_iters) as trace:
        res = register_batch(pairs, method, params, device)
    return res, trace


def alpha_grid() -> list[float]:
    g = [0.0]
    g += [i * 0.01 for i in range(1, 11)]
    g += [i * 0.1 for i in range(2, 11)]
    g += [1.0 + i * 0.5 for i in range(0, 9)]
    g += [5.0, 7.0, 10.0, 15.0, 25.0, 50.0, 60.0, 70.0, 80.0, 90.0, 100.0, 200.0, 300.0, 400.0, 500.0, 600.0, 700.0,
          800.0, 900.0, 1000.0]
    return sorted(set(g))


def _copy_params(p: _lib.Params) -> _lib.Params:
    q = _lib.Params()
    C.memmove(C.byref(q), C.byref(p), C.sizeof(_lib.Params))
    return q


def sweep_params(base: _lib.Params | None = None, **lists) -> list[_lib.Params]:
    base = base or _lib.default_params()
    lens = {len(v) for v in lists.values()}
    if len(lens) != 1:
        raise ValueError("sweep_params: give at least one list, all of one length")
    fields = {f[0] for f in _lib.Params._fields_}
    out = []
    for i in range(lens.pop()):
        q = _copy_params(base)
        for k, vals in lists.items():
            if k not in fields or k.startswith("_"):
                raise ValueError(f"sweep_params: no parameter {k!r}")
            setattr(q, k, vals[i])
        out.append(q)
    return out


def _variant_array(variants):
    nv = len(variants)
    arr = (_lib.Params * nv)()
    for i, p in enumerate(variants):
        C.memmove(C.byref(arr, i * C.sizeof(_lib.Params)), C.byref(p), C.sizeof(_lib.Params))
    return nv, (arr if nv else None)


def _sweep_results(res, nv, n) -> list[list[PairResult]]:
    flat = _results(res, nv * n)
    return [flat[v * n:(v + 1) * n] for v in range(nv)]


def register_sweep(pairs, method: str, variants, device: int = 0, max_group: int = 0) -> list[list[PairResult]]:
    n, args, _, _keep = _pair_args(pairs)
    nv, var = _variant_array(variants)
    res, _ = _outputs(nv * n)
    _registered(_lib.load().se3icp_register_sweep(device, n, *args, _lib.method_id(method), nv, var, max_group, res),
                "register_sweep")
    return _sweep_results(res, nv, n)


def register_sweep_device(src_ptr: int, src_off, tgt_ptr: int, tgt_off, method: str, variants, device: int = 0,
                          stream: int = 0, max_group: int = 0) -> list[list[PairResult]]:
    n, args = _offset_args(src_ptr, src_off, tgt_ptr, tgt_off)
    nv, var = _variant_array(variants)
    res, _ = _outputs(nv * n)
    _registered(_lib.load().se3icp_register_sweep_device(device, n, *args, _lib.method_id(method), nv, var, max_group,
                                                         res, _stream_arg(stream)), "register_sweep_device")
    return _sweep_results(res, nv, n)


def register_sweep_traced(pairs, method: str, variants, variant: int = 0, pair: int = 0, max_iters: int = 160,
                          device: int = 0, max_group: int = 0):
    with _armed_trace(device, variant * len(pairs) + pair, _as_xyz(pairs[pair][0]).shape[0], max_iters) as trace:
        res = register_sweep(pairs, method, variants, device, max_group)
    return res, trace


@dataclass
class PairReport:
    fitness: float
    inlier_rmse: float
    information: np.ndarray
    final_mse: float
    final_mse_change: float
    n_inliers: int
    switched: int
    stop_reason: int
    corr_idx: np.ndarray | None = None
    corr_dist: np.ndarray | None = None

    @property
    def stop_reason_name(self) -> str:
        return _lib.STOP_REASONS[self.stop_reason]


def _report(r, idx=None, dist=None) -> PairReport:
    return PairReport(float(r.fitness), float(r.inlier_rmse), np.array(r.information).reshape(6, 6), float(r.final_mse),
                      float(r.final_mse_change), int(r.n_inliers), int(r.switched), int(r.stop_reason), idx, dist)


def _report_options(max_correspondence_distance: float, idx_ptr=None, dist_ptr=None, on_device=False):
    return _lib.ReportOptions(float(max_correspondence_distance), idx_ptr, dist_ptr, 1 if on_device else 0, 0)


def _per_point_options(max_correspondence_distance: float, counts, per_point: bool):
    idx = np.full(sum(counts), -1, np.int32) if per_point else None
    dist = np.zeros(sum(counts)) if per_point else None
    return _report_options(max_correspondence_distance, idx.ctypes.data if per_point else None,
                           dist.ctypes.data if per_point else None), idx, dist


def _pair_reports(rep, counts, idx=None, dist=None) -> list[PairReport]:
    out, at = [], 0
    for i, n in enumerate(counts):
        out.append(_report(rep[i], None if idx is None else idx[at:at + n], None if dist is None else dist[at:at + n]))
        at += n
    return out


def register_batch_report(pairs, method: str, params: _lib.Params | None = None, device: int = 0,
                          max_correspondence_distance: float = 0.0, per_point: bool = False):
    n, args, counts, _keep = _pair_args(pairs)
    res, rep = _outputs(n)
    opts, idx, dist = _per_point_options(max_correspondence_distance, counts, per_point)
    _registered(_lib.load().se3icp_register_batch_report(device, n, *args, _lib.method_id(method), _params_ref(params),
                                                         res, C.byref(opts), rep), "register_batch_report")
    return _results(res, n), _pair_reports(rep, counts, idx, dist)


def register_batch_report_device(src_ptr: int, src_off, tgt_ptr: int, tgt_off, method: str,
                                 params: _lib.Params | None = None, device: int = 0, stream: int = 0,
                                 max_correspondence_distance: float = 0.0, corr_idx_ptr: int = 0,
                                 corr_dist_ptr: int = 0, outputs_on_device: bool = True):
    n, args = _offset_args(src_ptr, src_off, tgt_ptr, tgt_off)
    res, rep = _outputs(n)
    opts = _report_options(max_correspondence_distance, corr_idx_ptr or None, corr_dist_ptr or None, outputs_on_device)
    _registered(_lib.load().se3icp_register_batch_report_device(device, n, *args, _lib.method_id(method),
                                                                _params_ref(params), res, _stream_arg(stream),
                                                                C.byref(opts), rep), "register_batch_report_device")
    return _results(res, n), [_report(rep[i]) for i in range(n)]


def _sweep_reports(rep, nv, n):
    return [[_report(rep[v * n + p]) for p in range(n)] for v in range(nv)]


def register_sweep_report(pairs, method: str, variants, device: int = 0, max_group: int = 0,
                          max_correspondence_distance: float = 0.0):
    n, args, _, _keep = _pair_args(pairs)
    nv, var = _variant_array(variants)
    res, rep = _outputs(nv * n)
    opts = _report_options(max_correspondence_distance)
    _registered(_lib.load().se3icp_register_sweep_report(device, n, *args, _lib.method_id(method), nv, var, max_group,
                                                         res, C.byref(opts), rep), "register_sweep_report")
    return _sweep_results(res, nv, n), _sweep_reports(rep, nv, n)


def register_sweep_report_device(src_ptr: int, src_off, tgt_ptr: int, tgt_off, method: str, variants, device: int = 0,
                                 stream: int = 0, max_group: int = 0, max_correspondence_distance: float = 0.0):
    n, args = _offset_args(src_ptr, src_off, tgt_ptr, tgt_off)
    nv, var = _variant_array(variants)
    res, rep = _outputs(nv * n)
    opts = _report_options(max_correspondence_distance)
    _registered(_lib.load().se3icp_register_sweep_report_device(device, n, *args, _lib.method_id(method), nv, var,
                                                                max_group, res, _stream_arg(stream), C.byref(opts),
                                                                rep), "register_sweep_report_device")
    return _sweep_results(res, nv, n), _sweep_reports(rep, nv, n)


def sequence_edges(n: int) -> list[tuple[int, int]]:
    return [(i + 1, i) for i in range(max(0, int(n) - 1))]


def expand_edges(clouds, edges):
    return [(clouds[int(s)], clouds[int(t)]) for s, t in edges]


def _edge_arrays(edges):
    n = len(edges)
    es = (C.c_int32 * max(n, 1))(*[int(s) for s, _ in edges])
    et = (C.c_int32 * max(n, 1))(*[int(t) for _, t in edges])
    return n, es, et


def register_graph(clouds, edges, method: str, params: _lib.Params | None = None, device: int = 0,
                   sharing: int = 0) -> list[PairResult]:
    _keep, cargs = _cloud_args(clouds)
    n, es, et = _edge_arrays(edges)
    res, _ = _outputs(n)
    _registered(_lib.load().se3icp_register_graph(device, *cargs, n, es, et, _lib.method_id(method), _params_ref(params),
                                                  int(sharing), res), "register_graph")
    return _results(res, n)


def register_sequence(clouds, method: str, params: _lib.Params | None = None, device: int = 0,
                      sharing: int = 0) -> list[PairResult]:
    return register_graph(clouds, sequence_edges(len(clouds)), method, params, device, sharing)


def register_graph_device(xyz_ptr: int, off, edges, method: str, params: _lib.Params | None = None,
                          device: int = 0, stream: int = 0, sharing: int = 0) -> list[PairResult]:
    nc = len(off) - 1
    co = (C.c_int64 * (nc + 1))(*[int(x) for x in off])
    n, es, et = _edge_arrays(edges)
    res, _ = _outputs(n)
    _registered(_lib.load().se3icp_register_graph_device(device, nc, C.c_void_p(xyz_ptr), co, n, es, et,
                                                         _lib.method_id(method), _params_ref(params), int(sharing),
                                                         res, _stream_arg(stream)), "register_graph_device")
    return _results(res, n)


def register_graph_report(clouds, edges, method: str, params: _lib.Params | None = None, device: int = 0,
                          sharing: int = 0, max_correspondence_distance: float = 0.0, per_point: bool = False):
    cl, cargs = _cloud_args(clouds)
    n, es, et = _edge_arrays(edges)
    counts = [cl[int(s)].shape[0] for s, _ in edges]
    res, rep = _outputs(n)
    opts, idx, dist = _per_point_options(max_correspondence_distance, counts, per_point)
    _registered(_lib.load().se3icp_register_graph_report(device, *cargs, n, es, et, _lib.method_id(method),
                                                         _params_ref(params), int(sharing), res, C.byref(opts), rep),
                "register_graph_report")
    return _results(res, n), _pair_reports(rep, counts, idx, dist)


def register_graph_traced(clouds, edges, method: str, params: _lib.Params | None = None, edge: int = 0,
                          max_iters: int = 160, device: int = 0, sharing: int = 0):
    with _armed_trace(device, edge, _as_xyz(clouds[int(edges[edge][0])]).shape[0], max_iters) as trace:
        res = register_graph(clouds, edges, method, params, device, sharing)
    return res, trace


def last_graph_stats(device: int = 0) -> dict:
    out = (C.c_int64 * len(_lib.GRAPH_STATS))()
    _lib.check(_lib.load().se3icp_last_graph_stats(device, out, len(_lib.GRAPH_STATS)), "last_graph_stats")
    return {k: int(out[i]) for i, k in enumerate(_lib.GRAPH_STATS)}


def set_batch_sharing(level: int, device: int = 0) -> None:
    _lib.check(_lib.load().se3icp_set_batch_sharing(int(device), int(level)), "set_batch_sharing")


def toldi_frames(pts, k: int, device: int = 0) -> np.ndarray:
    pts = _as_xyz(pts)
    out = np.zeros((pts.shape[0], 4, 4))
    _lib.check(_lib.load().se3icp_toldi_frames(device, pts.ctypes.data_as(C.POINTER(C.c_double)), pts.shape[0], k,
                                               out.ctypes.data_as(C.POINTER(C.c_double))), "toldi_frames")
    return out


def knn_self(pts, k: int, device: int = 0) -> np.ndarray:
    pts = _as_xyz(pts)
    out = np.zeros((pts.shape[0], k), np.int32)
    _lib.check(_lib.load().se3icp_knn_self(device, pts.ctypes.data_as(C.POINTER(C.c_double)), pts.shape[0], k,
                                           out.ctypes.data_as(C.POINTER(C.c_int32))), "knn_self")
    return out


def estimate_normals(pts, k: int = 30, device: int = 0) -> np.ndarray:
    pts = _as_xyz(pts)
    out = np.zeros_like(pts)
    _lib.check(_lib.load().se3icp_estimate_normals(device, pts.ctypes.data_as(C.POINTER(C.c_double)), pts.shape[0],
                                                   k, out.ctypes.data_as(C.POINTER(C.c_double))), "estimate_normals")
    return out


def nearest_neighbors(query, data, device: int = 0):
    q = np.ascontiguousarray(query, dtype=np.float64)
    d = np.ascontiguousarray(data, dtype=np.float64)
    dim = d.shape[1]
    idx = np.zeros(q.shape[0], np.int32)
    d2 = np.zeros(q.shape[0])
    nr = C.c_int32(0)
    dp = C.POINTER(C.c_double)
    _lib.check(_lib.load().se3icp_nn(device, q.ctypes.data_as(dp), q.shape[0], d.ctypes.data_as(dp), d.shape[0], dim,
                                     idx.ctypes.data_as(C.POINTER(C.c_int32)), d2.ctypes.data_as(dp), C.byref(nr)),
               "nn")
    return idx, d2, int(nr.value)


def set_lrf_exact(mode, device: int = 0) -> None:
    _lib.check(_lib.load().se3icp_set_lrf_exact(device, int(mode)))


def set_nn_events(on: bool, device: int = 0) -> None:
    _lib.check(_lib.load().se3icp_set_nn_events(device, 1 if on else 0))


def set_profiling(on: bool, device: int = 0) -> None:
    _lib.check(_lib.load().se3icp_set_profiling(device, 1 if on else 0))


def last_kernel_times(device: int = 0) -> dict:
    keys = DeviceBatchRunner._KT_KEYS
    out = (C.c_double * len(keys))()
    _lib.check(_lib.load().se3icp_last_kernel_times_n(device, out, len(keys)))
    return dict(zip(keys, list(out)))
```

Baseline: 16560.

## Seed LRF kNN search radius from duplicate cloud classes in graph plans

```diff
diff --git a/include/se3icp.h b/include/se3icp.h
--- a/include/se3icp.h
+++ b/include/se3icp.h
@@ -121,6 +121,10 @@
 
 int se3icp_set_batch_sharing(int device, int level);
 
+int se3icp_set_lrf_seeding(int device, int mode);
+#define SE3ICP_SEED_STATS_N 4
+int se3icp_last_seed_stats(int device, int64_t* out, int n);
+
 typedef enum se3icp_stop_reason {
     SE3ICP_STOP_CONVERGED = 0,
     SE3ICP_STOP_MAX_ITERATIONS = 1,
diff --git a/se3-icp_amd/csrc/capi.cpp b/se3-icp_amd/csrc/capi.cpp
--- a/se3-icp_amd/csrc/capi.cpp
+++ b/se3-icp_amd/csrc/capi.cpp
@@ -353,6 +353,24 @@
     if (!e) return SE3ICP_ERR_NO_DEVICE;
     std::lock_guard<std::mutex> lk(e->mutex());
     e->set_batch_sharing(level);
+    return SE3ICP_OK;
+}
+
+int se3icp_set_lrf_seeding(int device, int mode) {
+    if (mode < se3icp::kLrfSeedingMin || mode > se3icp::kLrfSeedingMax) return SE3ICP_ERR_INVALID_ARG;
+    Engine* e = usable_engine(device);
+    if (!e) return SE3ICP_ERR_NO_DEVICE;
+    std::lock_guard<std::mutex> lk(e->mutex());
+    e->set_lrf_seeding(mode);
+    return SE3ICP_OK;
+}
+
+int se3icp_last_seed_stats(int device, int64_t* out, int n) {
+    if (!out || n < 4) return SE3ICP_ERR_INVALID_ARG;
+    Engine* e = usable_engine(device);
+    if (!e) return SE3ICP_ERR_NO_DEVICE;
+    std::lock_guard<std::mutex> lk(e->mutex());
+    for (int k = 0; k < 4; ++k) out[k] = e->seed_stats()[k];
     return SE3ICP_OK;
 }
 
diff --git a/se3-icp_amd/csrc/common.hpp b/se3-icp_amd/csrc/common.hpp
--- a/se3-icp_amd/csrc/common.hpp
+++ b/se3-icp_amd/csrc/common.hpp
@@ -8,6 +8,7 @@
 constexpr int kRedVals = 28;
 constexpr int kStatCols = 17;
 constexpr int kStatUseSe3 = 15, kStatUseR3 = 16;
+constexpr int kSeedStatCol = 14;
 constexpr int kHist = 256;
 constexpr int kTrimList = 4096;
 constexpr int kTrimBlocks = 32;
diff --git a/se3-icp_amd/csrc/engine.cpp b/se3-icp_amd/csrc/engine.cpp
--- a/se3-icp_amd/csrc/engine.cpp
+++ b/se3-icp_amd/csrc/engine.cpp
@@ -450,17 +450,34 @@
             launch_lrf(v, knn_list_ ? 1 : 0, s);
             big(nullptr, nullptr, kSmallK);
         } else {
-            std::vector<int32_t> wb(nclouds_ + 1, 0);
-            for (int c = 0; c < nclouds_; ++c) wb[c + 1] = wb[c] + (h_setup_[c].k_knn > 0 ? (h_clouds_[c].n + 7) / 8 : 0);
-            const int nw = wb[nclouds_];
-            if (!ensure<int32_t>(d_lrf_fb_, (size_t)8 * nw + 64) || !ensure<int32_t>(d_lrf_fbn_, 2 + nclouds_ + 1))
+            const bool seeding = seed_on_;
+            const int nt = nclouds_ + 1;
+            std::vector<int32_t> wb(2 * (size_t)nt, 0);
+            for (int c = 0; c < nclouds_; ++c) {
+                const int waves = h_setup_[c].k_knn > 0 ? (h_clouds_[c].n + 7) / 8 : 0;
+                const bool sd = seeding && seed_ref_[c].load >= 0;
+                wb[c + 1] = wb[c] + (sd ? 0 : waves);
+                wb[nt + c + 1] = wb[nt + c] + (sd ? waves : 0);
+            }
+            const int nw = wb[nclouds_], nw_sd = wb[nt + nclouds_];
+            if (!ensure<int32_t>(d_lrf_fb_, (size_t)8 * (nw + nw_sd) + 64) || !ensure<int32_t>(d_lrf_fbn_, 2 + 2 * (size_t)nt))
                 return SE3ICP_ERR_OUT_OF_MEMORY;
             int32_t* d_wb = (int32_t*)d_lrf_fbn_.p + 2;
             int32_t* fb = (int32_t*)d_lrf_fb_.p;
             int32_t* fbn = (int32_t*)d_lrf_fbn_.p;
             HIPCHK(hipMemsetAsync(fbn, 0, 2 * sizeof(int32_t), s));
-            HIPCHK(hipMemcpyAsync(d_wb, wb.data(), sizeof(int32_t) * (nclouds_ + 1), hipMemcpyHostToDevice, s));
-            launch_lrf8(v, d_wb, 0, nw, fb, fbn, s);
+            HIPCHK(hipMemcpyAsync(d_wb, wb.data(), sizeof(int32_t) * 2 * nt, hipMemcpyHostToDevice, s));
+            if (seeding) {
+                if (!ensure<float>(d_seed_, (size_t)seed_floats_) || !ensure<SeedRef>(d_seed_ref_, nclouds_))
+                    return SE3ICP_ERR_OUT_OF_MEMORY;
+                HIPCHK(hipMemsetAsync(d_seed_.p, 0xff, sizeof(float) * (size_t)seed_floats_, s));
+                HIPCHK(hipMemcpyAsync(d_seed_ref_.p, seed_ref_.data(), sizeof(SeedRef) * nclouds_, hipMemcpyHostToDevice, s));
+                launch_lrf8(v, d_wb, 0, nw, fb, fbn, s, (const SeedRef*)d_seed_ref_.p, (float*)d_seed_.p, false, lrf_seeding_);
+                launch_lrf8(v, d_wb + nt, 0, nw_sd, fb, fbn, s, (const SeedRef*)d_seed_ref_.p, (float*)d_seed_.p, true,
+                            lrf_seeding_);
+            } else {
+                launch_lrf8(v, d_wb, 0, nw, fb, fbn, s);
+            }
             launch_lrf_list(v, fb, fbn, s);
             big(fb, fbn, kSmallK);
         }
@@ -489,6 +506,11 @@
     ktimes_.lrf_box_tests = sum[3];
     ktimes_.lrf_candidates = sum[4];
     ktimes_.lrf_fallback = sum[6];
+    for (int k = 0; k < 3; ++k) {
+        unsigned long long q = 0;
+        for (int i = 0; i < kStatSlots; ++i) q += h_lrf_stats_[kStatCols * i + kSeedStatCol + k];
+        seed_stats_[1 + k] = (int64_t)q;
+    }
 #ifdef SE3ICP_PROF
     tree_prof_report();
     std::fprintf(stderr, "[prof] k_lrf cycles/query: knn|scan %.0f sort|tighten %.0f sums|final+sums %.0f finish %.0f "
@@ -538,6 +560,7 @@
     HIPCHK(hipSetDevice(dev_));
     c->s = user_stream ? user_stream : stream_;
     ktimes_ = KernelTimes{};
+    for (int64_t& x : seed_stats_) x = 0;
     HIPCHK(hipEventRecord(ev_[12], c->s));
     return 0;
 }
@@ -714,9 +737,40 @@
     }
     const int nchS = (int)sel_chunks_.size();
     if (!ensure<ChunkWork>(g_chunks_, nchS) || !ensure<GraphSeg>(g_seg_, U)) return SE3ICP_ERR_OUT_OF_MEMORY;
+    seed_ref_.clear();
+    seed_floats_ = 0;
+    if (lrf_seeding_ != 1 && lrf_exact_only_ == 0 && !knn_list_) {
+        std::vector<int32_t> kk(K);
+        std::vector<int64_t> nn(K);
+        for (int k = 0; k < K; ++k) {
+            kk[k] = sel_run_[home[k]].k_knn;
+            nn[k] = h_clouds_[home[k]].n;
+        }
+        std::vector<SeedClass> sc;
+        const int seeded = graph_plan_seeds(plan, kk.data(), nn.data(), &sc);
+        int64_t total = 0;
+        for (int k = 0; k < K; ++k)
+            if (sc[k].from >= 0) total += nn[k];
+        if (seeded > 0 && total <= INT32_MAX) {
+            seed_ref_.assign(U, SeedRef{-1, -1, 1.0});
+            for (int k = 0; k < K; ++k) {
+                if (sc[k].from < 0) continue;
+                SeedRef& src = seed_ref_[home[sc[k].from]];
+                if (src.store < 0) {
+                    src.store = (int32_t)seed_floats_;
+                    seed_floats_ += nn[k];
+                }
+                seed_ref_[home[k]].load = src.store;
+                seed_ref_[home[k]].rho2 = sc[k].rho2;
+            }
+            seed_stats_[0] = seeded;
+            seed_on_ = true;
+        }
+    }
     h_setup_ = sel_run_;
     HIPCHK(hipMemcpyAsync(d_setup_.p, sel_run_.data(), sizeof(CloudSetup) * U, hipMemcpyHostToDevice, s));
     const int rc = setup_knn(s);
+    seed_on_ = false;
     if (rc) return rc;
     HIPCHK(hipGetLastError());
     h_setup_ = sel_batch_;
diff --git a/se3-icp_amd/csrc/engine.hpp b/se3-icp_amd/csrc/engine.hpp
--- a/se3-icp_amd/csrc/engine.hpp
+++ b/se3-icp_amd/csrc/engine.hpp
@@ -69,6 +69,7 @@
     void set_lrf_exact(int mode) { lrf_exact_only_ = mode; }
     void set_nn_events(bool on) { nn_events_ = on; }
     void set_batch_sharing(int level) { batch_sharing_ = level; }
+    void set_lrf_seeding(int mode) { lrf_seeding_ = mode; }
     const KernelTimes& kernel_times() const { return ktimes_; }
 
     int register_batch(int npairs, const double* const* src, const int64_t* ns, const double* const* tgt,
@@ -85,6 +86,7 @@
                        se3icp_result* out, hipStream_t user_stream, const se3icp_report_options* ropts = nullptr,
                        se3icp_report* reports = nullptr);
     const int64_t* graph_stats() const { return graph_stats_; }
+    const int64_t* seed_stats() const { return seed_stats_; }
 
     int knn_self(const double* xyz, int64_t n, int k, int32_t* idx);
     int toldi_frames(const double* xyz, int64_t n, int k, double* frames);
@@ -154,6 +156,7 @@
     int lrf_exact_only_ = 0;
     bool nn_events_ = true;
     int batch_sharing_ = 0;
+    int lrf_seeding_ = 0;
     se3icp_trace* trace_ = nullptr;
     int record_trace(se3icp_trace* tr, int it, int& phase_of_it, hipStream_t s);
     double trace_prev_[kStatCols] = {};
@@ -190,6 +193,11 @@
     std::vector<ChunkWork> sel_chunks_;
     std::vector<GraphSeg> sel_seg_;
     int64_t graph_stats_[9] = {};
+    bool seed_on_ = false;
+    std::vector<SeedRef> seed_ref_;
+    int64_t seed_floats_ = 0;
+    DevBuf d_seed_{bufs_}, d_seed_ref_{bufs_};
+    int64_t seed_stats_[4] = {};
     Pinned<PairDev> h_pairs_{pins_};
     Pinned<double> h_red_{pins_}, h_partial_{pins_};
     Pinned<int32_t> h_rechecked_{pins_};
diff --git a/se3-icp_amd/csrc/graph.hpp b/se3-icp_amd/csrc/graph.hpp
--- a/se3-icp_amd/csrc/graph.hpp
+++ b/se3-icp_amd/csrc/graph.hpp
@@ -42,6 +42,7 @@
 struct GraphPlan {
     std::vector<int32_t> use_class;
     std::vector<GraphClass> classes;
+    bool normalize = false, dedupe = false;
 };
 
 struct GraphUse {
@@ -64,6 +65,8 @@
     std::map<Key, int32_t> seen;
     plan->use_class.assign((size_t)n_uses, -1);
     plan->classes.clear();
+    plan->normalize = normalize;
+    plan->dedupe = dedupe;
     for (int32_t u = 0; u < n_uses; ++u) {
         GraphClass g{};
         g.cloud = use[u].cloud;
@@ -104,6 +107,40 @@
         if (it == owner.end()) owner[g.cloud] = k;
         else if (plan->classes[it->second].k_nrm == g.k_nrm) g.nrm_from = it->second;
     }
+}
+
+constexpr int kLrfSeedingMin = 0, kLrfSeedingMax = 3;
+struct SeedClass {
+    int32_t from;
+    double rho2;
+};
+inline int32_t graph_plan_seeds(const GraphPlan& plan, const int32_t* k_knn, const int64_t* n_pts,
+                                std::vector<SeedClass>* seed) {
+    const int32_t K = (int32_t)plan.classes.size();
+    seed->assign((size_t)K, SeedClass{-1, 1.0});
+    if (!plan.normalize || !plan.dedupe) return 0;
+    auto uncentred = [](const GraphClass& g) { return g.f32_center[0] == 0.0 && g.f32_center[1] == 0.0 && g.f32_center[2] == 0.0; };
+    std::map<int32_t, int32_t> source;
+    int32_t seeded = 0;
+    for (int32_t k = 0; k < K; ++k) {
+        if (k_knn[k] <= 0) continue;
+        const GraphClass& g = plan.classes[k];
+        auto it = source.find(g.cloud);
+        if (it == source.end()) {
+            source[g.cloud] = k;
+            continue;
+        }
+        const int32_t a = it->second;
+        const GraphClass& ga = plan.classes[a];
+        const int64_t kw = k_knn[k] < n_pts[k] ? k_knn[k] : n_pts[k], kwa = k_knn[a] < n_pts[a] ? k_knn[a] : n_pts[a];
+        const double rho = g.norm_scale / ga.norm_scale;
+        if (std::memcmp(g.norm_center, ga.norm_center, sizeof(g.norm_center)) != 0 || !uncentred(g) || !uncentred(ga) ||
+            n_pts[k] != n_pts[a] || kw > kwa || !(rho > 0.0) || !std::isfinite(rho * rho))
+            continue;
+        (*seed)[k] = SeedClass{a, rho * rho};
+        ++seeded;
+    }
+    return seeded;
 }
 
 inline void graph_plan(int32_t n_pairs, const int32_t* src, const int32_t* tgt, bool normalize, double scale_pre,
diff --git a/se3-icp_amd/csrc/k_lrf8.hip b/se3-icp_amd/csrc/k_lrf8.hip
--- a/se3-icp_amd/csrc/k_lrf8.hip
+++ b/se3-icp_amd/csrc/k_lrf8.hip
@@ -208,6 +208,7 @@
     const unsigned tg = nbg >= Kw ? widen_bound(kth_of_two(list, mv, B, nb, Kw - 1) | kIdBits, S) : kAll;
     const int ka = upper_count(list, mv, tg), kb = upper_count(B, nb, tg);
     const int kept = ka + kb;
+    if (presort && tail_per == 0) return make_uint3(tg, (unsigned)ka, (unsigned)ka);
     if (__ballot(kept > 128) == 0ull) {
         unsigned k[16];
         load_head<16>(list, ka, l, k);
@@ -383,11 +384,13 @@
 
 static_assert(kW >= 2 && kW * kQ <= 64, "the per-block epilogue: waves 0 and 1, a lane per query");
 
+template <bool SD, bool ST>
 __global__ __launch_bounds__(64 * kW) __attribute__((amdgpu_waves_per_eu(kCap <= 192 ? 6 : (kCap <= 224 ? 5 : 4)))) void k_lrf8(
     View v, const int32_t* __restrict__ cloud_of, const CloudSetup* __restrict__ setup,
     const CloudDev* __restrict__ clouds, const float* __restrict__ tlo, const float* __restrict__ thi,
     const double4* __restrict__ P4, const int32_t* __restrict__ wave_base, int w_lo, int nwaves,
-    int32_t* __restrict__ fb_list, int32_t* __restrict__ fb_count) {
+    int32_t* __restrict__ fb_list, int32_t* __restrict__ fb_count, const SeedRef* __restrict__ seed,
+    float* __restrict__ seedbuf, int seed_mode) {
     __shared__ __attribute__((aligned(16))) unsigned s_list[kW][kQ][kStride];
     auto park_of = [&](int w, int j) __attribute__((always_inline)) {
         return reinterpret_cast<double*>(&s_list[w][j][kParkAt]);
@@ -480,6 +483,28 @@
         }
         n_q = kQ;
     }
+    bool sd_open = false, sd_close = false, t_cert = true;
+    unsigned n_sdq = 0, n_sda = 0, n_sdf = 0;
+    if constexpr (SD) {
+        if (mode == 2) n_sda = (unsigned)qn;
+        if (mode == 1) {
+            const SeedRef sr = seed[c];
+            float sv = 0.f;
+            if (lane < kQ) sv = seedbuf[sr.load + T.perm[w0 + lane]];
+            if (seed_mode == 2) sv *= 0.5f;
+            if (seed_mode == 3) sv *= 4.f;
+            if (__ballot(!(bool)((int)(sv >= 0.f) & (int)(sv < INFINITY))) == 0ull) {
+                const unsigned t0 = f32_up_bits((double)sv * sr.rho2 * (1.0 + 0x1p-20)) | kIdBits;
+                const unsigned tb = widen_bound(widen_bound(t0, s_norm), s_norm);
+#pragma unroll
+                for (int j = 0; j < kQ; ++j) Tq[j] = (unsigned)__builtin_amdgcn_readlane((int)tb, j);
+                sd_open = true;
+                n_sdq = kQ;
+            } else {
+                n_sda = kQ;
+            }
+        }
+    }
 
     auto tighten = [&]() __attribute__((always_inline)) {
         ++n_sel;
@@ -500,10 +525,22 @@
         const uint3 r3 = tighten_group_sorted(lists, g, l, (int)group_len(), mvv, (int)nmax, Kw, presort, tail_per, s_norm);
         mvv = (int)r3.z;
         __builtin_amdgcn_wave_barrier();
-#pragma unroll
-        for (int j = 0; j < kQ; ++j) {
-            Tq[j] = (unsigned)__builtin_amdgcn_readlane((int)r3.x, 8 * j);
-            nbq[j] = (unsigned)__builtin_amdgcn_readlane((int)r3.y, 8 * j);
+        if constexpr (SD) {
+            bool cert = true;
+#pragma unroll
+            for (int j = 0; j < kQ; ++j) {
+                const unsigned tn = (unsigned)__builtin_amdgcn_readlane((int)r3.x, 8 * j);
+                cert &= tn <= Tq[j];
+                Tq[j] = min(Tq[j], tn);
+                nbq[j] = (unsigned)__builtin_amdgcn_readlane((int)r3.y, 8 * j);
+            }
+            t_cert = cert;
+        } else {
+#pragma unroll
+            for (int j = 0; j < kQ; ++j) {
+                Tq[j] = (unsigned)__builtin_amdgcn_readlane((int)r3.x, 8 * j);
+                nbq[j] = (unsigned)__builtin_amdgcn_readlane((int)r3.y, 8 * j);
+            }
         }
     };
 
@@ -596,6 +633,9 @@
         int cur = -1, part = 0;
         bool do_tighten = false, retried = false;
         float tf = INFINITY;
+        if constexpr (SD) {
+            if (sd_open) tf = thr_f();
+        }
         while (!fb_wave) {
             if (do_tighten) {
                 PROF8_NOW(t_t0);
@@ -603,6 +643,16 @@
                 PROF8_NOW(t_t1);
                 PROF8_ADD(c_tight, t_t0, t_t1);
                 do_tighten = false;
+                if constexpr (SD) {
+                    if (sd_close) {
+                        sd_close = false;
+                        if (!t_cert) {
+                            fb_wave = true;
+                            n_sdf = kQ;
+                            continue;
+                        }
+                    }
+                }
                 tf = thr_f();
 #if defined(SE3ICP_LRF8_CUT) && SE3ICP_LRF8_CUT == 4
                 if (stage == 2) break;
@@ -634,7 +684,7 @@
             int leaf = -1;
             if (stage == 0) {
                 leaf = nxt++;
-                if (nxt > lf1) stage = 1;
+                if (nxt > lf1) stage = (SD && sd_open) ? 2 : 1;
             } else if (stage == 1) {
                 const bool more_hi = s_hi < nleaf - 1, more_lo = s_lo > 0;
                 const int cand = (more_hi && (up || !more_lo)) ? s_hi + 1 : s_lo - 1;
@@ -651,6 +701,15 @@
             } else if (stage == 2) {
                 if (!haveA) {
                     if (c0 >= nA) {
+                        if constexpr (SD) {
+                            if (sd_open) {
+                                sd_open = false;
+                                sd_close = true;
+                                do_tighten = true;
+                                retried = true;
+                                continue;
+                            }
+                        }
                         unsigned nmax = 0;
 #pragma unroll
                         for (int j = 0; j < kQ; ++j) nmax = max(nmax, nbq[j]);
@@ -741,6 +800,15 @@
 #endif
     const unsigned* rl = lists + g * kStride;
     double* pj = park_of(wid, g);
+    if constexpr (ST) {
+        if (mode == 1) {
+            const int so = seed[c].store;
+            if ((int)(so >= 0) & (int)mine & (int)(l == 0)) {
+                const p3 f = ld3(P4, (int)rl[Kw - 1]);
+                seedbuf[so + T.perm[wq]] = (float)l2_3(qg.x, qg.y, qg.z, f.x, f.y, f.z);
+            }
+        }
+    }
     {
         double x[12];
 #pragma unroll
@@ -823,6 +891,11 @@
         atomicAdd(ctr + 1, (unsigned long long)n_leaves);
         atomicAdd(ctr + 2, (unsigned long long)n_sel);
         atomicAdd(ctr + 4, (unsigned long long)n_cand);
+        if constexpr (SD) {
+            if (n_sdq) atomicAdd(ctr + kSeedStatCol, (unsigned long long)n_sdq);
+            if (n_sda) atomicAdd(ctr + kSeedStatCol + 1, (unsigned long long)n_sda);
+            if (n_sdf) atomicAdd(ctr + kSeedStatCol + 2, (unsigned long long)n_sdf);
+        }
     }
 
 #if defined(SE3ICP_LRF8_CUT) && SE3ICP_LRF8_CUT == 3
@@ -952,11 +1025,18 @@
 }
 
 void launch_lrf8(const View& v, const int32_t* wave_base, int w_lo, int w_hi, int32_t* fb_list, int32_t* fb_count,
-                 hipStream_t s) {
+                 hipStream_t s, const SeedRef* seed, float* seedbuf, bool seeded, int seed_mode) {
     const int nb = (w_hi - w_lo + kW - 1) / kW;
     if (nb <= 0) return;
-    hipLaunchKernelGGL(k_lrf8, dim3(nb), dim3(64 * kW), 0, s, v, v.cloud_of, v.setup, v.clouds, v.t3.lo, v.t3.hi,
-                       v.t3.tpt64, wave_base, w_lo, w_hi, fb_list, fb_count);
-}
-
-}
+    if (seeded)
+        hipLaunchKernelGGL((k_lrf8<true, false>), dim3(nb), dim3(64 * kW), 0, s, v, v.cloud_of, v.setup, v.clouds, v.t3.lo,
+                           v.t3.hi, v.t3.tpt64, wave_base, w_lo, w_hi, fb_list, fb_count, seed, seedbuf, seed_mode);
+    else if (seed != nullptr)
+        hipLaunchKernelGGL((k_lrf8<false, true>), dim3(nb), dim3(64 * kW), 0, s, v, v.cloud_of, v.setup, v.clouds, v.t3.lo,
+                           v.t3.hi, v.t3.tpt64, wave_base, w_lo, w_hi, fb_list, fb_count, seed, seedbuf, seed_mode);
+    else
+        hipLaunchKernelGGL((k_lrf8<false, false>), dim3(nb), dim3(64 * kW), 0, s, v, v.cloud_of, v.setup, v.clouds, v.t3.lo,
+                           v.t3.hi, v.t3.tpt64, wave_base, w_lo, w_hi, fb_list, fb_count, seed, seedbuf, seed_mode);
+}
+
+}
diff --git a/se3-icp_amd/csrc/view.hpp b/se3-icp_amd/csrc/view.hpp
--- a/se3-icp_amd/csrc/view.hpp
+++ b/se3-icp_amd/csrc/view.hpp
@@ -103,8 +103,10 @@
                        int state_stride, hipStream_t s);
 void launch_lrf(const View& v, int write_knn, hipStream_t s);
 void launch_lrf_list(const View& v, const int32_t* qlist, const int32_t* qcount, hipStream_t s, int qpw = 0);
+struct SeedRef { int32_t store; int32_t load; double rho2; };
 void launch_lrf8(const View& v, const int32_t* wave_base, int w_lo, int w_hi, int32_t* fb_list, int32_t* fb_count,
-                 hipStream_t s);
+                 hipStream_t s, const SeedRef* seed = nullptr, float* seedbuf = nullptr, bool seeded = false,
+                 int seed_mode = 0);
 int knn_big_cap(int kw_max);
 int knn_big_blocks(int cap, int nq);
 void launch_knn_big(const View& v, int write_knn, int k_min, const int32_t* qlist, const int32_t* qcount, int nblocks,
diff --git a/se3-icp_amd/se3icp/__init__.py b/se3-icp_amd/se3icp/__init__.py
--- a/se3-icp_amd/se3icp/__init__.py
+++ b/se3-icp_amd/se3icp/__init__.py
@@ -12,7 +12,7 @@
                            register_sweep_report_device,
                            expand_edges, last_graph_stats, register_graph, register_graph_device,
                            register_graph_report, register_graph_traced, register_sequence, sequence_edges,
-                           set_batch_sharing)
+                           set_batch_sharing, set_lrf_seeding, last_seed_stats)
 from ._lib import Report, ReportOptions
 
 __all__ = [
@@ -24,5 +24,5 @@
     "register_sweep_report", "register_sweep_report_device",
     "register_graph", "register_sequence", "sequence_edges", "expand_edges", "register_graph_device",
     "register_graph_report", "register_graph_traced", "last_graph_stats",
-    "set_batch_sharing",
+    "set_batch_sharing", "set_lrf_seeding", "last_seed_stats",
 ]
diff --git a/se3-icp_amd/se3icp/_lib.py b/se3-icp_amd/se3icp/_lib.py
--- a/se3-icp_amd/se3icp/_lib.py
+++ b/se3-icp_amd/se3icp/_lib.py
@@ -31,6 +31,7 @@
     "se3icp_register_sweep", "se3icp_register_sweep_device",
     "se3icp_register_graph", "se3icp_register_graph_device", "se3icp_register_graph_report",
     "se3icp_register_graph_report_device", "se3icp_last_graph_stats", "se3icp_set_batch_sharing",
+    "se3icp_set_lrf_seeding", "se3icp_last_seed_stats",
     "se3icp_report_version", "se3icp_register_batch_report", "se3icp_register_batch_report_device",
     "se3icp_register_sweep_report", "se3icp_register_sweep_report_device",
     "se3icp_request_report", "se3icp_get_report",
@@ -124,6 +125,7 @@
 
 GRAPH_STATS = ["clouds", "uses", "classes", "classes_full", "adopted", "rejected_order", "rejected_gap", "no_list",
                "bytes_uploaded"]
+SEED_STATS = ["classes_seeded", "queries_seeded", "queries_unseeded", "queries_failed"]
 
 
 class Se3IcpError(RuntimeError):
diff --git a/se3-icp_amd/se3icp/registration.py b/se3-icp_amd/se3icp/registration.py
--- a/se3-icp_amd/se3icp/registration.py
+++ b/se3-icp_amd/se3icp/registration.py
@@ -645,6 +645,16 @@
     return idx, d2, int(nr.value)
 
 
+def set_lrf_seeding(mode: int, device: int = 0) -> None:
+    _lib.check(_lib.load().se3icp_set_lrf_seeding(int(device), int(mode)), "set_lrf_seeding")
+
+
+def last_seed_stats(device: int = 0) -> dict:
+    out = (C.c_int64 * len(_lib.SEED_STATS))()
+    _lib.check(_lib.load().se3icp_last_seed_stats(int(device), out, len(_lib.SEED_STATS)), "last_seed_stats")
+    return {k: int(out[i]) for i, k in enumerate(_lib.SEED_STATS)}
+
+
 def set_lrf_exact(mode, device: int = 0) -> None:
     _lib.check(_lib.load().se3icp_set_lrf_exact(device, int(mode)))
 
```

Result: faster. 17410, median of 6 (+5.2%).
